# mayursharma/PageRank-using-Apache-Spark

Measured on AMD Instinct MI355X. Metric: PageRank GTEPS/iter + % HBM roofline, R-MAT scale-26 at 1/2/4/8 MI355X, higher is better.
Workload: dtype f64

## Files before the change

include/pagerank_hip.h:

```cpp
#ifndef PAGERANK_HIP_H
#define PAGERANK_HIP_H

#include <stdint.h>

#ifdef __cplusplus
extern "C" {
#endif

#define PR_ABI_VERSION 2

#define PR_OK 0
#define PR_ERR_INVALID (-1)
#define PR_ERR_HIP (-2)
#define PR_ERR_OOM (-3)
#define PR_ERR_COMM (-4)
#define PR_ERR_STATE (-5)
#define PR_ERR_NODEVICE (-6)

#define PR_DANGLING_LOCAL 0u
#define PR_DANGLING_NONE 1u
#define PR_INPUT_DEVICE 2u
#define PR_NO_CANONICAL 4u
#define PR_LAYOUT_FUSED 8u
#define PR_LAYOUT_SPLIT 16u

#define PR_VF_KEY 1u
#define PR_VF_SINK 2u
#define PR_VF_NOLINK 4u
#define PR_VF_INDEG0 8u

#define PR_INFO_N_VERTICES 0
#define PR_INFO_N_EDGES 1
#define PR_INFO_N_SINK 2
#define PR_INFO_N_NOLINK 3
#define PR_INFO_N_INDEG0 4
#define PR_INFO_MAX_INDEG 5
#define PR_INFO_LOCAL_ROWS 6
#define PR_INFO_LOCAL_EDGES 7
#define PR_INFO_PART 8
#define PR_INFO_N_PARTS 9
#define PR_INFO_N_UNITS 10
#define PR_INFO_N_LONG_ROWS 11
#define PR_INFO_DEVICE_BYTES 12
#define PR_INFO_CLASSES 13
#define PR_INFO_XCHG_SEND 14
#define PR_INFO_XCHG_RECV 15
#define PR_INFO_PARTIAL_SLOTS 16
#define PR_INFO_HOT_SLOTS 17
#define PR_INFO_EPILOGUE 18
#define PR_INFO_GATHER_EST 19
#define PR_INFO_WALK_GROUPS 20
#define PR_INFO_LAYOUT 21
#define PR_INFO_HOT_COVER 22
#define PR_INFO_CODE_BITS 23
#define PR_INFO_HOT_GATHER 24
#define PR_INFO_COUNT 25

#define PR_STAT_ITERS 0
#define PR_STAT_LAST_DC 1
#define PR_STAT_LAST_L1 2
#define PR_STAT_SPMV_MS_MEAN 3
#define PR_STAT_SPMV_LAUNCHES 4
#define PR_STAT_ITER_MS_MEAN 5
#define PR_STAT_BUILD_MS 6
#define PR_STAT_EXCHANGE_MS_MEAN 7
#define PR_STAT_COUNT 8

typedef struct pr_graph pr_graph;

typedef void (*pr_iter_cb)(int32_t iter, const double *ranks_or_null, double dangling_sum,
                           double l1_delta, double ms, void *user);
#define PR_CB_RANKS 1u

int pr_abi_version(void);
const char *pr_last_error(void);
int pr_device_count(int32_t *out);

int pr_graph_create(int32_t device, int32_t n_vertices, int64_t n_edges, const int32_t *src,
                    const int32_t *dst, uint32_t flags, pr_graph **out);

int pr_graph_create_part(int32_t device, int32_t part, int32_t n_parts, int32_t n_vertices,
                         int64_t n_edges, const int32_t *src, const int32_t *dst, uint32_t flags,
                         pr_graph **out);

#define PR_BOPT_CLASSES 1
#define PR_BOPT_HOT_SLOTS 2
#define PR_BOPT_EXCHANGE 3
#define PR_BOPT_XCHG_CHUNKS 4
#define PR_BOPT_HOT_RESERVE 5
#define PR_BOPT_EPI_WALK 6
#define PR_BOPT_EPI_NARROW 7
#define PR_BOPT_CODES 8
#define PR_BOPT_PACK_FUSED 9
#define PR_BOPT_XCHG_SDMA 10
#define PR_BOPT_EPI_ORDER 11
int pr_graph_create_ex(int32_t device, int32_t part, int32_t n_parts, int32_t n_vertices, int64_t n_edges,
                       const int32_t *src, const int32_t *dst, uint32_t flags, const int64_t *options,
                       int32_t n_options, pr_graph **out);

int pr_graph_info(const pr_graph *g, int64_t *info, int32_t n_info);

int pr_graph_export_csr(const pr_graph *g, int64_t *row_ptr, int32_t *col_idx, int32_t *out_deg,
                        uint8_t *vflags);

int pr_run(pr_graph *g, int32_t iterations, double teleport, double damping,
           const double *init_ranks, double *ranks_out, pr_iter_cb cb, uint32_t cb_flags,
           void *user);

int pr_reset(pr_graph *g, double teleport, double damping, const double *init_ranks);
int pr_step(pr_graph *g, int32_t iterations);
int pr_sync(pr_graph *g);
int pr_get_ranks(pr_graph *g, double *ranks_out);

int pr_set_teleport(pr_graph *g, const double *teleport);
int pr_set_teleport_sparse(pr_graph *g, int32_t n, const int32_t *ids, const double *values, double rest);

int pr_get_topk(pr_graph *g, int32_t k, int32_t *ids_out, double *ranks_out, int32_t *n_out);
int pr_topk_merge(int32_t n_lists, const int32_t *const *ids, const double *const *ranks,
                  const int32_t *counts, int32_t k, int32_t *ids_out, double *ranks_out, int32_t *n_out);
int pr_set_timing(pr_graph *g, int32_t enable);
int pr_get_stats(pr_graph *g, double *stats, int32_t n_stats);

#define PR_OPT_XCHG_CHUNKS 1
#define PR_OPT_HOT_RESERVE 2
#define PR_OPT_XCHG_IPC 3
#define PR_OPT_XCHG_IPC_BLIT 4
#define PR_OPT_HOT_GATHER 5
int pr_set_option(pr_graph *g, int32_t option, int64_t value);

#define PR_COMM_ID_BYTES 128
int pr_comm_unique_id(uint8_t *id_out);
int pr_graph_attach_comm(pr_graph *g, int32_t rank, int32_t n_ranks, const uint8_t *id);

int pr_group_reset(pr_graph *const *parts, int32_t n_parts, double teleport, double damping,
                   const double *init_ranks);
int pr_group_step(pr_graph *const *parts, int32_t n_parts, int32_t iterations);
int pr_group_sync(pr_graph *const *parts, int32_t n_parts);
int pr_group_topk(pr_graph *const *parts, int32_t n_parts, int32_t k, int32_t *ids_out,
                  double *ranks_out, int32_t *n_out);

void pr_graph_destroy(pr_graph *g);

typedef struct pr_batch pr_batch;
int pr_batch_create(pr_graph *g, int32_t width, pr_batch **out);
int pr_batch_set_teleport(pr_batch *b, int32_t column, const double *teleport);
int pr_batch_set_teleport_sparse(pr_batch *b, int32_t column, int32_t n, const int32_t *ids,
                                 const double *values, double rest);
int pr_batch_reset(pr_batch *b, double teleport, double damping, const double *init_ranks);
int pr_batch_step(pr_batch *b, int32_t iterations);
int pr_batch_step_until(pr_batch *b, int32_t max_iterations, double tol, int32_t *iters_out);
int pr_batch_reset_column(pr_batch *b, int32_t column, const double *init_ranks);
int pr_batch_step_until_any(pr_batch *b, uint32_t active, int32_t max_iterations, double tol,
                            int32_t *executed_out, uint32_t *converged_out);
typedef struct pr_batch_query {
  int32_t n_seeds;
  const int32_t *ids;
  const double *values;
  double rest;
  int32_t n_exclude;
  const int32_t *exclude;
} pr_batch_query;
typedef void (*pr_batch_done_cb)(int32_t query, int32_t column, int32_t iterations, int32_t converged,
                                 double l1, void *user);
int pr_batch_run_queue(pr_batch *b, int32_t n_queries, const pr_batch_query *queries,
                       int32_t max_iterations, double tol, const double *init_ranks,
                       pr_batch_done_cb done, void *user);
#define PR_BATCH_DANGLING_UNIFORM 0
#define PR_BATCH_DANGLING_TELEPORT 1
int pr_batch_set_dangling(pr_batch *b, int32_t mode);
int pr_batch_get_dangling(const pr_batch *b, int32_t *mode_out);
int pr_batch_get_teleport_sums(pr_batch *b, double *sums_out);
int pr_batch_sync(pr_batch *b);
int pr_batch_get_ranks(pr_batch *b, int32_t column, double *ranks_out);
int pr_batch_get_norms(pr_batch *b, double *dc_out, double *l_out);
int pr_batch_get_topk(pr_batch *b, int32_t column, int32_t k, int32_t *ids_out, double *ranks_out,
                      int32_t *n_out);
int pr_batch_set_exclude(pr_batch *b, int32_t column, int32_t n, const int32_t *ids);
int pr_batch_get_topk_all(pr_batch *b, int32_t k, int32_t *ids_out, double *ranks_out, int32_t *n_out);
int pr_batch_info(const pr_batch *b, int64_t *info, int32_t n_info);
void pr_batch_destroy(pr_batch *b);

int pr_gen_rmat(int32_t device, int32_t scale, int64_t n_edges, double a, double b, double c,
                uint64_t seed, int32_t *d_src, int32_t *d_dst);
int pr_gen_er(int32_t device, int32_t scale, int64_t n_edges, uint64_t seed, int32_t *d_src,
              int32_t *d_dst);
int pr_gen_chunglu(int32_t device, int32_t n_labels, int64_t n_edges, double gamma_out, double v0_out,
                   double gamma_in, double v0_in, double src_frac, int64_t n_nolink, uint64_t seed,
                   int32_t *d_src, int32_t *d_dst);
int pr_intern_device(int32_t device, int64_t n_edges, int32_t label_bound, int32_t *d_src,
                     int32_t *d_dst, int32_t *n_vertices_out);

#ifdef __cplusplus
}
#endif

#endif
```

java/src/sparky/hip/PageRankHip.java:

```java
package sparky.hip;

import static java.lang.foreign.ValueLayout.ADDRESS;
import static java.lang.foreign.ValueLayout.JAVA_DOUBLE;
import static java.lang.foreign.ValueLayout.JAVA_INT;
import static java.lang.foreign.ValueLayout.JAVA_LONG;

import java.lang.foreign.Arena;
import java.lang.foreign.FunctionDescriptor;
import java.lang.foreign.Linker;
import java.lang.foreign.MemorySegment;
import java.lang.foreign.SymbolLookup;
import java.lang.invoke.MethodHandle;
import java.lang.invoke.MethodHandles;
import java.lang.invoke.MethodType;

public final class PageRankHip implements AutoCloseable {
    public static final int PR_DANGLING_LOCAL = 0, PR_DANGLING_NONE = 1, PR_NO_CANONICAL = 4;
    static final int PR_CB_RANKS = 1;
    static final int PR_INFO_COUNT = 25;
    public static final int ABI_VERSION = 2;

    private static final Linker LINKER = Linker.nativeLinker();
    private static final SymbolLookup LIB = SymbolLookup.libraryLookup(
            System.getProperty("pagerank.hip.lib", "libpagerank_hip.so"), Arena.global());

    private static MethodHandle h(String name, FunctionDescriptor d) {
        return LINKER.downcallHandle(LIB.find(name).orElseThrow(
                () -> new UnsatisfiedLinkError("libpagerank_hip lacks " + name)), d);
    }

    private static final MethodHandle CREATE = h("pr_graph_create", FunctionDescriptor.of(JAVA_INT,
            JAVA_INT, JAVA_INT, JAVA_LONG, ADDRESS, ADDRESS, JAVA_INT, ADDRESS));
    private static final MethodHandle RUN = h("pr_run", FunctionDescriptor.of(JAVA_INT,
            ADDRESS, JAVA_INT, JAVA_DOUBLE, JAVA_DOUBLE, ADDRESS, ADDRESS, ADDRESS, JAVA_INT, ADDRESS));
    private static final MethodHandle INFO = h("pr_graph_info", FunctionDescriptor.of(JAVA_INT,
            ADDRESS, ADDRESS, JAVA_INT));
    private static final MethodHandle DESTROY = h("pr_graph_destroy", FunctionDescriptor.ofVoid(ADDRESS));
    private static final MethodHandle LAST_ERROR = h("pr_last_error", FunctionDescriptor.of(ADDRESS));
    private static final MethodHandle ABI = h("pr_abi_version", FunctionDescriptor.of(JAVA_INT));

    static {
        try {
            int v = (int) ABI.invokeExact();
            if (v != ABI_VERSION)
                throw new UnsatisfiedLinkError("libpagerank_hip ABI " + v + ", this binding needs " + ABI_VERSION);
        } catch (UnsatisfiedLinkError e) {
            throw e;
        } catch (Throwable t) {
            throw new ExceptionInInitializerError(t);
        }
    }
    private static final FunctionDescriptor CB_DESC = FunctionDescriptor.ofVoid(
            JAVA_INT, ADDRESS, JAVA_DOUBLE, JAVA_DOUBLE, JAVA_DOUBLE, ADDRESS);

    private final Arena arena = Arena.ofConfined();
    private final MemorySegment graph;
    private final int nVertices;
    private IterationListener listener;
    private Throwable listenerError;

    public PageRankHip(int device, int nVertices, int[] src, int[] dst, int flags) throws Throwable {
        if (src.length != dst.length) throw new IllegalArgumentException("src and dst lengths differ");
        this.nVertices = nVertices;
        try (Arena call = Arena.ofConfined()) {
            MemorySegment s = call.allocateFrom(JAVA_INT, src);
            MemorySegment d = call.allocateFrom(JAVA_INT, dst);
            MemorySegment out = call.allocate(ADDRESS);
            check((int) CREATE.invokeExact(device, nVertices, (long) src.length, s, d, flags | PR_NO_CANONICAL, out));
            graph = out.get(ADDRESS, 0);
        }
    }

    public long[] info() throws Throwable {
        try (Arena call = Arena.ofConfined()) {
            MemorySegment a = call.allocate(JAVA_LONG, PR_INFO_COUNT);
            check((int) INFO.invokeExact(graph, a, PR_INFO_COUNT));
            return a.toArray(JAVA_LONG);
        }
    }

    public double[] run(int iterations, double[] initRanks, IterationListener l, boolean ranksInCallback)
            throws Throwable {
        if (initRanks != null && initRanks.length != nVertices)
            throw new IllegalArgumentException("initRanks must hold " + nVertices + " ranks");
        listener = l;
        listenerError = null;
        try (Arena call = Arena.ofConfined()) {
            MemorySegment init = initRanks == null ? MemorySegment.NULL : call.allocateFrom(JAVA_DOUBLE, initRanks);
            MemorySegment out = call.allocate(JAVA_DOUBLE, Math.max(nVertices, 1));
            MemorySegment cb = MemorySegment.NULL;
            if (l != null) {
                MethodHandle target = MethodHandles.lookup().findVirtual(PageRankHip.class, "upcall",
                        MethodType.methodType(void.class, int.class, MemorySegment.class, double.class,
                                double.class, double.class, MemorySegment.class)).bindTo(this);
                cb = LINKER.upcallStub(target, CB_DESC, call);
            }
            int rc = (int) RUN.invokeExact(graph, iterations, 0.15, 0.85, init, out, cb,
                    ranksInCallback ? PR_CB_RANKS : 0, MemorySegment.NULL);
            if (listenerError != null) throw listenerError;
            check(rc);
            return out.asSlice(0, 8L * nVertices).toArray(JAVA_DOUBLE);
        } finally {
            listener = null;
        }
    }

    private void upcall(int iter, MemorySegment ranks, double dc, double l1, double ms, MemorySegment user) {
        if (listenerError != null) return;
        try {
            double[] r = ranks.equals(MemorySegment.NULL) ? null
                    : ranks.reinterpret(8L * nVertices).toArray(JAVA_DOUBLE);
            listener.onIteration(iter, r, dc, l1, ms);
        } catch (Throwable t) {
            listenerError = t;
        }
    }

    private static void check(int rc) throws Throwable {
        if (rc != 0) {
            MemorySegment msg = (MemorySegment) LAST_ERROR.invokeExact();
            throw new RuntimeException("libpagerank_hip error " + rc + ": " + msg.reinterpret(4096).getString(0));
        }
    }

    @Override
    public void close() throws Throwable {
        DESTROY.invokeExact(graph);
        arena.close();
    }
}
```

pagerank-using-apache-spark_amd/csrc/pr_api.hip:

```cpp
#include <rccl/rccl.h>

#include <algorithm>
#include <chrono>
#include <cmath>
#include <cstring>
#include <new>
#include <string>
#include <vector>

#include "pr_graph.h"
#include "pr_topk.h"
#include "pr_xcheck.h"

namespace pr {

static thread_local std::string g_last_error;

void set_error(const std::string &msg) { g_last_error = msg; }
int fail(int code, const std::string &msg) {
  g_last_error = msg;
  return code;
}

int DevBuf::alloc(size_t n) {
  reset();
  if (n == 0) n = 1;
  hipError_t e = hipMalloc(&p, n);
  if (e != hipSuccess) {
    p = nullptr;
    (void)hipGetLastError();
    return fail(PR_ERR_OOM, "hipMalloc(" + std::to_string(n) + " bytes) failed: " + hipGetErrorString(e));
  }
  bytes = n;
  return PR_OK;
}

void DevBuf::reset() {
  if (p) (void)hipFree(p);
  p = nullptr;
  bytes = 0;
}

}

size_t pr_graph::device_bytes() const {
  size_t b = canon_rowptr.bytes + canon_col.bytes + canon_deg.bytes + canon_vflags.bytes;
  b += rowptr.bytes + col.bytes + colp.bytes + rowinfo.bytes + colh.bytes + hunits.bytes + partial.bytes + poff.bytes + rmask.bytes + cbase.bytes + seg_slot.bytes + seg_p0.bytes + r.bytes + cbuf[0].bytes + cbuf[1].bytes + eoff.bytes + epos.bytes;
  b += units.bytes + unit_part.bytes + lr_row.bytes + lr_p0.bytes + piece_part.bytes;
  b += fin_part.bytes + fin_counter.bytes + reset_part.bytes + x_send.bytes + x_sbuf.bytes + hpos.bytes + cside.bytes;
  b += pr::topk_bytes(this);
  b += tele.bytes;
  return b;
}

using pr::fail;

namespace {

struct DeviceGuard {
  int prev = -1;
  explicit DeviceGuard(int dev) {
    if (hipGetDevice(&prev) != hipSuccess) prev = -1;
    (void)hipSetDevice(dev);
  }
  ~DeviceGuard() {
    if (prev >= 0) (void)hipSetDevice(prev);
  }
};

int check_device(int32_t device) {
  int n = 0;
  hipError_t e = hipGetDeviceCount(&n);
  if (e != hipSuccess || n <= 0) {
    (void)hipGetLastError();
    return fail(PR_ERR_NODEVICE, "no HIP device available");
  }
  if (device < 0 || device >= n) return fail(PR_ERR_INVALID, "device index out of range");
  return PR_OK;
}

int parse_options(const int64_t *options, int32_t n, pr_build_opts *o) {
  if (n < 0 || (n > 0 && !options)) return fail(PR_ERR_INVALID, "options is NULL");
  for (int32_t i = 0; i < n; ++i) {
    const int64_t k = options[2 * i], v = options[2 * i + 1];
    switch (k) {
      case PR_BOPT_CLASSES:
        if (v != 0 && v != 8 && v != 16 && v != 32 && v != 64 && v != 128)
          return fail(PR_ERR_INVALID, "PR_BOPT_CLASSES: 0 (policy), 8, 16, 32, 64 or 128");
        o->classes = (int)v;
        break;
      case PR_BOPT_HOT_SLOTS:
        if (v < -1 || v > pr::kHotSlotsMax) return fail(PR_ERR_INVALID, "PR_BOPT_HOT_SLOTS: -1 (default) or 0..18429");
        o->hot_slots = (int)v;
        break;
      case PR_BOPT_EXCHANGE:
        if (v != 0 && v != 1) return fail(PR_ERR_INVALID, "PR_BOPT_EXCHANGE: 0 (runs) or 1 (all-gather)");
        o->allgather = v == 1;
        break;
      case PR_BOPT_XCHG_CHUNKS:
        if (v != 0 && v != 1) return fail(PR_ERR_INVALID, "PR_BOPT_XCHG_CHUNKS: 0 (whole runs) or 1 (overlapped)");
        o->xchg_chunks = v == 1;
        break;
      case PR_BOPT_HOT_RESERVE:
        if (v < 0 || v > 3) return fail(PR_ERR_INVALID, "PR_BOPT_HOT_RESERVE: 0..3 CUs per XCD");
        o->hot_reserve = (int)v;
        break;
      case PR_BOPT_EPI_WALK:
        if (v != 0 && v != 1) return fail(PR_ERR_INVALID, "PR_BOPT_EPI_WALK: 0 (class loop) or 1 (per-row walk)");
        o->epi_walk = v == 1;
        break;
      case PR_BOPT_EPI_NARROW:
        if (v < -1 || v > 1) return fail(PR_ERR_INVALID, "PR_BOPT_EPI_NARROW: -1 (auto), 0 or 1");
        o->epi_narrow = (int)v;
        break;
      case PR_BOPT_CODES:
        if (v != -1 && v != 0) return fail(PR_ERR_INVALID, "PR_BOPT_CODES: -1 (compact where they fit) or 0 (32-bit)");
        o->codes = (int)v;
        break;
      case PR_BOPT_PACK_FUSED:
        if (v != 0 && v != 1) return fail(PR_ERR_INVALID, "PR_BOPT_PACK_FUSED: 0 (pack kernel) or 1 (in the epilogue)");
        o->pack_fused = v == 1;
        break;
      case PR_BOPT_XCHG_SDMA:
        if (v != 0 && v != 1) return fail(PR_ERR_INVALID, "PR_BOPT_XCHG_SDMA: 0 (device copies) or 1 (copy engines)");
        o->xchg_sdma = v == 1;
        break;
      case PR_BOPT_EPI_ORDER:
        if (v < -1 || v > 2)
          return fail(PR_ERR_INVALID, "PR_BOPT_EPI_ORDER: -1 (auto), 0 (row order), 1 (runs of 8 groups heaviest first), "
                                      "2 (groups heaviest first)");
        o->epi_order = (int)v;
        break;
      default:
        return fail(PR_ERR_INVALID, "unknown build option " + std::to_string(k));
    }
  }
  return PR_OK;
}

int create_common(int32_t device, int32_t part, int32_t n_parts, int32_t n_vertices, int64_t n_edges,
                  const int32_t *src, const int32_t *dst, uint32_t flags, const int64_t *options,
                  int32_t n_options, pr_graph **out) {
  if (!out) return fail(PR_ERR_INVALID, "out is NULL");
  *out = nullptr;
  if (n_parts < 1 || part < 0 || part >= n_parts) return fail(PR_ERR_INVALID, "bad part / n_parts");
  if (n_parts > pr::kMaxParts) return fail(PR_ERR_INVALID, "n_parts above 64 is not supported");
  if (n_vertices < 0 || n_edges < 0) return fail(PR_ERR_INVALID, "negative size");
  if (n_edges > 0 && (!src || !dst)) return fail(PR_ERR_INVALID, "src/dst is NULL");
  if (flags & ~(PR_DANGLING_NONE | PR_INPUT_DEVICE | PR_NO_CANONICAL | PR_LAYOUT_FUSED | PR_LAYOUT_SPLIT))
    return fail(PR_ERR_INVALID, "unknown flag bits");
  if ((flags & PR_LAYOUT_FUSED) && (flags & PR_LAYOUT_SPLIT)) return fail(PR_ERR_INVALID, "PR_LAYOUT_FUSED and PR_LAYOUT_SPLIT are exclusive");
  pr_build_opts opts;
  PR_TRY(parse_options(options, n_options, &opts));
  PR_TRY(check_device(device));
  DeviceGuard dg(device);
  pr_graph *g = new (std::nothrow) pr_graph();
  if (!g) return fail(PR_ERR_OOM, "host allocation failed");
  g->opts = opts;
  g->device = device;
  g->flags = flags;
  g->V = n_vertices;
  g->part = part;
  g->nparts = n_parts;
  if (hipStreamCreateWithFlags(&g->stream, hipStreamNonBlocking) != hipSuccess) {
    delete g;
    return fail(PR_ERR_HIP, "hipStreamCreate failed");
  }
  int rc = pr::build_graph(g, n_edges, src, dst);
  if (rc != PR_OK) {
    std::string msg = pr_last_error();
    pr_graph_destroy(g);
    pr::set_error(msg);
    return rc;
  }
  *out = g;
  return PR_OK;
}

}

extern "C" {

int pr_abi_version(void) { return PR_ABI_VERSION; }

const char *pr_last_error(void) { return pr::g_last_error.c_str(); }

int pr_device_count(int32_t *out) {
  if (!out) return fail(PR_ERR_INVALID, "out is NULL");
  int n = 0;
  hipError_t e = hipGetDeviceCount(&n);
  if (e != hipSuccess) {
    (void)hipGetLastError();
    n = 0;
  }
  *out = n;
  return PR_OK;
}

int pr_graph_create(int32_t device, int32_t n_vertices, int64_t n_edges, const int32_t *src,
                    const int32_t *dst, uint32_t flags, pr_graph **out) {
  return create_common(device, 0, 1, n_vertices, n_edges, src, dst, flags, nullptr, 0, out);
}

int pr_graph_create_part(int32_t device, int32_t part, int32_t n_parts, int32_t n_vertices,
                         int64_t n_edges, const int32_t *src, const int32_t *dst, uint32_t flags,
                         pr_graph **out) {
  return create_common(device, part, n_parts, n_vertices, n_edges, src, dst, flags, nullptr, 0, out);
}

int pr_graph_create_ex(int32_t device, int32_t part, int32_t n_parts, int32_t n_vertices, int64_t n_edges,
                       const int32_t *src, const int32_t *dst, uint32_t flags, const int64_t *options,
                       int32_t n_options, pr_graph **out) {
  return create_common(device, part, n_parts, n_vertices, n_edges, src, dst, flags, options, n_options, out);
}

static int64_t xchg_volume(const pr_graph *g, bool send) {
  if (g->nparts <= 1) return 0;
  if (g->x_allgather) return (send ? 1 : g->nparts - 1) * g->S_pad;
  const std::vector<int64_t> &o = send ? g->x_soff : g->x_roff;
  return o.empty() ? 0 : o.back();
}

int pr_graph_info(const pr_graph *g, int64_t *info, int32_t n_info) {
  if (!g || !info) return fail(PR_ERR_INVALID, "NULL argument");
  const int64_t v[PR_INFO_COUNT] = {g->V,        g->E_dedup,  g->n_sink,    g->n_nolink, g->n_indeg0,
                                    g->max_indeg, g->n_local,  g->local_nnz, g->part,     g->nparts,
                                    g->n_units + g->n_hunits, g->n_long + g->n_segs,
                                    (int64_t)g->device_bytes(), g->C,
                                    xchg_volume(g, true), xchg_volume(g, false), g->n_slots,
                                    g->C > 1 ? (int64_t)g->hot.P * g->hot.Kp : 0,
                                    g->C == 1 ? 0 : 3, g->gather_est, g->n_walk_groups, g->layout,
                                    g->hot_cover_ppm, g->C > 1 ? (g->code == pr::kCodeC20 || g->code == pr::kCodeC20P ? 20 : g->code == pr::kCodeC24 || g->code == pr::kCodeC24P ? 24 : 32) : 0,
                                    pr::hot_gather_dense(g) ? 1 : 0};
  for (int32_t i = 0; i < n_info && i < PR_INFO_COUNT; ++i) info[i] = v[i];
  return PR_OK;
}

int pr_graph_export_csr(const pr_graph *g, int64_t *row_ptr, int32_t *col_idx, int32_t *out_deg,
                        uint8_t *vflags) {
  if (!g) return fail(PR_ERR_INVALID, "NULL graph");
  if (!g->has_canonical) return fail(PR_ERR_STATE, "canonical CSR was dropped (PR_NO_CANONICAL)");
  DeviceGuard dg(g->device);
  hipStream_t s = g->stream;
  if (row_ptr)
    PR_HIP(hipMemcpyAsync(row_ptr, g->canon_rowptr.p, sizeof(int64_t) * ((size_t)g->V + 1), hipMemcpyDeviceToHost, s));
  if (col_idx && g->E_dedup > 0)
    PR_HIP(hipMemcpyAsync(col_idx, g->canon_col.p, sizeof(int32_t) * g->E_dedup, hipMemcpyDeviceToHost, s));
  if (out_deg && g->V > 0)
    PR_HIP(hipMemcpyAsync(out_deg, g->canon_deg.p, sizeof(int32_t) * g->V, hipMemcpyDeviceToHost, s));
  if (vflags && g->V > 0)
    PR_HIP(hipMemcpyAsync(vflags, g->canon_vflags.p, (size_t)g->V, hipMemcpyDeviceToHost, s));
  PR_HIP(hipStreamSynchronize(s));
  return PR_OK;
}

int pr_reset(pr_graph *g, double teleport, double damping, const double *init_ranks) {
  if (!g) return fail(PR_ERR_INVALID, "NULL graph");
  DeviceGuard dg(g->device);
  g->teleport = teleport;
  g->damping = damping;
  return pr::iter_reset(g, init_ranks);
}

int pr_set_teleport(pr_graph *g, const double *teleport) {
  if (!g) return fail(PR_ERR_INVALID, "NULL graph");
  if (teleport)
    for (int32_t v = 0; v < g->V; ++v)
      if (!std::isfinite(teleport[v])) return fail(PR_ERR_INVALID, "teleport[" + std::to_string(v) + "] is not finite");
  DeviceGuard dg(g->device);
  return teleport ? pr::set_teleport_dense(g, teleport) : pr::clear_teleport(g);
}

int pr_set_teleport_sparse(pr_graph *g, int32_t n, const int32_t *ids, const double *values, double rest) {
  if (!g) return fail(PR_ERR_INVALID, "NULL graph");
  if (n < 0) return fail(PR_ERR_INVALID, "n < 0");
  if (n > 0 && (!ids || !values)) return fail(PR_ERR_INVALID, "NULL argument");
  if (!std::isfinite(rest)) return fail(PR_ERR_INVALID, "rest is not finite");
  for (int32_t i = 0; i < n; ++i) {
    if (ids[i] < 0 || ids[i] >= g->V)
      return fail(PR_ERR_INVALID, "ids[" + std::to_string(i) + "] = " + std::to_string(ids[i]) + " is outside [0, V)");
    if (!std::isfinite(values[i])) return fail(PR_ERR_INVALID, "values[" + std::to_string(i) + "] is not finite");
  }
  if (n > 1) {
    std::vector<int32_t> sorted(ids, ids + n);
    std::sort(sorted.begin(), sorted.end());
    const auto dup = std::adjacent_find(sorted.begin(), sorted.end());
    if (dup != sorted.end()) return fail(PR_ERR_INVALID, "vertex " + std::to_string(*dup) + " is listed twice in ids");
  }
  DeviceGuard dg(g->device);
  return pr::set_teleport_sparse(g, n, ids, values, rest);
}

int pr_step(pr_graph *g, int32_t iterations) {
  if (!g || iterations < 0) return fail(PR_ERR_INVALID, "bad argument");
  DeviceGuard dg(g->device);
  return pr::iter_step(g, iterations);
}

int pr_sync(pr_graph *g) {
  if (!g) return fail(PR_ERR_INVALID, "NULL graph");
  DeviceGuard dg(g->device);
  PR_TRY(pr::join_exchange(g));
  PR_HIP(hipStreamSynchronize(g->stream));
  return PR_OK;
}

int pr_get_ranks(pr_graph *g, double *ranks_out) {
  if (!g || !ranks_out) return fail(PR_ERR_INVALID, "NULL argument");
  if (!g->ready) return fail(PR_ERR_STATE, "pr_get_ranks before pr_reset");
  DeviceGuard dg(g->device);
  std::vector<double> loc((size_t)g->n_rows);
  if (g->n_rows > 0)
    PR_HIP(hipMemcpyAsync(loc.data(), g->r.p, sizeof(double) * g->n_rows, hipMemcpyDeviceToHost, g->stream));
  PR_HIP(hipStreamSynchronize(g->stream));
  for (int64_t L = 0; L < g->n_rows; ++L)
    if (g->orig_of_local[L] >= 0) ranks_out[g->orig_of_local[L]] = loc[L];
  return PR_OK;
}

int pr_set_timing(pr_graph *g, int32_t enable) {
  if (!g) return fail(PR_ERR_INVALID, "NULL graph");
  g->timing = enable != 0;
  return PR_OK;
}

int pr_set_option(pr_graph *g, int32_t option, int64_t value) {
  if (!g) return fail(PR_ERR_INVALID, "NULL graph");
  DeviceGuard dg(g->device);
  if (option == PR_OPT_HOT_RESERVE) {
    if (value < 0 || value > 3) return fail(PR_ERR_INVALID, "PR_OPT_HOT_RESERVE: 0..3 CUs per XCD");
    if (g->C > 1) PR_TRY(pr::set_hot_reserve(g, (int)value));
    return PR_OK;
  }
  if (option == PR_OPT_HOT_GATHER) {
    if (value < -1 || value > 1) return fail(PR_ERR_INVALID, "PR_OPT_HOT_GATHER: -1 (auto), 0 (per position) or 1 (dense)");
    if (g->C > 1) g->hot_gather = (int)value;
    return PR_OK;
  }
  if (option == PR_OPT_XCHG_IPC_BLIT) {
    if (value != 0 && value != 1) return fail(PR_ERR_INVALID, "PR_OPT_XCHG_IPC_BLIT: 0 (copy engines) or 1 (blit kernel)");
    PR_TRY(pr::join_exchange(g));
    g->x_ipc_blit = value == 1;
    return PR_OK;
  }
  if (option == PR_OPT_XCHG_IPC) {
    if (value < 0 || value > 2)
      return fail(PR_ERR_INVALID, "PR_OPT_XCHG_IPC: 0 (RCCL), 1 (IPC copy engines) or 2 (IPC, per-chunk publication)");
    return pr::set_exchange_ipc(g, (int)value);
  }
  if (option != PR_OPT_XCHG_CHUNKS) return fail(PR_ERR_INVALID, "unknown option");
  PR_TRY(pr::join_exchange(g));
  g->x_chunked = value != 0 && g->n_xc > 1;
  if (g->comm && g->comm_size > 1) PR_TRY(pr::verify_exchange(g));
  return PR_OK;
}

int pr_get_stats(pr_graph *g, double *stats, int32_t n_stats) {
  if (!g || !stats) return fail(PR_ERR_INVALID, "NULL argument");
  DeviceGuard dg(g->device);
  PR_TRY(pr::join_exchange(g));
  PR_HIP(hipStreamSynchronize(g->stream));
  auto mean_ms = [&](const std::vector<std::pair<int, int>> &ev, double *out) -> int {
    double acc = 0.0;
    for (auto &pr_ : ev) {
      float ms = 0.f;
      PR_HIP(hipEventElapsedTime(&ms, g->ev_pool[pr_.first], g->ev_pool[pr_.second]));
      acc += ms;
    }
    *out = ev.empty() ? 0.0 : acc / (double)ev.size();
    return PR_OK;
  };
  double v[PR_STAT_COUNT] = {0};
  v[PR_STAT_ITERS] = (double)g->iters_done;
  if (g->ready) {
    PR_TRY(pr::read_slots(g, g->cur, &v[PR_STAT_LAST_DC], &v[PR_STAT_LAST_L1]));
    if (g->iters_done > 0) {
      double dc_prev = 0, l1_prev = 0;
      PR_TRY(pr::read_slots(g, g->cur ^ 1, &dc_prev, &l1_prev));
      v[PR_STAT_LAST_DC] = dc_prev;
    } else {
      v[PR_STAT_LAST_L1] = 0.0;
    }
  }
  PR_TRY(mean_ms(g->spmv_ev, &v[PR_STAT_SPMV_MS_MEAN]));
  if (g->spmv_passes > 0) v[PR_STAT_SPMV_MS_MEAN] *= (double)g->spmv_ev.size() / (double)g->spmv_passes;
  v[PR_STAT_SPMV_LAUNCHES] = (double)g->spmv_passes;
  if (g->xchg_ev.size() == g->iter_ev.size() && !g->xchg_ev.empty()) {
    double acc = 0.0;
    for (size_t i = 0; i < g->iter_ev.size(); ++i) {
      float a = 0.f, b = 0.f;
      PR_HIP(hipEventElapsedTime(&a, g->ev_pool[g->iter_ev[i].first], g->ev_pool[g->iter_ev[i].second]));
      PR_HIP(hipEventElapsedTime(&b, g->ev_pool[g->iter_ev[i].first], g->ev_pool[g->xchg_ev[i].second]));
      acc += a > b ? a : b;
    }
    v[PR_STAT_ITER_MS_MEAN] = acc / (double)g->iter_ev.size();
  } else {
    PR_TRY(mean_ms(g->iter_ev, &v[PR_STAT_ITER_MS_MEAN]));
    if (g->iter_timed > 0) v[PR_STAT_ITER_MS_MEAN] *= (double)g->iter_ev.size() / (double)g->iter_timed;
  }
  v[PR_STAT_BUILD_MS] = g->build_ms;
  PR_TRY(mean_ms(g->xchg_ev, &v[PR_STAT_EXCHANGE_MS_MEAN]));
  for (int32_t i = 0; i < n_stats && i < PR_STAT_COUNT; ++i) stats[i] = v[i];
  return PR_OK;
}

int pr_run(pr_graph *g, int32_t iterations, double teleport, double damping,
           const double *init_ranks, double *ranks_out, pr_iter_cb cb, uint32_t cb_flags,
           void *user) {
  if (!g || iterations < 0) return fail(PR_ERR_INVALID, "bad argument");
  DeviceGuard dg(g->device);
  g->teleport = teleport;
  g->damping = damping;
  PR_TRY(pr::iter_reset(g, init_ranks));
  std::vector<double> cb_ranks;
  if (cb && (cb_flags & PR_CB_RANKS)) {
    cb_ranks.assign((size_t)g->V, 0.0);
    if (init_ranks) std::memcpy(cb_ranks.data(), init_ranks, sizeof(double) * g->V);
  }
  for (int32_t it = 0; it < iterations; ++it) {
    if (!cb) {
      PR_TRY(pr::iter_step(g, iterations));
      break;
    }
    auto t0 = std::chrono::steady_clock::now();
    double dc = 0, l1 = 0, dummy = 0;
    PR_TRY(pr::read_slots(g, g->cur, &dc, &dummy));
    PR_TRY(pr::iter_step(g, 1));
    PR_HIP(hipStreamSynchronize(g->stream));
    PR_TRY(pr::read_slots(g, g->cur, &dummy, &l1));
    const double ms = std::chrono::duration<double, std::milli>(std::chrono::steady_clock::now() - t0).count();
    const double *rp = nullptr;
    if (cb_flags & PR_CB_RANKS) {
      PR_TRY(pr_get_ranks(g, cb_ranks.data()));
      rp = cb_ranks.data();
    }
    cb(it, rp, dc, l1, ms, user);
  }
  PR_HIP(hipStreamSynchronize(g->stream));
  if (ranks_out) PR_TRY(pr_get_ranks(g, ranks_out));
  return PR_OK;
}

int pr_comm_unique_id(uint8_t *id_out) {
  if (!id_out) return fail(PR_ERR_INVALID, "NULL argument");
  static_assert(sizeof(ncclUniqueId) == PR_COMM_ID_BYTES, "ncclUniqueId size");
  ncclUniqueId id;
  ncclResult_t rc = ncclGetUniqueId(&id);
  if (rc != ncclSuccess) return fail(PR_ERR_COMM, std::string("ncclGetUniqueId: ") + ncclGetErrorString(rc));
  std::memcpy(id_out, &id, sizeof(id));
  return PR_OK;
}

int pr_graph_attach_comm(pr_graph *g, int32_t rank, int32_t n_ranks, const uint8_t *id) {
  if (!g || !id) return fail(PR_ERR_INVALID, "NULL argument");
  if (n_ranks != g->nparts || rank != g->part)
    return fail(PR_ERR_INVALID, "rank/n_ranks must equal the graph's part/n_parts");
  if (g->comm) return fail(PR_ERR_STATE, "communicator already attached");
  DeviceGuard dg(g->device);
  if (!g->comm_scratch.p) {
    const size_t xrec = sizeof(int64_t) * (size_t)pr::xrec_width(n_ranks) * (size_t)(n_ranks + 1);
    PR_TRY(g->comm_scratch.alloc(std::max(pr::kCommScratchBytes, xrec)));
  }
  ncclUniqueId uid;
  std::memcpy(&uid, id, sizeof(uid));
  ncclResult_t rc = ncclCommInitRank(&g->comm, n_ranks, uid, rank);
  if (rc != ncclSuccess) {
    g->comm = nullptr;
    return fail(PR_ERR_COMM, std::string("ncclCommInitRank: ") + ncclGetErrorString(rc));
  }
  g->comm_rank = rank;
  g->comm_size = n_ranks;
  if (n_ranks > 1) {
    const int rv = pr::verify_exchange(g);
    if (rv != PR_OK) {
      ncclCommDestroy(g->comm);
      g->comm = nullptr;
      return rv;
    }
  }
  return PR_OK;
}

static int check_group(pr_graph *const *parts, int32_t n) {
  if (!parts || n < 1) return fail(PR_ERR_INVALID, "bad group");
  for (int32_t p = 0; p < n; ++p) {
    const pr_graph *g = parts[p];
    if (!g) return fail(PR_ERR_INVALID, "NULL part in group");
    if (g->nparts != n || g->part != p) return fail(PR_ERR_INVALID, "parts[p] must be part p of n_parts");
    if (g->V != parts[0]->V || g->S_pad != parts[0]->S_pad) return fail(PR_ERR_INVALID, "parts of different graphs");
    if (g->comm) return fail(PR_ERR_STATE, "a part with an RCCL communicator cannot join a group");
    if (g->x_allgather != parts[0]->x_allgather) return fail(PR_ERR_INVALID, "parts built with different PR_BOPT_EXCHANGE");
  }
  return PR_OK;
}

int pr_group_reset(pr_graph *const *parts, int32_t n_parts, double teleport, double damping,
                   const double *init_ranks) {
  PR_TRY(check_group(parts, n_parts));
  for (int32_t p = 0; p < n_parts; ++p) {
    pr_graph *g = parts[p];
    PR_HIP(hipSetDevice(g->device));
    if (!g->xev) PR_HIP(hipEventCreateWithFlags(&g->xev, hipEventDisableTiming));
    for (int32_t q = 0; q < n_parts; ++q) {
      if (parts[q]->device == g->device) continue;
      int can = 0;
      if (hipDeviceCanAccessPeer(&can, g->device, parts[q]->device) == hipSuccess && can) {
        hipError_t e = hipDeviceEnablePeerAccess(parts[q]->device, 0);
        if (e != hipSuccess && e != hipErrorPeerAccessAlreadyEnabled) PR_HIP(e);
        (void)hipGetLastError();
      }
    }
    g->grouped = true;
    g->teleport = teleport;
    g->damping = damping;
    PR_TRY(pr::iter_reset(g, init_ranks));
  }
  PR_TRY(pr::group_exchange(parts, n_parts, 0));
  for (int32_t p = 0; p < n_parts; ++p) {
    PR_HIP(hipSetDevice(parts[p]->device));
    PR_TRY(pr::join_exchange(parts[p]));
    PR_HIP(hipStreamSynchronize(parts[p]->stream));
    parts[p]->xchg_ev.clear();
  }
  return PR_OK;
}

int pr_group_step(pr_graph *const *parts, int32_t n_parts, int32_t iterations) {
  PR_TRY(check_group(parts, n_parts));
  if (iterations < 0) return fail(PR_ERR_INVALID, "iterations < 0");
  for (int32_t p = 0; p < n_parts; ++p)
    if (!parts[p]->grouped || !parts[p]->ready) return fail(PR_ERR_STATE, "pr_group_step before pr_group_reset");
  std::vector<int> i0((size_t)n_parts, -1);
  for (int32_t it = 0; it < iterations; ++it) {
    for (int32_t p = 0; p < n_parts; ++p) {
      PR_HIP(hipSetDevice(parts[p]->device));
      if (parts[p]->timing) PR_TRY(pr::time_mark(parts[p], parts[p]->stream, &i0[p]));
      PR_TRY(pr::iter_compute(parts[p]));
    }
    PR_TRY(pr::group_exchange(parts, n_parts, parts[0]->cur));
    for (int32_t p = 0; p < n_parts; ++p) {
      if (!parts[p]->timing) continue;
      PR_HIP(hipSetDevice(parts[p]->device));
      int i1 = -1;
      PR_TRY(pr::time_mark(parts[p], parts[p]->stream, &i1));
      parts[p]->iter_ev.push_back({i0[p], i1});
      ++parts[p]->iter_timed;
    }
  }
  return PR_OK;
}

int pr_group_sync(pr_graph *const *parts, int32_t n_parts) {
  PR_TRY(check_group(parts, n_parts));
  for (int32_t p = 0; p < n_parts; ++p) {
    PR_HIP(hipSetDevice(parts[p]->device));
    PR_TRY(pr::join_exchange(parts[p]));
    PR_HIP(hipStreamSynchronize(parts[p]->stream));
  }
  return PR_OK;
}

static int topk_args(int32_t k, const int32_t *ids_out, const double *ranks_out, const int32_t *n_out) {
  if (k < 0) return fail(PR_ERR_INVALID, "k < 0");
  if (!n_out || (k > 0 && (!ids_out || !ranks_out))) return fail(PR_ERR_INVALID, "NULL argument");
  return PR_OK;
}

int pr_get_topk(pr_graph *g, int32_t k, int32_t *ids_out, double *ranks_out, int32_t *n_out) {
  if (!g) return fail(PR_ERR_INVALID, "NULL graph");
  PR_TRY(topk_args(k, ids_out, ranks_out, n_out));
  if (!g->ready) return fail(PR_ERR_STATE, "pr_get_topk before pr_reset");
  DeviceGuard dg(g->device);
  return pr::topk_part(g, k, pr::kTopkNarrowDiv, ids_out, ranks_out, n_out, nullptr);
}

int pr_topk_select_ex(pr_graph *g, int32_t k, int64_t narrow_div, int32_t *ids_out, double *ranks_out,
                      int32_t *n_out, int32_t *info) {
  if (!g) return fail(PR_ERR_INVALID, "NULL graph");
  PR_TRY(topk_args(k, ids_out, ranks_out, n_out));
  if (narrow_div < 0) return fail(PR_ERR_INVALID, "narrow_div < 0");
  if (!g->ready) return fail(PR_ERR_STATE, "pr_get_topk before pr_reset");
  DeviceGuard dg(g->device);
  return pr::topk_part(g, k, narrow_div, ids_out, ranks_out, n_out, info);
}

int pr_topk_merge(int32_t n_lists, const int32_t *const *ids, const double *const *ranks, const int32_t *counts,
                  int32_t k, int32_t *ids_out, double *ranks_out, int32_t *n_out) {
  if (n_lists < 0) return fail(PR_ERR_INVALID, "n_lists < 0");
  PR_TRY(topk_args(k, ids_out, ranks_out, n_out));
  if (n_lists > 0 && (!ids || !ranks || !counts)) return fail(PR_ERR_INVALID, "NULL argument");
  for (int32_t l = 0; l < n_lists; ++l) {
    if (counts[l] < 0) return fail(PR_ERR_INVALID, "negative list length");
    if (counts[l] > 0 && (!ids[l] || !ranks[l])) return fail(PR_ERR_INVALID, "NULL list");
  }
  auto head = [&](int32_t l, int32_t i) {
    uint64_t bits;
    std::memcpy(&bits, &ranks[l][i], sizeof(bits));
    return pr::TopkPair{pr::topk_rank_key(bits), ids[l][i]};
  };
  std::vector<int32_t> at((size_t)n_lists, 0);
  int32_t n = 0;
  for (; n < k; ++n) {
    int32_t best = -1;
    pr::TopkPair bp{0, 0};
    for (int32_t l = 0; l < n_lists; ++l) {
      if (at[l] >= counts[l]) continue;
      const pr::TopkPair h = head(l, at[l]);
      if (best < 0 || pr::topk_before(h, bp)) {
        best = l;
        bp = h;
      }
    }
    if (best < 0) break;
    ids_out[n] = ids[best][at[best]];
    ranks_out[n] = ranks[best][at[best]];
    ++at[best];
  }
  *n_out = n;
  return PR_OK;
}

int pr_group_topk(pr_graph *const *parts, int32_t n_parts, int32_t k, int32_t *ids_out, double *ranks_out,
                  int32_t *n_out) {
  PR_TRY(check_group(parts, n_parts));
  PR_TRY(topk_args(k, ids_out, ranks_out, n_out));
  for (int32_t p = 0; p < n_parts; ++p)
    if (!parts[p]->ready) return fail(PR_ERR_STATE, "pr_group_topk before pr_group_reset");
  std::vector<std::vector<int32_t>> lid((size_t)n_parts);
  std::vector<std::vector<double>> lrk((size_t)n_parts);
  std::vector<const int32_t *> pid((size_t)n_parts);
  std::vector<const double *> prk((size_t)n_parts);
  std::vector<int32_t> cnt((size_t)n_parts, 0);
  for (int32_t p = 0; p < n_parts; ++p) {
    pr_graph *g = parts[p];
    const size_t m = (size_t)std::min<int64_t>(k, g->n_local);
    lid[p].resize(m + 1);
    lrk[p].resize(m + 1);
    DeviceGuard dg(g->device);
    PR_TRY(pr::topk_part(g, k, pr::kTopkNarrowDiv, lid[p].data(), lrk[p].data(), &cnt[p], nullptr));
    pid[p] = lid[p].data();
    prk[p] = lrk[p].data();
  }
  return pr_topk_merge(n_parts, pid.data(), prk.data(), cnt.data(), k, ids_out, ranks_out, n_out);
}

void pr_graph_destroy(pr_graph *g) {
  if (!g) return;
  DeviceGuard dg(g->device);
  if (g->ipc) {
    const bool idle = pr::stream_idle_within(g->stream, 30.0) && pr::stream_idle_within(g->xstream, 30.0);
    if (!idle) {
      pr::set_error("pr_graph_destroy: a stream did not drain within 30 s (a peer of the IPC exchange died?); "
                    "the handle is leaked");
      return;
    }
  }
  if (g->stream) (void)hipStreamSynchronize(g->stream);
  if (g->xstream) (void)hipStreamSynchronize(g->xstream);
  pr::ipc_destroy(g);
  pr::topk_destroy(g);
  if (g->comm) (void)ncclCommDestroy(g->comm);
  for (hipEvent_t e : g->ev_pool) (void)hipEventDestroy(e);
  if (g->xev) (void)hipEventDestroy(g->xev);
  for (hipEvent_t e : g->x_ev) (void)hipEventDestroy(e);
  if (g->x_pack_ev) (void)hipEventDestroy(g->x_pack_ev);
  if (g->x_free_ev) (void)hipEventDestroy(g->x_free_ev);
  if (g->xstream) (void)hipStreamDestroy(g->xstream);
  g->ev_pool.clear();
  hipStream_t s = g->stream;
  g->stream = nullptr;
  delete g;
  if (s) (void)hipStreamDestroy(s);
}

}
```

pagerank-using-apache-spark_amd/csrc/pr_build.hip:

```cpp
#include <algorithm>
#include <cstdlib>
#include <chrono>
#include <vector>

#include "pr_compact.h"
#include "pr_device.h"
#include "pr_graph.h"
#include "pr_plan.h"

namespace pr {
namespace {

constexpr uint64_t kSentinel = ~0ull;

__global__ void k_pack_edges(int64_t E, int32_t V, int b, const int32_t *__restrict__ src,
                             const int32_t *__restrict__ dst, uint64_t *__restrict__ keys,
                             uint8_t *__restrict__ appear, uint8_t *__restrict__ is_key,
                             unsigned *__restrict__ err) {
  for (int64_t i = blockIdx.x * (int64_t)blockDim.x + threadIdx.x; i < E;
       i += (int64_t)gridDim.x * blockDim.x) {
    const int32_t s = src[i], d = dst[i];
    if (s < 0 || s >= V || d < -1 || d >= V) {
      atomicOr(err, 1u);
      keys[i] = kSentinel;
// ... 544 lines not shown
  g->n_nolink = (int64_t)hc[1];
  g->n_indeg0 = (int64_t)hc[2];
  g->max_indeg = (int64_t)hc[3];
  const uint64_t max_outdeg = hc[4];

  g->n_local_max = (V + P - 1) / P;
  g->n_local = V > part ? (V - part + P - 1) / P : 0;
  if (max_outdeg > kRowDegMask) return fail(PR_ERR_INVALID, "out-degree above 2^28-1 is not supported");
  int64_t gather_est = g->n_local_max * 8;
  if (P > 1 && V > 0) {
    PR_HIP(hipMemsetAsync(cnt.p, 0, sizeof(unsigned long long), s));
    hipLaunchKernelGGL(k_reader_est, dim3(grid_for(V, T, 1024)), dim3(T), 0, s, V, P, c_deg.as<int32_t>(),
                       cnt.as<unsigned long long>());
    PR_HIP(hipGetLastError());
    unsigned long long est = 0;
    PR_HIP(hipMemcpyAsync(&est, cnt.p, sizeof(est), hipMemcpyDeviceToHost, s));
    PR_HIP(hipStreamSynchronize(s));
    gather_est += (int64_t)((double)est / 1048576.0 * (double)(P - 1) / (double)P) * 8;
  }
  g->gather_est = gather_est;
  const int bd = bits_for(max_outdeg);
  const uint64_t maxd = (uint64_t(1) << bd) - 1;
  DevBuf vk, vtmp, rank_of, gpos;
  PR_TRY(vk.alloc(sizeof(uint64_t) * ((size_t)V + 1)));
  PR_TRY(vtmp.alloc(sizeof(uint64_t) * ((size_t)V + 1)));
  PR_TRY(rank_of.alloc(sizeof(int32_t) * ((size_t)V + 1)));
  PR_TRY(gpos.alloc(sizeof(int32_t) * ((size_t)V + 1)));
  if (V > 0) {
    hipLaunchKernelGGL(k_order_keys, dim3(grid_for(V, T, 4096)), dim3(T), 0, s, V, b, maxd, c_deg.as<int32_t>(),
                       vk.as<uint64_t>());
    PR_TRY(radix_sort_u64(vk.as<uint64_t>(), vtmp.as<uint64_t>(), V, 0, b + bd, s));
  }
  vtmp.reset();
  const int c_split = class_setting(g->opts, gather_est);
  const bool big = (int64_t)P * g->n_local_max * 8 > kSplitMinSliceBytes;
  int layout = big ? kLayoutSplit : kLayoutFused;
  if (g->flags & PR_LAYOUT_FUSED) layout = kLayoutFused;
  if (g->flags & PR_LAYOUT_SPLIT) layout = kLayoutSplit;
  if ((int64_t)P * (g->n_local_max + 64 + kMaxClasses) * 8 >= (1ll << 31) - (1ll << 20)) layout = kLayoutFused;
  int C = layout == kLayoutSplit ? c_split : 1;
  g->layout = layout;
  g->C = C;
  g->Q_pad = (g->n_local_max + C - 1) / C;
  g->Q_pad = (g->Q_pad + 63) / 64 * 64;
  g->n_rows = (int64_t)C * g->Q_pad;
  g->S_pad = ((g->n_rows + 2 + 63) / 64) * 64;
  if ((int64_t)P * g->S_pad >= (int64_t(1) << 31)) return fail(PR_ERR_INVALID, "gather space exceeds 2^31 entries");
  if (V > 0) {
    hipLaunchKernelGGL(k_rank_gpos, dim3(grid_for(V, T, 65536)), dim3(T), 0, s, V, maskb, P, C,
                       g->Q_pad, g->S_pad, vk.as<uint64_t>(), rank_of.as<int32_t>(), gpos.as<int32_t>());
    PR_HIP(hipGetLastError());
  }
  ClassGeom geo{};
  geo.C = C;
  geo.Q_pad = g->Q_pad;
  geo.S_pad = g->S_pad;
  g->geo = geo;

  DevBuf cmap;
  PR_TRY(build_exchange(g, ukeys, m, b, maskb, rank_of.as<int32_t>(), gpos.as<int32_t>(), &cmap));

  const int64_t R = g->n_rows;
  const int bg = bits_for((uint64_t)P * g->S_pad);
  const int brow = bits_for((uint64_t)R);
  const int bseg = bits_for((uint64_t)C);
  const uint64_t maskg = (uint64_t(1) << bg) - 1;
  int64_t lm = 0;
  PR_TRY(compact_index(m, PartPred{ukeys, rank_of.as<int32_t>(), b, P, part},
                       PartXform{ukeys, gpos.as<int32_t>(), b, bg, brow, maskb, geo},
                       keys.as<uint64_t>(), &lm, s));
  g->local_nnz = lm;
  PR_TRY(radix_sort_u64(keys.as<uint64_t>(), tmp.as<uint64_t>(), lm, 0, bg + brow + bseg, s));
  PR_TRY(g->col.alloc(sizeof(int32_t) * (lm > 0 ? lm : 1)));
  if (lm > 0)
    hipLaunchKernelGGL(k_local_col, dim3(grid_for(lm, T, 65536)), dim3(T), 0, s,
                       keys.as<uint64_t>(), lm, maskg, g->col.as<int32_t>());
  if (cmap.p && lm > 0) {
    DevBuf bad;
    PR_TRY(bad.alloc(sizeof(unsigned long long)));
    PR_HIP(hipMemsetAsync(bad.p, 0, sizeof(unsigned long long), s));
    hipLaunchKernelGGL(k_map_cols, dim3(grid_for(lm, T, 65536)), dim3(T), 0, s, lm, cmap.as<int32_t>(),
                       g->col.as<int32_t>(), bad.as<unsigned long long>());
    unsigned long long hb = 0;
    PR_HIP(hipMemcpyAsync(&hb, bad.p, sizeof(hb), hipMemcpyDeviceToHost, s));
    PR_HIP(hipStreamSynchronize(s));
    if (hb) return fail(PR_ERR_STATE, "exchange lists miss a source of this part's in-links");
  }
  PR_TRY(g->rowinfo.alloc(sizeof(uint32_t) * ((size_t)R + 1)));
  DevBuf orig;
  PR_TRY(orig.alloc(sizeof(int32_t) * ((size_t)R + 1)));
  hipLaunchKernelGGL(k_local_rows, dim3(grid_for(R, T, 65536)), dim3(T), 0, s, R, g->n_local, P, part,
                     geo, maskb, (g->flags & PR_DANGLING_NONE) != 0, vk.as<uint64_t>(),
                     c_deg.as<int32_t>(), c_vflags.as<uint8_t>(), g->rowinfo.as<uint32_t>(),
                     orig.as<int32_t>());
  PR_HIP(hipGetLastError());
  vk.reset();
  rank_of.reset();
  gpos.reset();

  const uint64_t rmask = (uint64_t(1) << brow) - 1;
  std::vector<int64_t> rp;
  std::vector<int32_t> seg_p0;
  std::vector<int32_t> lr_row, lr_p0;
  std::vector<Unit> light_units;
  int64_t pieces = 0;
  g->nblk = (R + 63) / 64;
  std::vector<int64_t> poff(kMaxClasses + 1, 0);
  if (C == 1) {
    DevBuf rp_dev;
    PR_TRY(rp_dev.alloc(sizeof(int64_t) * ((size_t)R + 1)));
    hipLaunchKernelGGL(k_row_ptr_seg, dim3(grid_for(lm + 1, T, 65536)), dim3(T), 0, s, keys.as<uint64_t>(),
                       (int64_t)0, lm, bg, rmask, R, rp_dev.as<int64_t>());
    PR_HIP(hipGetLastError());
    rp.assign((size_t)R + 1, 0);
    PR_HIP(hipMemcpyAsync(rp.data(), rp_dev.p, sizeof(int64_t) * rp.size(), hipMemcpyDeviceToHost, s));
    PR_HIP(hipStreamSynchronize(s));
    keys.reset();
    tmp.reset();
    UnitPlan px;
    plan_units(rp, kUnitNnz, kUnitRows, &px);
    g->rowptr = std::move(rp_dev);
    lr_row = px.lr_row;
    lr_p0 = px.lr_p0;
    light_units = px.units;
    pieces = px.n_pieces;
    if (px.padded_len / 8 >= (int64_t(1) << 32)) return fail(PR_ERR_INVALID, "graph part too large for 32-bit unit offsets");
    PR_TRY(g->colp.alloc(sizeof(int32_t) * (px.padded_len > 0 ? px.padded_len : 8)));
    PR_TRY(build_padded_cols(px, g->col.as<int32_t>(), g->colp.as<int32_t>(), s));
    seg_p0.push_back(0);
  } else {
    SplitPlanner sp;
    PR_TRY(sp.segments(keys.as<uint64_t>(), lm, bg, brow, C, R, g->col.as<int32_t>(), s));
    keys.reset();
    tmp.reset();
    for (int x = 0; x <= C; ++x) poff[x] = sp.cseg[x];
    for (int x = C; x < kMaxClasses; ++x) poff[x + 1] = poff[x];
    for (int x = 0; x < C; ++x)
      if (poff[x + 1] - poff[x] >= (int64_t(1) << 29)) return fail(PR_ERR_INVALID, "a column class exceeds 2^29 segments");
    if (poff[C] >= (int64_t(1) << 31) - 4) return fail(PR_ERR_INVALID, "more than 2^31 - 4 partial slots");
    PR_TRY(sp.block_bases(true, s));
    PR_TRY(sp.units_plan(s));
    g->rmask = std::move(sp.rmask);
    g->cbase = std::move(sp.cbase);
    PR_TRY(plan_epi_walk(g));
    pieces = sp.n_pieces;
    if (sp.entries / 8 >= (int64_t(1) << 32)) return fail(PR_ERR_INVALID, "graph part too large for 32-bit unit offsets");
    int slots = hot_slots_setting(g->opts);
    const bool compact = g->opts.codes != 0 && P == 1 && g->gsize == g->S_pad;
    g->code = compact && g->Q_pad < (int64_t(1) << kC20IdxBits)   ? kCodeC20
              : compact && g->Q_pad < (int64_t(1) << kC24IdxBits) ? kCodeC24
                                                                   : kCodeU32;
    PiecePlan pplan;
    if (g->opts.codes != 0 && P > 1 && P <= kMaxPackParts) {
      PR_TRY(plan_pieces(g, cmap.p ? cmap.as<int32_t>() : nullptr, C, P, &pplan, s));
      HotGeom t{};
      t.P = P;
      t.tbl = 1;
      int ps = slots;
      for (;; --ps) {
        t.Kp = ps / P;
        if (t.lds_bytes() <= (size_t)kHotLdsBytes) break;
      }
      const int64_t top = (int64_t)P * (ps / P) + pplan.vmax;
      g->code = top < (int64_t(1) << kC20IdxBits)   ? kCodeC20P
                : top < (int64_t(1) << kC24IdxBits) ? kCodeC24P
                                                     : kCodeU32;
      if (code_is_piece(g->code)) slots = ps;
    }
    HotGeom hg{};
    hg.C = C;
    hg.P = P;
    hg.Kp = slots / P;
    hg.q_load = (int)std::min<int64_t>(hg.Kp, g->Q_pad);
    hg.S_pad = g->S_pad;
    hg.Q_pad = g->Q_pad;
    hg.tbl = code_is_piece(g->code) ? 1 : 0;
    g->hot = hg;
    DevBuf hotidx;
    const int64_t nh = (int64_t)P * hg.Kp;
    PR_TRY(g->hpos.alloc(sizeof(int32_t) * (size_t)(C * nh > 0 ? C * nh : 1)));
    PR_TRY(hotidx.alloc(sizeof(int32_t) * (size_t)g->gsize));
    PR_HIP(hipMemsetAsync(hotidx.p, 0, sizeof(int32_t) * (size_t)g->gsize, s));
    if (C * nh > 0)
      hipLaunchKernelGGL(k_hot_tables, dim3(grid_for(C * nh, T, 65536)), dim3(T), 0, s, hg,
                         cmap.p ? cmap.as<int32_t>() : nullptr, g->hpos.as<int32_t>(), hotidx.as<int32_t>());
    PR_HIP(hipGetLastError());
    int n_cu = 0;
    PR_HIP(hipDeviceGetAttribute(&n_cu, hipDeviceAttributeMultiprocessorCount, g->device));
    g->hot_grid = std::max(C, n_cu / C * C);
    g->hot_grid_full = g->hot_grid;
    PR_TRY(set_hot_reserve(g, g->opts.hot_reserve));

    PR_TRY(prepare_hot_kernel());
    const int64_t nu = sp.n_units;
    g->n_hunits = nu;
    g->hunits = std::move(sp.units);
    PR_TRY(g->hucum.alloc(sizeof(int64_t) * (kMaxClasses + 1)));
    PR_TRY(g->poff.alloc(sizeof(int64_t) * (kMaxClasses + 1)));
    const bool c20 = g->code == kCodeC20 || g->code == kCodeC20P, c24 = g->code == kCodeC24 || g->code == kCodeC24P;
    const bool piece = code_is_piece(g->code);
    if (piece) {
      PR_TRY(g->ptab.alloc(sizeof(int32_t) * pplan.tbl.size()));
      PR_HIP(hipMemcpyAsync(g->ptab.p, pplan.tbl.data(), sizeof(int32_t) * pplan.tbl.size(), hipMemcpyHostToDevice, s));
    }
    DevBuf pcd;
    if (piece) {
      PR_TRY(pcd.alloc(sizeof(int32_t) * pplan.pc.size()));
      PR_HIP(hipMemcpyAsync(pcd.p, pplan.pc.data(), sizeof(int32_t) * pplan.pc.size(), hipMemcpyHostToDevice, s));
    }
    if (c20 || c24) {
      PR_TRY(g->colh.alloc(sizeof(uint16_t) * (sp.entries > 0 ? sp.entries : 8)));
      PR_TRY(g->cside.alloc((c24 ? sizeof(uint64_t) : sizeof(uint32_t)) * (sp.entries > 0 ? sp.entries / 8 : 1)));
    } else {
      PR_TRY(g->colh.alloc(sizeof(uint32_t) * (sp.entries > 0 ? sp.entries : 8)));
      PR_TRY(g->cside.alloc(sizeof(uint32_t)));
    }
    PR_TRY(g->partial.alloc(sizeof(double) * (size_t)(poff[C] + 2)));
    g->n_slots = poff[C];
    PR_HIP(hipMemcpyAsync(g->hucum.p, sp.ucum.data(), sizeof(int64_t) * (kMaxClasses + 1), hipMemcpyHostToDevice, s));
    PR_HIP(hipMemcpyAsync(g->poff.p, poff.data(), sizeof(int64_t) * (kMaxClasses + 1), hipMemcpyHostToDevice, s));
    if (nu > 0) {
      PR_HIP(hipMemsetAsync(cnt.p, 0, 2 * sizeof(unsigned long long), s));
      const unsigned fgrid = (unsigned)std::min<int64_t>(nu, 65536);
      const int nhs = P * hg.Kp;
      if (piece && c20)
        hipLaunchKernelGGL((k_fill_piece<3, uint32_t>), dim3(fgrid), dim3(64), 0, s, nu, g->hunits.as<Unit>(),
                           sp.src_off.as<int64_t>(), sp.n_real.as<int32_t>(), g->col.as<int32_t>(),
                           g->hucum.as<int64_t>(), C, P, pcd.as<int32_t>(), hotidx.as<int32_t>(), nhs,
                           g->colh.as<uint16_t>(), g->cside.as<uint32_t>(), cnt.as<unsigned long long>(),
                           cnt.as<unsigned long long>() + 1);
      else if (piece)
        hipLaunchKernelGGL((k_fill_piece<4, uint64_t>), dim3(fgrid), dim3(64), 0, s, nu, g->hunits.as<Unit>(),
                           sp.src_off.as<int64_t>(), sp.n_real.as<int32_t>(), g->col.as<int32_t>(),
                           g->hucum.as<int64_t>(), C, P, pcd.as<int32_t>(), hotidx.as<int32_t>(), nhs,
                           g->colh.as<uint16_t>(), g->cside.as<uint64_t>(), cnt.as<unsigned long long>(),
                           cnt.as<unsigned long long>() + 1);
      else if (c20)
        hipLaunchKernelGGL((k_fill_compact<3, uint32_t>), dim3((unsigned)std::min<int64_t>(nu, 65536)), dim3(64), 0, s,
                           nu, g->hunits.as<Unit>(), sp.src_off.as<int64_t>(), sp.n_real.as<int32_t>(),
                           g->col.as<int32_t>(), g->Q_pad, hg.q_load, g->colh.as<uint16_t>(),
                           g->cside.as<uint32_t>(), cnt.as<unsigned long long>(), cnt.as<unsigned long long>() + 1);
      else if (c24)
        hipLaunchKernelGGL((k_fill_compact<4, uint64_t>), dim3((unsigned)std::min<int64_t>(nu, 65536)), dim3(64), 0, s,
                           nu, g->hunits.as<Unit>(), sp.src_off.as<int64_t>(), sp.n_real.as<int32_t>(),
                           g->col.as<int32_t>(), g->Q_pad, hg.q_load, g->colh.as<uint16_t>(),
                           g->cside.as<uint64_t>(), cnt.as<unsigned long long>(), cnt.as<unsigned long long>() + 1);
      else
        hipLaunchKernelGGL(k_fill_hot, dim3((unsigned)std::min<int64_t>(nu, 65536)), dim3(256), 0, s, nu,
                           g->hunits.as<Unit>(), sp.src_off.as<int64_t>(), sp.n_real.as<int32_t>(),
                           g->col.as<int32_t>(), hotidx.as<int32_t>(), g->colh.as<uint32_t>(),
                           cnt.as<unsigned long long>());
      PR_HIP(hipGetLastError());
      unsigned long long n_hot[2] = {0, 0};
      PR_HIP(hipMemcpyAsync(n_hot, cnt.p, sizeof(n_hot), hipMemcpyDeviceToHost, s));
      PR_HIP(hipStreamSynchronize(s));
      if (n_hot[1]) return fail(PR_ERR_STATE, "compact codes: a unit reads outside its class region / pieces");
      g->hot_cover_ppm = lm > 0 ? (int64_t)((double)n_hot[0] * 1e6 / (double)lm) : 0;
    }
    g->n_segs = sp.n_long;
    g->seg_slot = std::move(sp.seg_slot);
    g->seg_p0 = std::move(sp.seg_p0);
  }
  g->col.reset();
  if (lr_p0.empty()) lr_p0.push_back((int32_t)pieces);
  g->n_units = (int64_t)light_units.size();
  g->n_long = (int64_t)lr_row.size();
  g->n_pieces = pieces;
  PR_TRY(g->units.alloc(sizeof(Unit) * (light_units.size() + 1)));
  PR_TRY(g->lr_row.alloc(sizeof(int32_t) * (lr_row.size() + 1)));
  PR_TRY(g->lr_p0.alloc(sizeof(int32_t) * (lr_p0.size() + 1)));
  if (C == 1) {
    g->n_segs = 0;
    PR_TRY(g->seg_slot.alloc(sizeof(int64_t)));
    PR_TRY(g->seg_p0.alloc(sizeof(int32_t) * (seg_p0.size() + 1)));
    PR_HIP(hipMemcpyAsync(g->seg_p0.p, seg_p0.data(), sizeof(int32_t) * seg_p0.size(), hipMemcpyHostToDevice, s));
  }
  PR_TRY(g->piece_part.alloc(sizeof(double) * ((size_t)g->n_pieces + 1)));
  if (!light_units.empty())
    PR_HIP(hipMemcpyAsync(g->units.p, light_units.data(), sizeof(Unit) * light_units.size(), hipMemcpyHostToDevice, s));
  if (!lr_row.empty())
    PR_HIP(hipMemcpyAsync(g->lr_row.p, lr_row.data(), sizeof(int32_t) * lr_row.size(), hipMemcpyHostToDevice, s));
  PR_HIP(hipMemcpyAsync(g->lr_p0.p, lr_p0.data(), sizeof(int32_t) * lr_p0.size(), hipMemcpyHostToDevice, s));
  g->orig_of_local.resize((size_t)R);
  if (R > 0)
    PR_HIP(hipMemcpyAsync(g->orig_of_local.data(), orig.p, sizeof(int32_t) * R, hipMemcpyDeviceToHost, s));
  PR_HIP(hipStreamSynchronize(s));

  PR_TRY(g->r.alloc(sizeof(double) * ((size_t)g->n_rows + 1)));
  for (int k = 0; k < 2; ++k) {
    PR_TRY(g->cbuf[k].alloc(sizeof(double) * (size_t)g->gsize));
    PR_HIP(hipMemsetAsync(g->cbuf[k].p, 0, sizeof(double) * (size_t)g->gsize, s));
  }
  g->fin_blocks = (int)std::min<int64_t>(512, std::max<int64_t>(16, (g->n_long + kThreads / kWave - 1) / (kThreads / kWave)));
  PR_TRY(g->fin_part.alloc(sizeof(double) * 2 * g->fin_blocks));
  PR_TRY(g->fin_counter.alloc(sizeof(unsigned) * 4));
  PR_HIP(hipMemsetAsync(g->fin_counter.p, 0, sizeof(unsigned) * 4, s));
  g->reset_blocks = (int)grid_for(g->n_rows > 0 ? g->n_rows : 1, 256, 2048);
  if (C > 1) {
    const int64_t ngrp = (g->nblk + kEpiGroup - 1) / kEpiGroup;
    const bool auto_narrow = g->n_walk_groups * 10 >= ngrp;
    g->epi_narrow = epi_narrow_ok(C) && (g->opts.epi_narrow < 0 ? auto_narrow : g->opts.epi_narrow != 0);
    g->ep_blocks = (int)grid_for(ngrp, epi_grp_threads(g->epi_narrow) / kWave, 1u << 20);
    PR_TRY(plan_epi_order(g));
  }
  const int64_t ep_parts = C > 1 ? (g->nblk + kEpiGroup - 1) / kEpiGroup : 0;
  PR_TRY(g->unit_part.alloc(sizeof(double) * 2 * ((size_t)g->n_units + ep_parts + 1)));
  PR_TRY(g->reset_part.alloc(sizeof(double) * 2 * g->reset_blocks));

  if (g->flags & PR_NO_CANONICAL) {
    c_rowptr.reset();
    c_col.reset();
    c_deg.reset();
    c_vflags.reset();
    g->has_canonical = false;
  } else {
    g->canon_rowptr = std::move(c_rowptr);
    g->canon_col = std::move(c_col);
    g->canon_deg = std::move(c_deg);
    g->canon_vflags = std::move(c_vflags);
    g->has_canonical = true;
  }
  PR_HIP(hipStreamSynchronize(s));
  g->build_ms = std::chrono::duration<double, std::milli>(std::chrono::steady_clock::now() - t_start).count();
  return PR_OK;
}

}
```

pagerank-using-apache-spark_amd/csrc/pr_graph.h:

```cpp
#pragma once

#include <rccl/rccl.h>

#include <vector>

#include "pr_internal.h"

namespace pr {
struct IpcState;
struct TopkState;
}

struct pr_build_opts {
  int classes = 0;
  int hot_slots = -1;
  bool allgather = false;
  bool xchg_chunks = false;
  int hot_reserve = 0;
  bool epi_walk = true;
  int epi_narrow = -1;
  int codes = -1;
  bool pack_fused = true;
  bool xchg_sdma = false;
  int epi_order = -1;
};

struct pr_graph {
  int device = 0;
  hipStream_t stream = nullptr;
  uint32_t flags = 0;
  pr_build_opts opts;

  int32_t V = 0;
  int64_t E_dedup = 0;
  int part = 0, nparts = 1;
  int64_t n_local = 0;
  int64_t n_rows = 0;
  int layout = 0;
  int C = 1;
  int64_t gather_est = 0;
  int64_t Q_pad = 0;
  int64_t n_local_max = 0;
  int64_t S_pad = 0;
  int64_t local_nnz = 0;

  int64_t n_sink = 0, n_nolink = 0, n_indeg0 = 0, max_indeg = 0;
  int64_t n_units = 0, n_long = 0, n_pieces = 0;
  double build_ms = 0.0;

  pr::DevBuf canon_rowptr, canon_col, canon_deg, canon_vflags;
  bool has_canonical = false;

  pr::DevBuf rowptr, col, colp, rowinfo, r;
  pr::DevBuf colh, hunits, hucum, poff, partial, rmask, cbase, seg_slot, seg_p0, hpos;
  int code = pr::kCodeU32;
  pr::DevBuf cside;
  pr::DevBuf ptab;
  int ep_blocks = 0;
  pr::ClassGeom geo{};
  pr::HotGeom hot{};
  int hot_grid = 0;
  int hot_grid_full = 0;
  int hot_gather = -1;
  bool epi_walk = false;
  bool epi_narrow = false;
  int64_t n_walk_groups = 0;
  pr::DevBuf eoff, epos;
  pr::DevBuf epi_ord;
  int64_t n_hunits = 0, n_segs = 0, nblk = 0, n_slots = 0;
  int64_t hot_cover_ppm = 0;
  pr::DevBuf cbuf[2];
  pr::DevBuf units, unit_part;
  pr::DevBuf lr_row, lr_p0, piece_part;
  pr::DevBuf fin_part, fin_counter;
  pr::DevBuf reset_part;
  int fin_blocks = 0;
  int reset_blocks = 0;
  std::vector<int32_t> orig_of_local;

  double teleport = 0.15, damping = 0.85;
  pr::DevBuf tele;
  bool tele_on = false;
  int cur = 0;
  int64_t iters_done = 0;
  bool ready = false;

  bool timing = false;
  std::vector<hipEvent_t> ev_pool;
  std::vector<std::pair<int, int>> spmv_ev, iter_ev, xchg_ev;
  int64_t spmv_passes = 0, iter_timed = 0;
  size_t ev_next = 0;
  int ev_start_hint = -1;

  int64_t gsize = 0;
  int64_t own_off = 0;
  pr::SlotPos slots{};
  pr::DevBuf x_send, x_sbuf;
  std::vector<int64_t> x_soff, x_roff;
  bool x_allgather = false;
  int n_xc = 1;
  bool x_chunked = false;
  std::vector<int64_t> x_sch, x_rch;
  hipStream_t xstream = nullptr;
  std::vector<hipEvent_t> x_ev;
  hipEvent_t x_pack_ev = nullptr;
  bool x_pending = false;
  bool x_fused = false;
  pr::DevBuf x_pmask, x_sbase;
  int x_packed = -1;

  pr::IpcState *ipc = nullptr;
  bool x_ipc = false;
  bool x_ipc_early = false;
  bool x_ipc_blit = false;
  hipEvent_t x_free_ev = nullptr;

  ncclComm_t comm = nullptr;
  int comm_rank = 0, comm_size = 1;
  pr::DevBuf comm_scratch;
  bool grouped = false;
  hipEvent_t xev = nullptr;

  pr::TopkState *topk = nullptr;

  size_t device_bytes() const;
};

namespace pr {
constexpr size_t kCommScratchBytes = 256 << 10;
int build_graph(pr_graph *g, int64_t n_edges, const int32_t *src, const int32_t *dst);
int iter_reset(pr_graph *g, const double *init_ranks_host);
int plan_epi_walk(pr_graph *g);
int plan_epi_order(pr_graph *g);
int prepare_hot_kernel();
int prepare_tele_kernels(const pr_graph *g);
int set_teleport_dense(pr_graph *g, const double *teleport);
int set_teleport_sparse(pr_graph *g, int32_t n, const int32_t *ids, const double *values, double rest);
int clear_teleport(pr_graph *g);
int launch_hot(pr_graph *g, int in_buf, int ph0 = 0, int ph1 = -1);
int join_exchange(pr_graph *g);
void set_exchange_chunking(pr_graph *g);
int n_hot_phases(const pr_graph *g);
int set_hot_reserve(pr_graph *g, int per_xcd);
bool hot_gather_dense(const pr_graph *g);
int iter_step(pr_graph *g, int32_t iterations);
int iter_compute(pr_graph *g);
int group_exchange(pr_graph *const *parts, int n, int buf);
int build_exchange(pr_graph *g, const uint64_t *ukeys, int64_t m, int b, uint64_t mask, const int32_t *rank_of,
                   const int32_t *gpos, DevBuf *cmap);
int exchange(pr_graph *g, int buf, hipEvent_t ev_a = nullptr, hipEvent_t ev_b = nullptr);
double *send_runs(const pr_graph *g, int buf);
int verify_exchange(pr_graph *g);
int read_slots(pr_graph *g, int buf, double *dc, double *l1);
int set_exchange_ipc(pr_graph *g, int mode);
int ipc_send_runs_free(pr_graph *g, int buf);
bool ipc_early(const pr_graph *g);
int ipc_chunk_sent(pr_graph *g, int buf, int c);
int exchange_ipc(pr_graph *g, int buf, hipEvent_t ev_a, hipEvent_t ev_b);
void ipc_destroy(pr_graph *g);
bool stream_idle_within(hipStream_t s, double seconds);
hipEvent_t next_event(pr_graph *g);
int time_mark(pr_graph *g, hipStream_t s, int *index);
constexpr int64_t kTopkNarrowDiv = 8;
int topk_part(pr_graph *g, int64_t k, int64_t narrow_div, int32_t *ids_out, double *ranks_out, int32_t *n_out,
              int32_t *info);
size_t topk_bytes(const pr_graph *g);
void topk_destroy(pr_graph *g);
int topk_select(TopkState **state, int device, hipStream_t s, const double *r, const int32_t *oid, int64_t n_rows,
                int64_t n_owned, int64_t k, int64_t narrow_div, int32_t *ids_out, double *ranks_out, int32_t *n_out,
                int32_t *info);
size_t topk_state_bytes(const TopkState *t);
void topk_state_free(TopkState *t);
struct BTopkState;
int btopk_select(BTopkState **state, int device, hipStream_t s, const double *R, int64_t V, int width, int stride,
                 const uint16_t *mask, const int64_t *n_excl, int64_t k, int64_t narrow_div, int32_t *ids_out,
                 double *ranks_out, int32_t *n_out, int32_t *info);
int64_t btopk_kernel_ns(const BTopkState *t);
size_t btopk_state_bytes(const BTopkState *t);
void btopk_state_free(BTopkState *t);
}
```

pagerank-using-apache-spark_amd/csrc/pr_iter.hip:

```cpp
#include <algorithm>
#include <climits>
#include <vector>

#include "pr_device.h"
#include "pr_graph.h"
#include "pr_ipc_protocol.h"
#include "pr_spmv.h"

namespace pr {
namespace {

__device__ __forceinline__ void store_sc1(double *p, double x) {
  __hip_atomic_store(reinterpret_cast<unsigned long long *>(p), (unsigned long long)__double_as_longlong(x),
                     __ATOMIC_RELAXED, __HIP_MEMORY_SCOPE_AGENT);
}
__device__ __forceinline__ double load_sc1(const double *p) {
  return __longlong_as_double((long long)__hip_atomic_load(
      reinterpret_cast<const unsigned long long *>(p), __ATOMIC_RELAXED, __HIP_MEMORY_SCOPE_AGENT));
}

template <bool TELE>
__global__ __launch_bounds__(kThreads) void k_finalize(
    int64_t n_long, const int32_t *__restrict__ lr_row, const int32_t *__restrict__ lr_p0,
    const double *__restrict__ piece_part, const double2 *__restrict__ parts, int64_t n_parts,
    double *__restrict__ r, const uint32_t *__restrict__ rowinfo, const double *__restrict__ cin,
    double *__restrict__ cout, SlotPos sp, double n_vertices, double teleport,
    double damping, double *__restrict__ fin_part, unsigned *__restrict__ counter,
    double *__restrict__ slot_out, PackSlots ps, const double *__restrict__ tele) {
  __shared__ double red[kThreads / kWave];
  __shared__ int is_last;
  const int t = threadIdx.x, lane = lane_id();
  double dcp = 0.0, l1p = 0.0;
  if (n_long > 0) {
    const double tdc = dc_from_slots(cin, sp) / n_vertices;
    const int64_t nw = (int64_t)gridDim.x * (kThreads / kWave);
    for (int64_t q = (int64_t)blockIdx.x * (kThreads / kWave) + wave_id(); q < n_long; q += nw) {
      const int32_t p0 = lr_p0[q], np = lr_p0[q + 1] - p0;
      double acc = 0.0;
      for (int k = lane; k < np; k += kWave) acc = __dadd_rn(acc, piece_part[p0 + k]);
      acc = wave_sum(acc);
      if (lane == 0) {
        const int32_t v = lr_row[q];
        const double rold = r[v];
        double tv = teleport;
        if constexpr (TELE) tv = tele[v];
        const double rn = affine(acc, tdc, tv, damping);
        r[v] = rn;
        const uint32_t info = rowinfo[v];
        const uint32_t d = info & kRowDegMask;
        if (d > 0) cout[v] = __ddiv_rn(rn, (double)d);
        else if (info & kRowSink) dcp = __dadd_rn(dcp, rn);
        l1p = __dadd_rn(l1p, fabs(rn - rold));
      }
    }
  }
  for (int64_t i = (int64_t)blockIdx.x * kThreads + t; i < n_parts; i += (int64_t)gridDim.x * kThreads) {
    const double2 pv = parts[i];
    dcp = __dadd_rn(dcp, pv.x);
    l1p = __dadd_rn(l1p, pv.y);
  }
  dcp = block_sum<kThreads>(dcp, red);
  l1p = block_sum<kThreads>(l1p, red);
  if (t == 0) {
    store_sc1(&fin_part[2 * blockIdx.x], dcp);
    store_sc1(&fin_part[2 * blockIdx.x + 1], l1p);
    asm volatile("s_waitcnt vmcnt(0)" ::: "memory");
    const unsigned prev = __hip_atomic_fetch_add(counter, 1u, __ATOMIC_RELAXED, __HIP_MEMORY_SCOPE_AGENT);
    is_last = (prev == gridDim.x - 1) ? 1 : 0;
  }
  __syncthreads();
  if (!is_last) return;
  double a = 0.0, b = 0.0;
  for (int i = t; i < (int)gridDim.x; i += kThreads) {
    a = __dadd_rn(a, load_sc1(&fin_part[2 * i]));
    b = __dadd_rn(b, load_sc1(&fin_part[2 * i + 1]));
  }
  a = block_sum<kThreads>(a, red);
  b = block_sum<kThreads>(b, red);
  if (t == 0) {
    slot_out[0] = a;
    slot_out[1] = b;
    __hip_atomic_store(counter, 0u, __ATOMIC_RELAXED, __HIP_MEMORY_SCOPE_AGENT);
  }
  if (t < ps.n) {
    ps.sbuf[ps.off[t]] = a;
    ps.sbuf[ps.off[t] + 1] = b;
  }
}

__global__ __launch_bounds__(kThreads) void k_reset(int64_t n_rows, const double *__restrict__ init,
                                                    double *__restrict__ r,
                                                    const uint32_t *__restrict__ rowinfo,
                                                    double *__restrict__ cout,
                                                    double2 *__restrict__ parts) {
  __shared__ double red[kThreads / kWave];
  double dcp = 0.0;
  for (int64_t j = (int64_t)blockIdx.x * kThreads + threadIdx.x; j < n_rows;
       j += (int64_t)gridDim.x * kThreads) {
    const uint32_t info = rowinfo[j];
    if (info & kRowHole) {
      r[j] = 0.0;
      continue;
    }
    const double x = init ? init[j] : 1.0;
    r[j] = x;
    const uint32_t d = info & kRowDegMask;
    if (d > 0) cout[j] = __ddiv_rn(x, (double)d);
    else if (info & kRowSink) dcp = __dadd_rn(dcp, x);
  }
  dcp = block_sum<kThreads>(dcp, red);
  if (threadIdx.x == 0) parts[blockIdx.x] = make_double2(dcp, 0.0);
}

int launch_finalize(pr_graph *g, int64_t n_long, const double2 *parts, int64_t n_parts, int in_buf,
                    int out_buf, hipStream_t stream) {
  double *cout = g->cbuf[out_buf].as<double>() + g->own_off;
  PackSlots ps{};
  if (g->x_fused) {
    ps.sbuf = send_runs(g, out_buf);
    for (int q = 0; q < g->nparts; ++q)
      if (q != g->part) ps.off[ps.n++] = g->x_soff[q + 1] - 2;
  }
  const bool tele = g->tele_on && n_long > 0;
  hipLaunchKernelGGL((tele ? k_finalize<true> : k_finalize<false>), dim3(g->fin_blocks), dim3(kThreads), 0, stream,
                     n_long, g->lr_row.as<int32_t>(), g->lr_p0.as<int32_t>(), g->piece_part.as<double>(),
                     parts, n_parts, g->r.as<double>(), g->rowinfo.as<uint32_t>(),
                     g->cbuf[in_buf].as<double>(), cout, g->slots, (double)g->V,
                     g->teleport, g->damping, g->fin_part.as<double>(), g->fin_counter.as<unsigned>(),
                     cout + g->S_pad - 2, ps, tele ? g->tele.as<double>() : nullptr);
  PR_HIP(hipGetLastError());
  return PR_OK;
}

}

hipEvent_t next_event(pr_graph *g) {
  if (g->ev_next >= g->ev_pool.size()) {
    hipEvent_t e;
    if (hipEventCreate(&e) != hipSuccess) return nullptr;
    g->ev_pool.push_back(e);
  }
  return g->ev_pool[g->ev_next++];
}

int time_mark(pr_graph *g, hipStream_t s, int *index) {
  hipEvent_t e = next_event(g);
  if (!e) return fail(PR_ERR_HIP, "hipEventCreate failed");
  PR_HIP(hipEventRecord(e, s));
  *index = (int)g->ev_next - 1;
  return PR_OK;
}

int prepare_hot_kernel() {
  for (int c : {8, 16, 32, 64, 128})
    for (bool walk : {false, true})
      for (bool narrow : {false, true}) {
        if ((walk || narrow) && c > kWave) continue;
        PR_HIP(hipFuncSetAttribute(reinterpret_cast<const void *>(epi_grp_kernel(c, walk, narrow)),
                                   hipFuncAttributeMaxDynamicSharedMemorySize, (int)epi_grp_lds(narrow)));
      }
  return PR_OK;
}

int prepare_tele_kernels(const pr_graph *g) {
  if (g->C <= 1) return PR_OK;
  PR_HIP(hipFuncSetAttribute(reinterpret_cast<const void *>(epi_grp_kernel(g->C, g->epi_walk, g->epi_narrow, true)),
                             hipFuncAttributeMaxDynamicSharedMemorySize, (int)epi_grp_lds(g->epi_narrow)));
  return PR_OK;
}

int plan_epi_walk(pr_graph *g) {
  g->epi_walk = false;
  g->n_walk_groups = 0;
  if (!g->opts.epi_walk || g->C > kWave || g->nblk <= 0) return PR_OK;
  const int64_t ngrp = (g->nblk + kEpiGroup - 1) / kEpiGroup;
  using PlanFn = void (*)(int64_t, const void *, const int32_t *, int64_t *, uint16_t *);
  PlanFn count = nullptr, write = nullptr;
  switch (g->C) {
    case 8: count = k_epi_walk_plan<8, true>, write = k_epi_walk_plan<8, false>; break;
    case 16: count = k_epi_walk_plan<16, true>, write = k_epi_walk_plan<16, false>; break;
    case 32: count = k_epi_walk_plan<32, true>, write = k_epi_walk_plan<32, false>; break;
    case 64: count = k_epi_walk_plan<64, true>, write = k_epi_walk_plan<64, false>; break;
    default: return PR_OK;
  }
  PR_TRY(g->eoff.alloc(sizeof(int64_t) * (size_t)ngrp));
  const unsigned blocks = grid_for(ngrp, kEpiThreads / kWave, 8192);
  hipLaunchKernelGGL(count, dim3(blocks), dim3(kEpiThreads), 0, g->stream, g->nblk, g->rmask.p, g->cbase.as<int32_t>(),
                     g->eoff.as<int64_t>(), nullptr);
  PR_HIP(hipGetLastError());
  std::vector<int64_t> off((size_t)ngrp);
  PR_HIP(hipMemcpyAsync(off.data(), g->eoff.p, sizeof(int64_t) * (size_t)ngrp, hipMemcpyDeviceToHost, g->stream));
  PR_HIP(hipStreamSynchronize(g->stream));
  int64_t total = 0;
  for (auto &o : off) {
    if (o < 0) continue;
    const int64_t n = o;
    o = total;
    total += n;
    ++g->n_walk_groups;
  }
  PR_TRY(g->epos.alloc(sizeof(uint16_t) * (size_t)(total > 0 ? total : 8)));
  PR_HIP(hipMemcpyAsync(g->eoff.p, off.data(), sizeof(int64_t) * (size_t)ngrp, hipMemcpyHostToDevice, g->stream));
  if (total > 0)
    hipLaunchKernelGGL(write, dim3(blocks), dim3(kEpiThreads), 0, g->stream, g->nblk, g->rmask.p,
                       g->cbase.as<int32_t>(), g->eoff.as<int64_t>(), g->epos.as<uint16_t>());
  PR_HIP(hipGetLastError());
  PR_HIP(hipStreamSynchronize(g->stream));
  g->epi_walk = true;
  return PR_OK;
}

namespace {
__global__ __launch_bounds__(kThreads) void k_epi_cost(int64_t nblk, int C, const int32_t *__restrict__ cbase,
                                                       int32_t *__restrict__ cost) {
  const int64_t ngrp = (nblk + kEpiGroup - 1) / kEpiGroup;
  const int64_t gi = (int64_t)blockIdx.x * kThreads + threadIdx.x;
  if (gi >= ngrp) return;
  const int64_t b0 = gi * kEpiGroup, b1 = min(nblk, b0 + kEpiGroup);
  int64_t n = 0;
  for (int x = 0; x < C; ++x) n += (int64_t)cbase[b1 * C + x] - cbase[b0 * C + x];
  cost[gi] = (int32_t)min(n, (int64_t)INT32_MAX);
}
}

constexpr int64_t kEpiOrderRun = 8;
int plan_epi_order(pr_graph *g) {
  g->epi_ord.reset();
  const int order = g->opts.epi_order >= 0 ? g->opts.epi_order : (g->nparts > 1 ? 2 : 0);
  if (order == 0 || g->C <= 1 || g->nblk <= 0) return PR_OK;
  const int64_t ngrp = (g->nblk + kEpiGroup - 1) / kEpiGroup;
  DevBuf dcost;
  PR_TRY(dcost.alloc(sizeof(int32_t) * (size_t)ngrp));
  hipLaunchKernelGGL(k_epi_cost, dim3((unsigned)((ngrp + kThreads - 1) / kThreads)), dim3(kThreads), 0, g->stream,
                     g->nblk, g->C, g->cbase.as<int32_t>(), dcost.as<int32_t>());
  PR_HIP(hipGetLastError());
  std::vector<int32_t> cost((size_t)ngrp), ord(2 * (size_t)ngrp);
  PR_HIP(hipMemcpyAsync(cost.data(), dcost.p, sizeof(int32_t) * (size_t)ngrp, hipMemcpyDeviceToHost, g->stream));
  PR_HIP(hipStreamSynchronize(g->stream));
  const int64_t run = order == 1 ? kEpiOrderRun : 1;
  auto sort_range = [&](int32_t *o, int64_t lo, int64_t hi) {
    std::vector<std::pair<int64_t, int64_t>> runs;
    for (int64_t a = lo; a < hi; a += run) {
      int64_t n = 0;
      for (int64_t k = a; k < std::min(hi, a + run); ++k) n += cost[k];
      runs.emplace_back(-n, a);
    }
    std::sort(runs.begin(), runs.end());
    int64_t w = lo;
    for (const auto &r : runs)
      for (int64_t k = r.second; k < std::min(hi, r.second + run); ++k) o[w++] = (int32_t)k;
  };
  sort_range(ord.data(), 0, ngrp);
  const int nxc = std::max(1, g->C / kXcds);
  const int64_t rows_per_grp = (int64_t)kEpiGroup * kWave, chunk_rows = (int64_t)kXcds * g->Q_pad;
  int64_t lo = 0;
  for (int c = 0; c < nxc; ++c) {
    const int64_t hi = std::max(lo, ipc_epi_chunk_end(ngrp, c, nxc, chunk_rows, rows_per_grp));
    sort_range(ord.data() + ngrp, lo, hi);
    lo = hi;
  }
  if (lo < ngrp) sort_range(ord.data() + ngrp, lo, ngrp);
  PR_TRY(g->epi_ord.alloc(sizeof(int32_t) * ord.size()));
  PR_HIP(hipMemcpyAsync(g->epi_ord.p, ord.data(), sizeof(int32_t) * ord.size(), hipMemcpyHostToDevice, g->stream));
  PR_HIP(hipStreamSynchronize(g->stream));
  return PR_OK;
}

int n_hot_phases(const pr_graph *g) { return g->C > 1 ? std::max(1, g->C / kXcds) : 1; }

int set_hot_reserve(pr_graph *g, int per_xcd) {
  if (per_xcd == 0 || g->C <= 1) {
    g->hot_grid = g->hot_grid_full;
    return PR_OK;
  }
  const int grid = g->hot_grid_full - kXcds * per_xcd;
  if (per_xcd < 0 || grid < kXcds) return fail(PR_ERR_INVALID, "bad CU reserve");
  g->hot_grid = grid;
  return PR_OK;
}

constexpr int64_t kDenseUnitsPerCU = 1024;
bool hot_gather_dense(const pr_graph *g) {
  if (g->C <= 1) return false;
  if (g->hot_gather >= 0) return g->hot_gather == 1;
  return g->n_hunits >= kDenseUnitsPerCU * (int64_t)g->hot_grid_full;
}
template <bool DENSE>
void *hot_kernel(int code) {
  return code == kCodeC20    ? reinterpret_cast<void *>(k_spmv_hot<kCodeC20, DENSE>)
         : code == kCodeC24  ? reinterpret_cast<void *>(k_spmv_hot<kCodeC24, DENSE>)
         : code == kCodeC20P ? reinterpret_cast<void *>(k_spmv_hot<kCodeC20P, DENSE>)
         : code == kCodeC24P ? reinterpret_cast<void *>(k_spmv_hot<kCodeC24P, DENSE>)
                             : reinterpret_cast<void *>(k_spmv_hot<kCodeU32, DENSE>);
}

int launch_hot(pr_graph *g, int in, int ph0, int ph1) {
  if (ph1 < 0) ph1 = n_hot_phases(g);
  const CodeSrc cd{g->colh.p, g->cside.as<uint32_t>()};
  const bool dense = hot_gather_dense(g);
  auto kern = reinterpret_cast<decltype(&k_spmv_hot<kCodeU32, false>)>(dense ? hot_kernel<true>(g->code)
                                                                              : hot_kernel<false>(g->code));
  if (g->hot.lds_bytes() > (size_t)kHotLdsBytes) return fail(PR_ERR_STATE, "hot set exceeds the LDS");
  hipLaunchKernelGGL(kern, dim3((unsigned)g->hot_grid), dim3(kHotThreads), 0, g->stream,
                     g->hunits.as<Unit>(), g->hucum.as<int64_t>(), g->hot, cd, g->cbuf[in].as<double>(),
                     (uint32_t)(sizeof(double) * g->gsize), g->partial.as<double>(), g->poff.as<int64_t>(),
                     g->piece_part.as<double>(), g->hpos.as<int32_t>(), g->ptab.as<int32_t>(), ph0, ph1);
  PR_HIP(hipGetLastError());
  return PR_OK;
}

void set_exchange_chunking(pr_graph *g) { g->x_chunked = g->opts.xchg_chunks && g->n_xc > 1; }

int join_exchange(pr_graph *g) {
  if (!g->x_pending) return PR_OK;
  PR_HIP(hipStreamWaitEvent(g->stream, g->x_ev.back(), 0));
  g->x_pending = false;
  return PR_OK;
}

int iter_reset(pr_graph *g, const double *init_host) {
  hipStream_t s = g->stream;
  PR_TRY(join_exchange(g));
  DevBuf dinit;
  if (init_host && g->n_rows > 0) {
    std::vector<double> loc((size_t)g->n_rows, 0.0);
    for (int64_t L = 0; L < g->n_rows; ++L)
      if (g->orig_of_local[L] >= 0) loc[L] = init_host[g->orig_of_local[L]];
    PR_TRY(dinit.alloc(sizeof(double) * g->n_rows));
    PR_HIP(hipMemcpyAsync(dinit.p, loc.data(), sizeof(double) * g->n_rows, hipMemcpyHostToDevice, s));
    PR_HIP(hipStreamSynchronize(s));
  }
  g->cur = 0;
  g->x_packed = -1;
  if (g->x_free_ev) PR_HIP(hipEventRecord(g->x_free_ev, s));
  PR_TRY(ipc_send_runs_free(g, 0));
  const int64_t own = g->own_off;
  hipLaunchKernelGGL(k_reset, dim3(g->reset_blocks), dim3(kThreads), 0, s, g->n_rows,
                     dinit.p ? dinit.as<double>() : nullptr, g->r.as<double>(), g->rowinfo.as<uint32_t>(),
                     g->cbuf[0].as<double>() + own, g->reset_part.as<double2>());
  PR_HIP(hipGetLastError());
  PR_TRY(launch_finalize(g, 0, g->reset_part.as<double2>(), g->reset_blocks, 0, 0, s));
  if (!g->grouped) {
    PR_TRY(exchange(g, 0));
    PR_TRY(join_exchange(g));
  }
  PR_HIP(hipStreamSynchronize(s));
  g->iters_done = 0;
  g->ready = true;
  g->ev_next = 0;
  g->spmv_ev.clear();
  g->spmv_passes = 0;
  g->iter_timed = 0;
  g->iter_ev.clear();
  g->xchg_ev.clear();
  return PR_OK;
}

namespace {
int64_t epi_groups(const pr_graph *g) { return (g->nblk + kEpiGroup - 1) / kEpiGroup; }
}

int iter_compute(pr_graph *g) {
  hipStream_t s = g->stream;
  const int64_t own = g->own_off;
  const int in = g->cur, out = g->cur ^ 1;
  int open_ev = -1;
  const int hint = g->ev_start_hint;
  g->ev_start_hint = -1;
  bool enqueued = false;
  auto mark_start = [&]() -> int {
    if (!g->timing) return PR_OK;
    if (hint >= 0 && !enqueued) {
      open_ev = hint;
      enqueued = true;
      return PR_OK;
    }
    hipEvent_t e = next_event(g);
    if (!e) return fail(PR_ERR_HIP, "hipEventCreate failed");
    PR_HIP(hipEventRecord(e, s));
    open_ev = (int)g->ev_next - 1;
    return PR_OK;
  };
  auto mark_end = [&]() -> int {
    if (!g->timing) return PR_OK;
    hipEvent_t e = next_event(g);
    if (!e) return fail(PR_ERR_HIP, "hipEventCreate failed");
    PR_HIP(hipEventRecord(e, s));
    g->spmv_ev.push_back({open_ev, (int)g->ev_next - 1});
    open_ev = (int)g->ev_next - 1;
    return PR_OK;
  };
  if (g->x_free_ev) PR_HIP(hipEventRecord(g->x_free_ev, s));
  PR_TRY(ipc_send_runs_free(g, out));
  const int nph = g->C > 1 ? n_hot_phases(g) : 1;
  const bool phased_wait = g->C > 1 && g->n_hunits > 0 && g->x_pending && g->x_chunked && g->n_xc == nph && nph > 1;
  enqueued = g->nparts > 1 || g->x_free_ev != nullptr || g->x_pending;
  if (!phased_wait) PR_TRY(join_exchange(g));
  else PR_HIP(hipStreamWaitEvent(s, g->x_ev[0], 0));
  PR_TRY(mark_start());
  const double *tele = g->tele_on ? g->tele.as<double>() : nullptr;
  if (g->n_units > 0)
    hipLaunchKernelGGL((tele ? k_spmv_units<kPerThread, true, true> : k_spmv_units<kPerThread, true, false>),
                       dim3((unsigned)g->n_units), dim3(kThreads), 0, s,
                       g->units.as<Unit>(), g->rowptr.as<int64_t>(), g->colp.as<int32_t>(),
                       g->cbuf[in].as<double>(), g->cbuf[out].as<double>() + own, g->r.as<double>(),
                       g->rowinfo.as<uint32_t>(), g->piece_part.as<double>(), g->unit_part.as<double2>(),
                       g->slots, g->S_pad, (double)g->V, g->teleport, g->damping, tele);
  int64_t n_parts = g->n_units;
  if (g->C > 1) {
    if (phased_wait) {
      for (int c = 0; c < nph; ++c) {
        if (c > 0) {
          PR_TRY(mark_end());
          PR_HIP(hipStreamWaitEvent(s, g->x_ev[c], 0));
          PR_TRY(mark_start());
        }
        PR_TRY(launch_hot(g, in, c, c + 1));
      }
      g->x_pending = false;
    } else if (g->n_hunits > 0) {
      PR_TRY(launch_hot(g, in));
    }
    if (g->n_segs > 0)
      hipLaunchKernelGGL(k_seg_reduce, dim3(grid_for(g->n_segs, kThreads / kWave, 4096)), dim3(kThreads), 0, s,
                         g->n_segs, g->seg_slot.as<int64_t>(), g->seg_p0.as<int32_t>(), g->piece_part.as<double>(),
                         g->partial.as<double>());
    const EpiGrpFn epi = epi_grp_kernel(g->C, g->epi_walk, g->epi_narrow, tele != nullptr);
    PackDst pd{};
    if (g->x_fused) {
      pd.sbuf = send_runs(g, out);
      pd.P = g->nparts;
      pd.self = g->part;
      for (int q = 0; q < g->nparts; ++q) pd.soff[q] = g->x_soff[q];
    }
    const int64_t ngrp = epi_groups(g);
    const int32_t *ord = g->epi_ord.p ? g->epi_ord.as<int32_t>() + (ipc_early(g) ? ngrp : 0) : nullptr;
    auto epilogue = [&](int64_t g_lo, int64_t g_hi, unsigned grid) -> int {
      hipLaunchKernelGGL(epi, dim3(grid), dim3(epi_grp_threads(g->epi_narrow)), epi_grp_lds(g->epi_narrow), s,
                         g->nblk, g_lo, g_hi, g->partial.as<double>(), g->rmask.p, g->cbase.as<int32_t>(),
                         g->rowinfo.as<uint32_t>(), g->r.as<double>(), g->cbuf[out].as<double>() + own,
                         g->cbuf[in].as<double>(), g->slots, (double)g->V, g->teleport, g->damping,
                         g->unit_part.as<double2>() + g->n_units, g->eoff.as<int64_t>(), g->epos.as<uint16_t>(),
                         g->x_pmask.as<uint8_t>(), g->x_sbase.as<int32_t>(), ord, pd, tele);
      PR_HIP(hipGetLastError());
      return PR_OK;
    };
    if (!ipc_early(g)) {
      PR_TRY(epilogue(0, ngrp, (unsigned)g->ep_blocks));
    } else {
      const int64_t rows_per_grp = (int64_t)kEpiGroup * kWave, chunk_rows = (int64_t)kXcds * g->Q_pad;
      const int wpb = epi_grp_threads(g->epi_narrow) / kWave;
      int64_t g_lo = 0;
      for (int c = 0; c < g->n_xc; ++c) {
        const int64_t g_hi = ipc_epi_chunk_end(ngrp, c, g->n_xc, chunk_rows, rows_per_grp);
        if (g_hi > g_lo) PR_TRY(epilogue(g_lo, g_hi, grid_for(g_hi - g_lo, wpb, 1u << 20)));
        g_lo = std::max(g_lo, g_hi);
        if (c < g->n_xc - 1) PR_TRY(ipc_chunk_sent(g, out, c));
      }
    }
    n_parts += epi_groups(g);
  }
  PR_HIP(hipGetLastError());
  PR_TRY(mark_end());
  if (g->timing) ++g->spmv_passes;
  PR_TRY(launch_finalize(g, g->n_long, g->unit_part.as<double2>(), n_parts, in, out, s));
  g->x_packed = (g->x_fused && g->C > 1) ? out : -1;
  g->cur = out;
  ++g->iters_done;
  return PR_OK;
}

int iter_step(pr_graph *g, int32_t iterations) {
  if (!g->ready) return fail(PR_ERR_STATE, "pr_step before pr_reset");
  if (g->grouped) return fail(PR_ERR_STATE, "graph belongs to a group: use pr_group_step");
  if (g->timing && g->nparts == 1 && iterations > 0) {
    hipEvent_t e0 = next_event(g);
    if (!e0) return fail(PR_ERR_HIP, "hipEventCreate failed");
    PR_HIP(hipEventRecord(e0, g->stream));
    const int i0 = (int)g->ev_next - 1;
    g->timing = false;
    int rc = PR_OK;
    for (int32_t it = 0; it < iterations && rc == PR_OK; ++it) {
      rc = iter_compute(g);
      if (rc == PR_OK) rc = exchange(g, g->cur);
    }
    g->timing = true;
    PR_TRY(rc);
    hipEvent_t e1 = next_event(g);
    if (!e1) return fail(PR_ERR_HIP, "hipEventCreate failed");
    PR_HIP(hipEventRecord(e1, g->stream));
    const int i1 = (int)g->ev_next - 1;
    g->spmv_ev.push_back({i0, i1});
    g->spmv_passes += iterations;
    g->iter_ev.push_back({i0, i1});
    g->iter_timed += iterations;
    return PR_OK;
  }
  int carry = -1;
  for (int32_t it = 0; it < iterations; ++it) {
    hipEvent_t e0 = nullptr, e1 = nullptr;
    int i0 = carry;
    if (g->timing && i0 < 0) {
      e0 = next_event(g);
      if (!e0) return fail(PR_ERR_HIP, "hipEventCreate failed");
      PR_HIP(hipEventRecord(e0, g->stream));
      i0 = (int)g->ev_next - 1;
    }
    g->ev_start_hint = g->timing ? i0 : -1;
    PR_TRY(iter_compute(g));
    hipEvent_t xa = nullptr, xb = nullptr;
    if (g->timing && g->nparts > 1) {
      xa = next_event(g);
      xb = next_event(g);
      if (!xa || !xb) return fail(PR_ERR_HIP, "hipEventCreate failed");
      const int ia = (int)g->ev_next - 2;
      g->xchg_ev.push_back({ia, ia + 1});
    }
    PR_TRY(exchange(g, g->cur, xa, xb));
    if (g->timing) {
      e1 = next_event(g);
      if (!e1) return fail(PR_ERR_HIP, "hipEventCreate failed");
      PR_HIP(hipEventRecord(e1, g->stream));
      const int i1 = (int)g->ev_next - 1;
      g->iter_ev.push_back({i0, i1});
      ++g->iter_timed;
      carry = i1;
    }
  }
  return PR_OK;
}

int read_slots(pr_graph *g, int buf, double *dc, double *l1) {
  PR_TRY(join_exchange(g));
  std::vector<double> h(2 * (size_t)g->nparts);
  for (int p = 0; p < g->nparts; ++p)
    PR_HIP(hipMemcpyAsync(&h[2 * p], g->cbuf[buf].as<double>() + g->slots.pos[p], 2 * sizeof(double),
                          hipMemcpyDeviceToHost, g->stream));
  PR_HIP(hipStreamSynchronize(g->stream));
  double a = 0.0, b = 0.0;
  for (int p = 0; p < g->nparts; ++p) {
    a += h[2 * p];
    b += h[2 * p + 1];
  }
  *dc = a;
  *l1 = b;
  return PR_OK;
}

namespace {
__global__ __launch_bounds__(kThreads) void k_tele_fill(int64_t rows, double value, double *__restrict__ tele) {
  for (int64_t j = (int64_t)blockIdx.x * kThreads + threadIdx.x; j < rows; j += (int64_t)gridDim.x * kThreads)
    tele[j] = value;
}
__global__ __launch_bounds__(kThreads) void k_tele_scatter(int64_t n, const int64_t *__restrict__ rows,
                                                           const double *__restrict__ values,
                                                           double *__restrict__ tele) {
  for (int64_t i = (int64_t)blockIdx.x * kThreads + threadIdx.x; i < n; i += (int64_t)gridDim.x * kThreads)
    tele[rows[i]] = values[i];
}

int tele_quiesce(pr_graph *g) {
  PR_TRY(join_exchange(g));
  PR_HIP(hipStreamSynchronize(g->stream));
  return PR_OK;
}

int tele_ensure(pr_graph *g) {
  if (g->tele.p) return PR_OK;
  DevBuf b;
  PR_TRY(b.alloc(sizeof(double) * ((size_t)g->n_rows + 1)));
  PR_TRY(prepare_tele_kernels(g));
  g->tele = std::move(b);
  return PR_OK;
}
}

int clear_teleport(pr_graph *g) {
  PR_TRY(tele_quiesce(g));
  g->tele_on = false;
  return PR_OK;
}

int set_teleport_dense(pr_graph *g, const double *teleport) {
  PR_TRY(tele_quiesce(g));
  std::vector<double> loc((size_t)g->n_rows, 0.0);
  for (int64_t L = 0; L < g->n_rows; ++L)
    if (g->orig_of_local[L] >= 0) loc[L] = teleport[g->orig_of_local[L]];
  PR_TRY(tele_ensure(g));
  if (g->n_rows > 0) {
    PR_HIP(hipMemcpyAsync(g->tele.p, loc.data(), sizeof(double) * g->n_rows, hipMemcpyHostToDevice, g->stream));
    PR_HIP(hipStreamSynchronize(g->stream));
  }
  g->tele_on = true;
  return PR_OK;
}

int set_teleport_sparse(pr_graph *g, int32_t n, const int32_t *ids, const double *values, double rest) {
  PR_TRY(tele_quiesce(g));
  std::vector<std::pair<int32_t, int32_t>> seeds((size_t)n);
  for (int32_t i = 0; i < n; ++i) seeds[i] = {ids[i], i};
  std::sort(seeds.begin(), seeds.end());
  std::vector<int64_t> rows;
  std::vector<double> vals;
  if (n > 0)
    for (int64_t L = 0; L < g->n_rows; ++L) {
      const int32_t id = g->orig_of_local[L];
      if (id < 0) continue;
      const auto it = std::lower_bound(seeds.begin(), seeds.end(), std::make_pair(id, (int32_t)0));
      if (it == seeds.end() || it->first != id) continue;
      rows.push_back(L);
      vals.push_back(values[it->second]);
    }
  const int64_t m = (int64_t)rows.size();
  DevBuf drows, dvals;
  if (m > 0) {
    PR_TRY(drows.alloc(sizeof(int64_t) * (size_t)m));
    PR_TRY(dvals.alloc(sizeof(double) * (size_t)m));
  }
  PR_TRY(tele_ensure(g));
  hipStream_t s = g->stream;
  if (g->n_rows > 0) {
    hipLaunchKernelGGL(k_tele_fill, dim3(grid_for(g->n_rows, kThreads, 4096)), dim3(kThreads), 0, s, g->n_rows, rest,
                       g->tele.as<double>());
    PR_HIP(hipGetLastError());
  }
  if (m > 0) {
    PR_HIP(hipMemcpyAsync(drows.p, rows.data(), sizeof(int64_t) * (size_t)m, hipMemcpyHostToDevice, s));
    PR_HIP(hipMemcpyAsync(dvals.p, vals.data(), sizeof(double) * (size_t)m, hipMemcpyHostToDevice, s));
    hipLaunchKernelGGL(k_tele_scatter, dim3(grid_for(m, kThreads, 4096)), dim3(kThreads), 0, s, m, drows.as<int64_t>(),
                       dvals.as<double>(), g->tele.as<double>());
    PR_HIP(hipGetLastError());
  }
  PR_HIP(hipStreamSynchronize(s));
  g->tele_on = true;
  return PR_OK;
}

}
```

pagerank-using-apache-spark_amd/csrc/pr_spmv.h:

```cpp
#pragma once

#include <climits>

#include "pr_device.h"
#include "pr_internal.h"

namespace pr {

__device__ __forceinline__ double dc_from_slots(const double *cin, const SlotPos &sp) {
  double dc = 0.0;
  for (int p = 0; p < sp.n; ++p) dc = __dadd_rn(dc, cin[sp.pos[p]]);
  return dc;
}

__device__ __forceinline__ double affine(double S, double tdc, double teleport, double damping) {
  return __dadd_rn(teleport, __dmul_rn(damping, __dadd_rn(S, tdc)));
}

typedef int pr_v4i __attribute__((ext_vector_type(4)));
typedef int pr_v2i __attribute__((ext_vector_type(2)));
typedef pr_v4i pr_v4i_alias __attribute__((may_alias));
typedef uint32_t pr_u32_alias __attribute__((may_alias));
typedef double pr_f64_alias __attribute__((may_alias));

template <int PT, bool NT>
__device__ __forceinline__ void load_cols(const int32_t *__restrict__ p, int32_t (&ci)[PT]) {
  static_assert(PT % 4 == 0, "PT must be a multiple of 4");
  const pr_v4i *q = reinterpret_cast<const pr_v4i *>(p);
#pragma unroll
  for (int k = 0; k < PT / 4; ++k) {
    pr_v4i x;
    if constexpr (NT) x = __builtin_nontemporal_load(q + k);
    else x = q[k];
    ci[4 * k + 0] = x.x;
    ci[4 * k + 1] = x.y;
    ci[4 * k + 2] = x.z;
    ci[4 * k + 3] = x.w;
  }
}

template <int PT, bool NT, bool TELE>
__global__ __launch_bounds__(kThreads) void k_spmv_units(
    const Unit *__restrict__ units, const int64_t *__restrict__ rowptr,
    const int32_t *__restrict__ colp, const double *__restrict__ cin, double *__restrict__ cout,
    double *__restrict__ r, const uint32_t *__restrict__ rowinfo, double *__restrict__ piece_part,
    double2 *__restrict__ unit_part, SlotPos sp, int64_t S_pad, double n_vertices, double teleport,
    double damping, const double *__restrict__ tele) {
  __shared__ double rowsum[kUnitRows];
  __shared__ int32_t lrp[kUnitRows + 1];
  __shared__ double red[kThreads / kWave];
  __shared__ double2 red2[kThreads / kWave];
  __shared__ int32_t wrow_first[kThreads / kWave], wrow_last[kThreads / kWave];
  __shared__ double wval_last[kThreads / kWave];

  const int t = threadIdx.x, lane = lane_id(), w = wave_id();
  const Unit u = units[blockIdx.x];
  const int n = unit_n(u);
  const int i0 = t * PT;
  const bool stream = u.meta >= 0;
  const int nr = stream ? u.meta : 0;
  const int32_t r0 = u.r0;

  int32_t ci[PT];
  if (i0 < n) {
    load_cols<PT, NT>(colp + (int64_t)u.p8 * 8 + i0, ci);
  } else {
#pragma unroll
    for (int j = 0; j < PT; ++j) ci[j] = 0;
  }
  int64_t rp_t = 0;
  double rold0 = 0.0, tele0 = teleport;
  uint32_t info0 = 0;
  if (stream) {
    if (t <= nr) rp_t = rowptr[r0 + t];
    if (t < nr) {
      rold0 = r[(int64_t)r0 + t];
      info0 = rowinfo[(int64_t)r0 + t];
      if constexpr (TELE) tele0 = tele[(int64_t)r0 + t];
    }
  }

  double v[PT];
#pragma unroll
  for (int j = 0; j < PT; ++j) v[j] = (i0 + j < n) ? cin[ci[j]] : 0.0;

  if (!stream) {
    double acc = 0.0;
#pragma unroll
    for (int j = 0; j < PT; ++j) acc = __dadd_rn(acc, v[j]);
    acc = block_sum<kThreads>(acc, red);
    if (t == 0) {
      piece_part[-u.meta - 1] = acc;
      unit_part[blockIdx.x] = make_double2(0.0, 0.0);
    }
    return;
  }

  const int64_t e0 = rowptr[r0];
  if (t <= nr) lrp[t] = (int32_t)(rp_t - e0);
  for (int k = t + kThreads; k <= nr; k += kThreads) lrp[k] = (int32_t)(rowptr[r0 + k] - e0);
  const double tdc = dc_from_slots(cin, sp) / n_vertices;
  __syncthreads();

  int carry_row = -1, first_row = -1;
  double carry_val = 0.0, first_sum = 0.0;
  if (i0 < n) {
    int lo = 0, hi = nr + 1;
    while (lo < hi) {
      const int mid = (lo + hi) >> 1;
      if (lrp[mid] <= i0) lo = mid + 1;
      else hi = mid;
    }
    int cur = lo - 1;
    const int kstart = cur;
    const bool started_before = lrp[cur] < i0;
    int next_end = lrp[cur + 1];
    double acc = 0.0;
    bool open = false;
#pragma unroll
    for (int j = 0; j < PT; ++j) {
      if (i0 + j < n) {
        acc = __dadd_rn(acc, v[j]);
        open = true;
        if (i0 + j + 1 == next_end) {
          if (cur == kstart && started_before) {
            first_row = cur;
            first_sum = acc;
          } else {
            rowsum[cur] = acc;
          }
          acc = 0.0;
          open = false;
          ++cur;
          while (cur < nr && lrp[cur + 1] == lrp[cur]) ++cur;
          next_end = (cur < nr) ? lrp[cur + 1] : INT_MAX;
        }
      }
    }
    if (open) {
      carry_row = cur;
      carry_val = acc;
    }
  }

  int srow = carry_row;
  double sval = carry_val;
#pragma unroll
  for (int off = 1; off < kWave; off <<= 1) {
    const int prow = __shfl_up(srow, off, kWave);
    const double pval = __shfl_up(sval, off, kWave);
    if (lane >= off && srow >= 0 && prow == srow) sval = __dadd_rn(pval, sval);
  }
  const int lane0_row = __shfl(carry_row, 0, kWave);
  if (lane == kWave - 1) {
    wrow_last[w] = srow;
    wval_last[w] = sval;
    wrow_first[w] = lane0_row;
  }
  __syncthreads();
  int prow_in = -1;
  double pval_in = 0.0;
  for (int ww = 0; ww < w; ++ww) {
    const int rl = wrow_last[ww];
    const bool full = (rl >= 0) && (wrow_first[ww] == rl);
    if (full && prow_in == rl) {
      pval_in = __dadd_rn(pval_in, wval_last[ww]);
    } else {
      prow_in = rl;
      pval_in = (rl >= 0) ? wval_last[ww] : 0.0;
    }
  }
  if (srow >= 0 && srow == prow_in && lane0_row == srow) sval = __dadd_rn(pval_in, sval);
  int erow = __shfl_up(srow, 1, kWave);
  double eval = __shfl_up(sval, 1, kWave);
  if (lane == 0) {
    erow = prow_in;
    eval = pval_in;
  }
  if (first_row >= 0) rowsum[first_row] = (erow == first_row) ? __dadd_rn(eval, first_sum) : first_sum;
  __syncthreads();

  double dcp = 0.0, l1p = 0.0;
  for (int k = t; k < nr; k += kThreads) {
    const int64_t vtx = (int64_t)r0 + k;
    const double rold = (k == t) ? rold0 : r[vtx];
    const uint32_t info = (k == t) ? info0 : rowinfo[vtx];
    if (info & kRowHole) continue;
    const double S = (lrp[k + 1] > lrp[k]) ? rowsum[k] : rold;
    double tv = teleport;
    if constexpr (TELE) tv = (k == t) ? tele0 : tele[vtx];
    const double rn = affine(S, tdc, tv, damping);
    r[vtx] = rn;
    const uint32_t d = info & kRowDegMask;
    if (d > 0) cout[vtx] = __ddiv_rn(rn, (double)d);
    else if (info & kRowSink) dcp = __dadd_rn(dcp, rn);
    l1p = __dadd_rn(l1p, fabs(rn - rold));
  }
  const double2 part = block_sum2<kThreads>(make_double2(dcp, l1p), red2);
  if (t == 0) unit_part[blockIdx.x] = part;
}


template <int CTRL>
__device__ __forceinline__ double dpp_f64(double x) {
  const pr_v2i v = __builtin_bit_cast(pr_v2i, x);
  pr_v2i r;
  r.x = __builtin_amdgcn_update_dpp(0, v.x, CTRL, 0xF, 0xF, true);
  r.y = __builtin_amdgcn_update_dpp(0, v.y, CTRL, 0xF, 0xF, true);
  return __builtin_bit_cast(double, r);
}

template <int CTRL>
__device__ __forceinline__ int dpp_i32(int x) {
  return __builtin_amdgcn_update_dpp(0, x, CTRL, 0xF, 0xF, true);
}

__device__ __forceinline__ int wave_incl_scan_i32(int x) {
  const int row = lane_id() >> 4;
  x += dpp_i32<0x111>(x);
  x += dpp_i32<0x112>(x);
  x += dpp_i32<0x114>(x);
  x += dpp_i32<0x118>(x);
  int p = dpp_i32<0x142>(x);
  if (row == 1 || row == 3) x += p;
  p = dpp_i32<0x143>(x);
  if (row >= 2) x += p;
  return x;
}

__device__ __forceinline__ int wave_incl_max_i32(int x) {
  const int row = lane_id() >> 4;
  x = max(x, dpp_i32<0x111>(x));
  x = max(x, dpp_i32<0x112>(x));
  x = max(x, dpp_i32<0x114>(x));
  x = max(x, dpp_i32<0x118>(x));
  int p = dpp_i32<0x142>(x);
  if (row == 1 || row == 3) x = max(x, p);
  p = dpp_i32<0x143>(x);
  if (row >= 2) x = max(x, p);
  return x;
}

struct WaveCodes {
  uint32_t c[kWavePT];
};

__device__ __forceinline__ void wave_unit_codes(const Unit &u, const uint32_t *__restrict__ colh, WaveCodes &w) {
  const __amdgpu_buffer_rsrc_t rs =
      __builtin_amdgcn_make_buffer_rsrc((void *)(colh + (int64_t)u.p8 * 8), 0, u.n * 4, 0x00020000);
  const int base = lane_id() * kWavePT * 4;
#pragma unroll
  for (int q = 0; q < kWavePT / 4; ++q) {
    const pr_v4i x = __builtin_bit_cast(pr_v4i, __builtin_amdgcn_raw_buffer_load_b128(rs, base + 16 * q, 0, 2));
    w.c[4 * q + 0] = (uint32_t)x.x;
    w.c[4 * q + 1] = (uint32_t)x.y;
    w.c[4 * q + 2] = (uint32_t)x.z;
    w.c[4 * q + 3] = (uint32_t)x.w;
  }
}

struct WaveCodesC20 {
  uint32_t w[kWavePT / 2];
  uint32_t s;
};
__device__ __forceinline__ void wave_unit_codes(const Unit &u, const uint16_t *__restrict__ code16,
                                                const uint32_t *__restrict__ cside, WaveCodesC20 &w) {
  const __amdgpu_buffer_rsrc_t rm =
      __builtin_amdgcn_make_buffer_rsrc((void *)(code16 + (int64_t)u.p8 * 8), 0, u.n * 2, 0x00020000);
  const __amdgpu_buffer_rsrc_t rsd =
      __builtin_amdgcn_make_buffer_rsrc((void *)(cside + (int64_t)u.p8), 0, u.n / 2, 0x00020000);
  const pr_v4i x = __builtin_bit_cast(pr_v4i, __builtin_amdgcn_raw_buffer_load_b128(rm, lane_id() * 16, 0, 2));
  w.w[0] = (uint32_t)x.x;
  w.w[1] = (uint32_t)x.y;
  w.w[2] = (uint32_t)x.z;
  w.w[3] = (uint32_t)x.w;
  w.s = __builtin_amdgcn_raw_buffer_load_b32(rsd, lane_id() * 4, 0, 2);
}

struct WaveCodesC24 {
  uint32_t w[kWavePT / 2];
  uint64_t s;
};
__device__ __forceinline__ void wave_unit_codes(const Unit &u, const uint16_t *__restrict__ code16,
                                                const uint64_t *__restrict__ cside, WaveCodesC24 &w) {
  const __amdgpu_buffer_rsrc_t rm =
      __builtin_amdgcn_make_buffer_rsrc((void *)(code16 + (int64_t)u.p8 * 8), 0, u.n * 2, 0x00020000);
  const __amdgpu_buffer_rsrc_t rsd =
      __builtin_amdgcn_make_buffer_rsrc((void *)(cside + (int64_t)u.p8), 0, u.n, 0x00020000);
  const pr_v4i x = __builtin_bit_cast(pr_v4i, __builtin_amdgcn_raw_buffer_load_b128(rm, lane_id() * 16, 0, 2));
  w.w[0] = (uint32_t)x.x;
  w.w[1] = (uint32_t)x.y;
  w.w[2] = (uint32_t)x.z;
  w.w[3] = (uint32_t)x.w;
  w.s = __builtin_bit_cast(uint64_t, __builtin_amdgcn_raw_buffer_load_b64(rsd, lane_id() * 8, 0, 2));
}

__device__ __forceinline__ uint32_t end_marks(const WaveCodes &w) {
  uint32_t endm = 0;
#pragma unroll
  for (int j = 0; j < kWavePT; ++j) endm |= (w.c[j] & 1u) << j;
  return endm;
}
__device__ __forceinline__ uint32_t end_marks(const WaveCodesC20 &w) { return w.s & 0xFFu; }
__device__ __forceinline__ uint32_t end_marks(const WaveCodesC24 &w) { return (uint32_t)w.s & 0xFFu; }

struct LaneMeta {
  uint32_t endm;
// ... 196 lines not shown

__device__ __forceinline__ void stage_segment_sums(const LaneMeta &m, const double (&sv)[kWavePT], double carry,
                                                   int base, double *stage) {
  int e = m.excl - base;
#pragma unroll
  for (int j = 0; j < kWavePT; ++j) {
    const bool end = (m.endm >> j) & 1u;
    if (end && e >= 0 && e < kStageSlots) stage[e] = sv[j];
    e += end ? 1 : 0;
  }
  const int e0 = m.excl - base;
  if (m.endm != 0u && e0 >= 0 && e0 < kStageSlots) stage[e0] = __dadd_rn(carry, stage[e0]);
}


struct UnitSums {
  LaneMeta m;
  double sv[kWavePT];
  double carry;
};

template <class WC>
__device__ __forceinline__ bool wave_unit_sums(const Unit &u, const WC &w, const double (&v)[kWavePT],
                                               double *__restrict__ piece_part, UnitSums &r) {
  if (u.meta < 0) {
    double acc = 0.0;
#pragma unroll
    for (int j = 0; j < kWavePT; ++j) acc = __dadd_rn(acc, v[j]);
    acc = wave_sum(acc);
    if (lane_id() == 0) piece_part[-u.meta - 1] = acc;
    return false;
  }
  r.m = derive_meta(end_marks(w));
  wave_segmented_sums(r.m, v, r.sv, &r.carry);
  return true;
}

__device__ __forceinline__ void wave_unit_store(const Unit &u, const UnitSums &r, double *pcls, double *stage) {
  const int nseg = u.meta;
  static_assert(kStageSlots <= 2 * kWave, "one b128 pass");
  const __amdgpu_buffer_rsrc_t urs =
      __builtin_amdgcn_make_buffer_rsrc((void *)(pcls + u.r0), 0, (uint32_t)nseg * 8u, 0x00020000);
  for (int base = 0; base < nseg; base += kStageSlots) {
    stage_segment_sums(r.m, r.sv, r.carry, base, stage);
    const int n = min(kStageSlots, nseg - base);
    const int i2 = 2 * lane_id();
#if PR_HOT_DIAG == 4 || PR_HOT_DIAG == 6
    if (u.r0 != 0x7FFFFFFF) continue;
#endif
    if (i2 < n)
      __builtin_amdgcn_raw_buffer_store_b128(*reinterpret_cast<const pr_v4i_alias *>(stage + i2), urs,
                                             (uint32_t)(base + i2) * 8u, 0, 2);
  }
}

struct CodeSrc {
  const void *codes;
  const uint32_t *side;
};
template <int CODE>
struct CodeOf {
  using T = WaveCodes;
};
template <>
struct CodeOf<kCodeC20> {
  using T = WaveCodesC20;
};
template <>
struct CodeOf<kCodeC24> {
  using T = WaveCodesC24;
};
template <>
struct CodeOf<kCodeC20P> {
  using T = WaveCodesC20;
};
template <>
struct CodeOf<kCodeC24P> {
  using T = WaveCodesC24;
};
template <int CODE>
__device__ __forceinline__ void unit_codes(const Unit &u, const CodeSrc &cd, typename CodeOf<CODE>::T &w) {
  if constexpr (CODE == kCodeC20 || CODE == kCodeC20P)
    wave_unit_codes(u, static_cast<const uint16_t *>(cd.codes), cd.side, w);
  else if constexpr (CODE == kCodeC24 || CODE == kCodeC24P)
    wave_unit_codes(u, static_cast<const uint16_t *>(cd.codes), reinterpret_cast<const uint64_t *>(cd.side), w);
  else wave_unit_codes(u, static_cast<const uint32_t *>(cd.codes), w);
}

template <int CODE, bool DENSE>
__device__ __forceinline__ void unit_gather(const typename CodeOf<CODE>::T &w, const double *hot, const ClassSrc &cs,
                                            double (&v)[kWavePT], double *win) {
  if constexpr (DENSE && (!PR_HOT_DIAG || PR_HOT_DIAG == 7)) {
    wave_unit_gather_compact<code_is_piece(CODE)>(w, hot, cs, v, win);
  } else {
    (void)win;
    wave_unit_gather<code_is_piece(CODE)>(w, hot, cs, v);
  }
}

template <int CODE, bool DENSE>
__device__ __forceinline__ void hot_class_units(int x, int team, int nteams, const Unit *__restrict__ units,
                                                const int64_t *__restrict__ ucum, const HotGeom &hg,
                                                const CodeSrc &cd, const double *hot, const ClassSrc &cs,
                                                double *__restrict__ partial, const int64_t *__restrict__ poff,
                                                double *__restrict__ piece_part, double *stage) {
  const int64_t p0 = poff[x];
  const int64_t beg = ucum[x], end = ucum[x + 1];
  constexpr int kWaves = kHotThreads / kWave;
  team = (team + 5 * (x / kXcds)) % nteams;
  const int64_t stride = (int64_t)nteams * kWaves;
  uint32_t *ctr = reinterpret_cast<uint32_t *>(const_cast<double *>(hot) + hg.ctr_slot());
  const int lane = lane_id();
  auto counter = [&]() -> uint32_t {
    uint32_t t = 0;
    if (lane == 0) t = atomicAdd(ctr, 1u);
    return (uint32_t)__builtin_amdgcn_readlane((int)t, 0);
  };
  auto take = [&]() -> int64_t {
    const uint32_t t = counter();
    return beg + (int64_t)team * kWaves + (int64_t)(t % kWaves) + (int64_t)(t / kWaves) * stride;
  };
  int64_t k = take();
  if (k >= end) return;
  const __attribute__((address_space(4))) pr_v4i *cu = (const __attribute__((address_space(4))) pr_v4i *)units;
  auto unit_at = [&](int64_t i) -> Unit {
    const pr_v4i q = cu[i];
    return Unit{(uint32_t)q.x, q.y, q.z, q.w};
  };
  const int64_t none_k = ucum[kMaxClasses];
  Unit u[3];
  typename CodeOf<CODE>::T wc[3];
  double v[3][kWavePT];
  int64_t k1 = take();
  u[0] = unit_at(k);
  unit_codes<CODE>(u[0], cd, wc[0]);
  u[1] = unit_at(k1 < end ? k1 : none_k);
  unit_codes<CODE>(u[1], cd, wc[1]);
  unit_gather<CODE, DENSE>(wc[0], hot, cs, v[0], stage);
  while (true) {
#pragma unroll
    for (int sl = 0; sl < 3; ++sl) {
      const int s1 = (sl + 1) % 3, s2 = (sl + 2) % 3;
      const int64_t k2 = take();
      u[s2] = unit_at(k2 < end ? k2 : none_k);
      unit_codes<CODE>(u[s2], cd, wc[s2]);
#if PR_HOT_DIAG == 7
      {
        uint32_t d = (uint32_t)lane;
#pragma unroll
        for (int q = 0; q < 64; ++q) asm volatile("v_add_u32 %0, %0, %1" : "+v"(d) : "v"((uint32_t)q));
        if (d == 0xFFFFFFFFu) piece_part[0] = 0.0;
      }
#endif
      UnitSums us;
      const bool stream = wave_unit_sums(u[sl], wc[sl], v[sl], piece_part, us);
      if (stream) wave_unit_store(u[sl], us, partial + p0, stage);
      unit_gather<CODE, DENSE>(wc[s1], hot, cs, v[s1], stage);
      k = k1;
      k1 = k2;
      if (k >= end) return;
    }
  }
}

template <bool PIECE, bool CONTIG = false>
__device__ __forceinline__ void stage_hot_set(const HotGeom &hg, int x, const int32_t *__restrict__ hpos,
                                              const int32_t *__restrict__ ptab, const double *__restrict__ cin,
                                              double *hot, uint32_t *tblw) {
  const int nh = hg.P * hg.Kp;
  const int32_t *hp = hpos + (int64_t)x * nh;
  const double *reg = cin + (int64_t)x * hg.Q_pad;
  const bool load = PR_HOT_DIAG != 5 || x < kXcds;
  constexpr int kSB = 6;
  for (int b0 = 0; load && b0 < nh; b0 += kSB * kHotThreads) {
    int32_t pos[kSB];
    double val[kSB];
    if constexpr (CONTIG) {
#pragma unroll
      for (int j = 0; j < kSB; ++j) {
        const int i = b0 + (int)threadIdx.x + j * kHotThreads;
        val[j] = i < hg.q_load ? reg[i] : 0.0;
      }
    } else {
#pragma unroll
      for (int j = 0; j < kSB; ++j) {
        const int i = b0 + (int)threadIdx.x + j * kHotThreads;
        pos[j] = i < nh ? hp[i] : -1;
      }
#pragma unroll
      for (int j = 0; j < kSB; ++j) val[j] = pos[j] >= 0 ? cin[pos[j]] : 0.0;
    }
#pragma unroll
    for (int j = 0; j < kSB; ++j) {
      const int i = b0 + (int)threadIdx.x + j * kHotThreads;
      if (i < nh) hot[1 + i] = val[j];
    }
  }
  if constexpr (PIECE)
    for (int i = (int)threadIdx.x; i < kPieceTblWords; i += kHotThreads)
      tblw[i] = (uint32_t)ptab[(int64_t)x * kPieceTblWords + i];
  if (threadIdx.x == 0) {
    hot[0] = 0.0;
    hot[hg.slots()] = 0.0;
    *reinterpret_cast<uint32_t *>(hot + hg.ctr_slot()) = 0u;
  }
}

template <int CODE, bool DENSE>
__global__ __launch_bounds__(kHotThreads) void k_spmv_hot(const Unit *__restrict__ units,
                                                          const int64_t *__restrict__ ucum, HotGeom hg,
                                                          CodeSrc cd, const double *__restrict__ cin,
                                                          uint32_t cin_bytes, double *__restrict__ partial,
                                                          const int64_t *__restrict__ poff,
                                                          double *__restrict__ piece_part,
                                                          const int32_t *__restrict__ hpos,
                                                          const int32_t *__restrict__ ptab, int ph0, int ph1) {
  __shared__ double hot[kHotLdsBytes / sizeof(double)];
  constexpr bool kPiece = code_is_piece(CODE);
  ClassSrc cs;
  cs.zb = (uint32_t)hg.slots() * 8u;
  cs.hb = kPiece ? cs.zb : (uint32_t)(hg.q_load + 1) * 8u;
  uint32_t *tblw = reinterpret_cast<uint32_t *>(hot + hg.tbl_off());
  cs.tbl = tblw;
  if constexpr (CODE == kCodeU32 || kPiece)
    cs.crs = __builtin_amdgcn_make_buffer_rsrc((void *)cin, 0, cin_bytes, 0x00020000);
  const int wv = __builtin_amdgcn_readfirstlane(wave_id());
  double *stage = hot + hg.stage_off() + wv * kStageSlots;
  const int team = (int)(blockIdx.x / kXcds), nteams = (int)(gridDim.x / kXcds);
  for (int ph = ph0; ph < ph1; ++ph) {
    const int x = (int)(blockIdx.x % kXcds) + kXcds * ph;
    if constexpr (CODE == kCodeC20 || CODE == kCodeC24) {
      const int64_t first = (int64_t)x * hg.Q_pad + hg.q_load;
      cs.crs = __builtin_amdgcn_make_buffer_rsrc((void *)(cin + first), 0,
                                                 (uint32_t)((hg.Q_pad - hg.q_load) * 8), 0x00020000);
    }
    if (ph > ph0) __syncthreads();
    stage_hot_set<kPiece, CODE == kCodeC20 || CODE == kCodeC24>(hg, x, hpos, ptab, cin, hot, tblw);
    __syncthreads();
    hot_class_units<CODE, DENSE>(x, team, nteams, units, ucum, hg, cd, hot, cs, partial, poff, piece_part, stage);
  }
}

__global__ __launch_bounds__(kThreads) void k_seg_reduce(int64_t n_seg, const int64_t *__restrict__ seg_slot,
                                                         const int32_t *__restrict__ seg_p0,
                                                         const double *__restrict__ piece_part,
                                                         double *__restrict__ partial) {
  const int lane = lane_id();
  const int64_t nw = (int64_t)gridDim.x * (kThreads / kWave);
  for (int64_t q = (int64_t)blockIdx.x * (kThreads / kWave) + wave_id(); q < n_seg; q += nw) {
    const int32_t p0 = seg_p0[q], np = seg_p0[q + 1] - p0;
    double acc = 0.0;
    for (int k = lane; k < np; k += kWave) acc = __dadd_rn(acc, piece_part[p0 + k]);
    acc = wave_sum(acc);
    if (lane == 0) partial[seg_slot[q]] = acc;
  }
}

template <int G>
__device__ __forceinline__ int epi_class_add(const uint32_t (&mw)[G], uint32_t bit, int run, const double *win,
                                             int zslot, double (&S)[G]) {
  double v[G];
#pragma unroll
  for (int g = 0; g < G; ++g) {
    const bool has = (mw[g] & bit) != 0u;
    const unsigned long long bal = __ballot(has);
    const int idx = (int)__builtin_amdgcn_mbcnt_hi((uint32_t)(bal >> 32),
                                                   __builtin_amdgcn_mbcnt_lo((uint32_t)bal, (uint32_t)run));
    v[g] = win[has ? idx : zslot];
    run += __popcll(bal);
  }
#pragma unroll
  for (int g = 0; g < G; ++g) S[g] = __dadd_rn(S[g], v[g]);
  return run;
}

template <int C, int W>
__device__ __forceinline__ int walk_batch_end(int x0, int incl, int pre, int sincl, int spre) {
  static_assert(W >= 64 * kEpiGroup + 2 + 2 * 8 * kEpiGroup, "one class and its positions fit the window");
  const int lane = lane_id();
  const int base = __builtin_amdgcn_readlane(pre, x0), sbase = __builtin_amdgcn_readlane(spre, x0);
  const int need = (incl - base) + 2 * ((sincl - sbase + 7) >> 3);
  const unsigned long long over = __ballot(lane >= x0 && lane < C && need > W);
  return over ? (int)__builtin_ctzll(over) : C;
}
__device__ __forceinline__ uint64_t class_range_mask(int x0, int x1) {
  const uint64_t hi = x1 >= 64 ? ~0ull : ((1ull << x1) - 1ull);
  return hi & ~((1ull << x0) - 1ull);
}


struct EpiArgs {
  int64_t nblk;
  const double *partial;
  const void *rmask;
  const int32_t *cbase;
  const uint32_t *rowinfo;
  double *r, *cout;
  double teleport, damping;
  const int64_t *eoff;
  const uint16_t *epos;
  const uint8_t *pmask;
  const int32_t *sbase;
  const double *tele;
};

#ifndef PR_EPI_DMA_AUX
#define PR_EPI_DMA_AUX 0
#endif
#ifndef PR_EPI_LATE_ROW
#define PR_EPI_LATE_ROW 0
#endif
#ifndef PR_EPI_TELE_EARLY
#define PR_EPI_TELE_EARLY 0
#endif

template <int C, bool WALK, bool TELE>
__device__ __forceinline__ void epi_group(const EpiArgs &a, const PackDst &pd, int64_t gi, double tdc, double *win,
                                          double2 *__restrict__ ep_part) {
  double dcp = 0.0, l1p = 0.0;
  constexpr int G = kEpiGroup, W = kEpiWin;
  constexpr int MW = mask_words<C>();
  static_assert(MW == 1 || MW == 2 || MW == 4, "mask words");
  static_assert(W >= 64 * G + 2, "one class run of a group must fit the window");
  static_assert(!WALK || C <= kWave, "the per-row walk needs at most 64 classes");
  const int lane = lane_id();
  const int64_t b0 = gi * G;
  const int nb = (int)min((int64_t)G, a.nblk - b0);
  uint32_t mw[MW][G], info[G];
  double rold[G], S[G];
  double tv[G];
  double cnv[G];
  uint32_t pmv[G];
#pragma unroll
  for (int g = 0; g < G; ++g) pmv[g] = (pd.P > 1 && g < nb) ? a.pmask[(b0 + g) * kWave + lane] : 0u;
#pragma unroll
  for (int g = 0; g < G; ++g) {
    const int64_t L = (b0 + g) * kWave + lane;
    const bool ok = g < nb;
    if constexpr (MW == 4) {
      const uint4 q = ok ? static_cast<const uint4 *>(a.rmask)[L] : make_uint4(0u, 0u, 0u, 0u);
      mw[0][g] = q.x, mw[1][g] = q.y, mw[2][g] = q.z, mw[3][g] = q.w;
    } else if constexpr (MW == 2) {
      const uint2 q = ok ? static_cast<const uint2 *>(a.rmask)[L] : make_uint2(0u, 0u);
      mw[0][g] = q.x, mw[1][g] = q.y;
    } else {
      mw[0][g] = ok ? static_cast<const uint32_t *>(a.rmask)[L] : 0u;
    }
#if !PR_EPI_LATE_ROW
    info[g] = ok ? a.rowinfo[L] : kRowHole;
    rold[g] = ok ? a.r[L] : 0.0;
#endif
#if PR_EPI_TELE_EARLY
    if constexpr (TELE) tv[g] = ok ? a.tele[L] : 0.0;
#endif
    S[g] = 0.0;
  }
  const int cs = lane < C ? a.cbase[b0 * C + lane] : 0;
  const int ce = lane < C ? a.cbase[(b0 + nb) * C + lane] : 0;
  if constexpr (C <= kWave) {
    const int sa = cs & ~1;
    const int n2 = (lane < C && ce > cs) ? (((ce + 1) & ~1) - sa) : 0;
    const int incl = wave_incl_scan_i32(n2);
    const int pre = incl - n2;
    const int roff = incl - n2 + (cs - sa);
    bool walked = false;
    if constexpr (WALK) {
      const int64_t eo = a.eoff[gi];
      if (eo >= 0) {
        const int nsl = lane < C ? ce - cs : 0;
        const int sincl = wave_incl_scan_i32(nsl);
        for (int y = 0; y < C; ++y) {
          const int n = __builtin_amdgcn_readlane(n2, y);
          if (n == 0) continue;
          const double *src = a.partial + __builtin_amdgcn_readlane(sa, y);
          double *dst = win + __builtin_amdgcn_readlane(pre, y);
          for (int o = 0; o < n; o += 2 * kWave)
            if (o + 2 * lane < n) __builtin_amdgcn_global_load_lds(src + o + 2 * lane, dst + o, 16, 0, PR_EPI_DMA_AUX);
        }
        const int Tb = __builtin_amdgcn_readlane(incl, C - 1);
        const int nl = (__builtin_amdgcn_readlane(sincl, C - 1) + 7) >> 3;
        const double *esrc = reinterpret_cast<const double *>(a.epos + eo);
        for (int o = 0; o < nl; o += kWave)
          if (o + lane < nl) __builtin_amdgcn_global_load_lds(esrc + 2 * (o + lane), win + Tb + 2 * o, 16, 0, PR_EPI_DMA_AUX);
        __builtin_amdgcn_s_waitcnt(0);
        const uint16_t *ep = reinterpret_cast<const uint16_t *>(win + Tb);
        int acc = 0;
#pragma unroll
        for (int g = 0; g < G; ++g) {
          const uint64_t m = (uint64_t)(MW > 1 ? mw[MW > 1 ? 1 : 0][g] : 0u) << 32 | mw[0][g];
          const int cnt = __popcll(m);
          const int inc = wave_incl_scan_i32(cnt);
          const uint16_t *e = ep + acc + inc - cnt;
          acc += __builtin_amdgcn_readlane(inc, kWave - 1);
          for (int k = 0; __ballot(k < cnt) != 0ull; ++k)
            if (k < cnt) S[g] = __dadd_rn(S[g], win[e[k]]);
        }
        __builtin_amdgcn_s_waitcnt(0);
        walked = true;
      }
    }
    for (int x0 = 0; x0 < C && !walked;) {
      const int base = __builtin_amdgcn_readlane(pre, x0);
      const unsigned long long over = __ballot(lane >= x0 && lane < C && incl - base > W);
      const int x1 = over ? (int)__builtin_ctzll(over) : C;
      for (int y = x0; y < x1; ++y) {
        const int n = __builtin_amdgcn_readlane(n2, y);
        if (n == 0) continue;
        const double *src = a.partial + __builtin_amdgcn_readlane(sa, y);
        double *dst = win + (__builtin_amdgcn_readlane(pre, y) - base);
        for (int o = 0; o < n; o += 2 * kWave)
          if (o + 2 * lane < n) __builtin_amdgcn_global_load_lds(src + o + 2 * lane, dst + o, 16, 0, PR_EPI_DMA_AUX);
      }
      __builtin_amdgcn_s_waitcnt(0);
      for (int y = x0; y < x1; ++y) {
        if (__builtin_amdgcn_readlane(n2, y) == 0) continue;
        const uint32_t bit = 1u << (y & 31);
        const int run = __builtin_amdgcn_readlane(roff, y) - base;
        if (MW == 1 || y < 32) epi_class_add<G>(mw[0], bit, run, win, W, S);
        else epi_class_add<G>(mw[MW > 1 ? 1 : 0], bit, run, win, W, S);
      }
      __builtin_amdgcn_s_waitcnt(0);
      x0 = x1;
    }
  } else {
    const int cs1 = lane + kWave < C ? a.cbase[b0 * C + kWave + lane] : 0;
    const int ce1 = lane + kWave < C ? a.cbase[(b0 + nb) * C + kWave + lane] : 0;
    auto run_start = [&](int y) {
      return y < kWave ? __builtin_amdgcn_readlane(cs, y) : __builtin_amdgcn_readlane(cs1, y - kWave);
    };
    auto run_end = [&](int y) {
      return y < kWave ? __builtin_amdgcn_readlane(ce, y) : __builtin_amdgcn_readlane(ce1, y - kWave);
    };
    for (int x = 0; x < C;) {
      int fill = 0, xe = x;
      for (; xe < C; ++xe) {
        const int s = run_start(xe), e = run_end(xe);
        if (e == s) continue;
        const int sa = s & ~1, n2 = ((e + 1) & ~1) - sa;
        if (xe > x && fill + n2 > W) break;
        const double *src = a.partial + sa;
        for (int o = 0; o < n2; o += 2 * kWave)
          if (o + 2 * lane < n2) __builtin_amdgcn_global_load_lds(src + o + 2 * lane, win + fill + o, 16, 0, PR_EPI_DMA_AUX);
        fill += n2;
      }
      __builtin_amdgcn_s_waitcnt(0);
      fill = 0;
      for (int y = x; y < xe; ++y) {
        const int s = run_start(y), e = run_end(y);
        if (e == s) continue;
        const int sa = s & ~1;
        const uint32_t bit = 1u << (y & 31);
        const int run = fill + (s - sa);
        if (y < 32) epi_class_add<G>(mw[0], bit, run, win, W, S);
        else if (y < 64) epi_class_add<G>(mw[MW > 1 ? 1 : 0], bit, run, win, W, S);
        else if (y < 96) epi_class_add<G>(mw[MW > 2 ? 2 : 0], bit, run, win, W, S);
        else epi_class_add<G>(mw[MW > 3 ? 3 : 0], bit, run, win, W, S);
        fill += ((e + 1) & ~1) - sa;
      }
      __builtin_amdgcn_s_waitcnt(0);
      x = xe;
    }
  }
#if PR_EPI_LATE_ROW
#pragma unroll
  for (int g = 0; g < G; ++g) {
    const int64_t L = (b0 + g) * kWave + lane;
    const bool ok = g < nb;
    info[g] = ok ? a.rowinfo[L] : kRowHole;
    rold[g] = ok ? a.r[L] : 0.0;
  }
#endif
#pragma unroll
  for (int g = 0; g < G; ++g) {
    const int64_t L = (b0 + g) * kWave + lane;
    if constexpr (!TELE) tv[g] = a.teleport;
#if !PR_EPI_TELE_EARLY
    else tv[g] = g < nb ? a.tele[L] : 0.0;
#endif
    double Sv = S[g];
    uint32_t any = 0u;
#pragma unroll
    for (int w = 0; w < MW; ++w) any |= mw[w][g];
    if (any == 0u) Sv = rold[g];
    const double rn = affine(Sv, tdc, tv[g], a.damping);
    double cn = 0.0;
    if (!(info[g] & kRowHole)) {
      a.r[L] = rn;
      const uint32_t d = info[g] & kRowDegMask;
      if (d > 0) {
        cn = __ddiv_rn(rn, (double)d);
        a.cout[L] = cn;
      } else if (info[g] & kRowSink) {
        dcp = __dadd_rn(dcp, rn);
      }
      l1p = __dadd_rn(l1p, fabs(rn - rold[g]));
    }
    cnv[g] = cn;
  }
  static_assert(G * kWave <= W, "a group's run for one peer fits the window");
  if (pd.P > 1) {
    const int64_t sb0 = b0 * pd.P;
    for (int q = 0; q < pd.P; ++q) {
      int run = 0;
#pragma unroll
      for (int g = 0; g < G; ++g) {
        const bool has = (pmv[g] >> q) & 1u;
        const unsigned long long bal = __ballot(has);
        const int k = (int)__builtin_amdgcn_mbcnt_hi((uint32_t)(bal >> 32), __builtin_amdgcn_mbcnt_lo((uint32_t)bal, (uint32_t)run));
        if (has) win[k] = cnv[g];
        run += __popcll(bal);
      }
      if (run == 0) continue;
      const __amdgpu_buffer_rsrc_t rs = __builtin_amdgcn_make_buffer_rsrc(
          (void *)(pd.sbuf + pd.soff[q] + a.sbase[sb0 + q]), 0, (uint32_t)run * 8u, 0x00020000);
      for (int o = 0; o < run; o += 2 * kWave) {
        const int i = o + 2 * lane;
        if (i < run)
          __builtin_amdgcn_raw_buffer_store_b128(*reinterpret_cast<const pr_v4i_alias *>(win + i), rs, (uint32_t)i * 8u, 0, 0);
      }
    }
  }
  dcp = wave_sum(dcp);
  l1p = wave_sum(l1p);
  if (lane == 0) ep_part[gi] = make_double2(dcp, l1p);
}

#ifndef PR_EPI_WAVES
#define PR_EPI_WAVES 0
#endif
#if PR_EPI_WAVES > 0
#define PR_EPI_BOUNDS(NT) __attribute__((amdgpu_flat_work_group_size(NT, NT), amdgpu_waves_per_eu(PR_EPI_WAVES)))
#else
#define PR_EPI_BOUNDS(NT) __launch_bounds__(NT, 4)
#endif
template <int C, bool WALK, int NT, bool TELE>
__global__ PR_EPI_BOUNDS(NT) void k_epilogue_grp(
    int64_t nblk, int64_t g_lo, int64_t g_hi, const double *__restrict__ partial, const void *__restrict__ rmask_v,
    const int32_t *__restrict__ cbase, const uint32_t *__restrict__ rowinfo, double *__restrict__ r,
    double *__restrict__ cout, const double *__restrict__ cin, SlotPos sp, double n_vertices, double teleport,
    double damping, double2 *__restrict__ ep_part , const int64_t *__restrict__ eoff,
    const uint16_t *__restrict__ epos, const uint8_t *__restrict__ pmask, const int32_t *__restrict__ sbase,
    const int32_t *__restrict__ order, PackDst pd, const double *__restrict__ tele) {
  constexpr int W = kEpiWin;
  constexpr int NW = NT / kWave;
  extern __shared__ double epi_lds[];
  const EpiArgs a{nblk, partial, rmask_v, cbase, rowinfo, r, cout, teleport, damping, eoff, epos, pmask, sbase, tele};
  const int lane = lane_id();
  const int wv = __builtin_amdgcn_readfirstlane(wave_id());
  double *win = epi_lds + wv * (W + 2);
  if (lane == 0) win[W] = 0.0;
  const double tdc = dc_from_slots(cin, sp) / n_vertices;
  const int64_t nw = (int64_t)gridDim.x * NW;
  for (int64_t k = g_lo + (int64_t)blockIdx.x * NW + wv; k < g_hi; k += nw)
    epi_group<C, WALK, TELE>(a, pd, order ? (int64_t)order[k] : k, tdc, win, ep_part);
}

template <int C, bool COUNT>
__global__ __launch_bounds__(kEpiThreads) void k_epi_walk_plan(int64_t nblk, const void *__restrict__ rmask_v,
                                                               const int32_t *__restrict__ cbase,
                                                               int64_t *__restrict__ eoff,
                                                               uint16_t *__restrict__ epos) {
  static_assert(C <= kWave, "per-row walk: at most 64 classes");
  constexpr int G = kEpiGroup, W = kEpiWin;
  constexpr int MW = mask_words<C>();
  const int lane = lane_id();
  const int64_t ngrp = (nblk + G - 1) / G;
  const int64_t nw = (int64_t)gridDim.x * (kEpiThreads / kWave);
  for (int64_t gi = (int64_t)blockIdx.x * (kEpiThreads / kWave) + wave_id(); gi < ngrp; gi += nw) {
    int64_t ebase = 0;
    if constexpr (!COUNT) {
      ebase = eoff[gi];
      if (ebase < 0) continue;
    }
    const int64_t b0 = gi * G;
    const int nb = (int)min((int64_t)G, nblk - b0);
    uint64_t m[G];
#pragma unroll
    for (int g = 0; g < G; ++g) {
      const int64_t L = (b0 + g) * kWave + lane;
      if (g >= nb) m[g] = 0;
      else if constexpr (MW == 2) m[g] = static_cast<const uint64_t *>(rmask_v)[L];
      else m[g] = static_cast<const uint32_t *>(rmask_v)[L];
    }
    const int cs = lane < C ? cbase[b0 * C + lane] : 0;
    const int ce = lane < C ? cbase[(b0 + nb) * C + lane] : 0;
    const int sa = cs & ~1;
    const int n2 = (lane < C && ce > cs) ? (((ce + 1) & ~1) - sa) : 0;
    const int incl = wave_incl_scan_i32(n2);
    const int pre = incl - n2;
    const int roff = pre + (cs - sa);
    const int nsl = lane < C ? ce - cs : 0;
    const int sincl = wave_incl_scan_i32(nsl);
    const int spre = sincl - nsl;
    const int x1 = walk_batch_end<C, W>(0, incl, pre, sincl, spre);
    const int nl = (__builtin_amdgcn_readlane(sincl, x1 - 1) + 7) >> 3;
    if constexpr (COUNT) {
      if (lane == 0) eoff[gi] = x1 == C ? 8 * (int64_t)nl : -1;
    } else {
      int pref[G], acc = 0;
#pragma unroll
      for (int g = 0; g < G; ++g) {
        const int cnt = __popcll(m[g]);
        const int inc = wave_incl_scan_i32(cnt);
        pref[g] = acc + inc - cnt;
        acc += __builtin_amdgcn_readlane(inc, kWave - 1);
      }
      for (int x = 0; x < C; ++x) {
        int run = __builtin_amdgcn_readlane(roff, x);
#pragma unroll
        for (int g = 0; g < G; ++g) {
          const bool has = (m[g] >> x) & 1ull;
          const unsigned long long bal = __ballot(has);
          if (has) {
            const int k = __popcll(m[g] & ((1ull << x) - 1ull));
            epos[ebase + pref[g] + k] = (uint16_t)__builtin_amdgcn_mbcnt_hi(
                (uint32_t)(bal >> 32), __builtin_amdgcn_mbcnt_lo((uint32_t)bal, (uint32_t)run));
          }
          run += __popcll(bal);
        }
      }
    }
  }
}

using EpiGrpFn = void (*)(int64_t, int64_t, int64_t, const double *, const void *, const int32_t *, const uint32_t *, double *,
                          double *, const double *, SlotPos, double, double, double, double2 *, const int64_t *,
                          const uint16_t *, const uint8_t *, const int32_t *, const int32_t *, PackDst, const double *);
template <int C, bool TELE>
inline EpiGrpFn epi_grp_kernel_c(bool walk, bool narrow) {
  if constexpr (C <= kWave) {
    if (narrow)
      return walk ? k_epilogue_grp<C, true, kEpiThreadsNarrow, TELE> : k_epilogue_grp<C, false, kEpiThreadsNarrow, TELE>;
    if (walk) return k_epilogue_grp<C, true, kEpiThreads, TELE>;
  }
  return k_epilogue_grp<C, false, kEpiThreads, TELE>;
}
template <bool TELE>
inline EpiGrpFn epi_grp_kernel_t(int C, bool walk, bool narrow) {
  switch (C) {
    case 8: return epi_grp_kernel_c<8, TELE>(walk, narrow);
    case 16: return epi_grp_kernel_c<16, TELE>(walk, narrow);
    case 32: return epi_grp_kernel_c<32, TELE>(walk, narrow);
    case 64: return epi_grp_kernel_c<64, TELE>(walk, narrow);
    default: return epi_grp_kernel_c<128, TELE>(false, false);
  }
}
inline EpiGrpFn epi_grp_kernel(int C, bool walk, bool narrow, bool tele = false) {
  return tele ? epi_grp_kernel_t<true>(C, walk, narrow) : epi_grp_kernel_t<false>(C, walk, narrow);
}

}
```

pagerank-using-apache-spark_amd/sparky_hip/_lib.py:

```python
from __future__ import annotations

import ctypes
import os
import sys

_PKG_DIR = os.path.dirname(os.path.abspath(__file__))
BUILD_DIR = os.path.join(os.path.dirname(_PKG_DIR), "build")
LIB_PATH = os.environ.get("PR_LIB_PATH") or os.path.join(BUILD_DIR, "libpagerank_hip.so")

ABI_VERSION = 2

PR_OK = 0
PR_ERR_INVALID = -1
PR_ERR_HIP = -2
PR_ERR_OOM = -3
PR_ERR_COMM = -4
PR_ERR_STATE = -5
PR_ERR_NODEVICE = -6

PR_DANGLING_LOCAL = 0
PR_DANGLING_NONE = 1
PR_INPUT_DEVICE = 2
PR_NO_CANONICAL = 4
PR_LAYOUT_FUSED = 8
PR_LAYOUT_SPLIT = 16

PR_VF_KEY, PR_VF_SINK, PR_VF_NOLINK, PR_VF_INDEG0 = 1, 2, 4, 8

INFO_NAMES = ["n_vertices", "n_edges", "n_sink", "n_nolink", "n_indeg0", "max_indeg", "local_rows",
              "local_edges", "part", "n_parts", "n_units", "n_long_rows", "device_bytes", "classes",
              "xchg_send", "xchg_recv", "partial_slots", "hot_slots", "epilogue", "gather_est",
              "walk_groups", "layout", "hot_cover_ppm", "code_bits", "hot_gather"]
BUILD_OPTIONS = {"classes": 1, "hot_slots": 2, "exchange_allgather": 3, "xchg_chunks": 4, "hot_reserve": 5,
                 "epi_walk": 6, "epi_narrow": 7, "codes": 8, "pack_fused": 9, "xchg_sdma": 10,
                 "epi_order": 11}
STAT_NAMES = ["iters", "last_dc", "last_l1", "spmv_ms_mean", "spmv_launches", "iter_ms_mean",
              "build_ms", "exchange_ms_mean"]
PR_CB_RANKS = 1
PR_OPT_XCHG_CHUNKS = 1
PR_OPT_HOT_RESERVE = 2
PR_OPT_XCHG_IPC = 3
PR_OPT_XCHG_IPC_BLIT = 4
PR_OPT_HOT_GATHER = 5
PR_COMM_ID_BYTES = 128

EXPORTED = [
    "pr_abi_version", "pr_last_error", "pr_device_count", "pr_graph_create", "pr_graph_create_part",
    "pr_graph_create_ex",
    "pr_graph_info", "pr_graph_export_csr", "pr_run", "pr_reset", "pr_step", "pr_sync",
    "pr_get_ranks", "pr_set_timing", "pr_set_option", "pr_get_stats", "pr_comm_unique_id", "pr_graph_attach_comm",
    "pr_graph_destroy", "pr_gen_rmat", "pr_gen_er", "pr_gen_chunglu", "pr_intern_device", "pr_group_reset",
    "pr_group_step", "pr_group_sync", "pr_get_topk", "pr_group_topk", "pr_topk_merge",
    "pr_set_teleport", "pr_set_teleport_sparse",
    "pr_batch_create", "pr_batch_set_teleport", "pr_batch_set_teleport_sparse", "pr_batch_reset", "pr_batch_step",
    "pr_batch_sync", "pr_batch_get_ranks", "pr_batch_get_norms", "pr_batch_get_topk", "pr_batch_info",
    "pr_batch_destroy", "pr_batch_set_exclude", "pr_batch_get_topk_all", "pr_batch_step_until",
    "pr_batch_reset_column", "pr_batch_step_until_any", "pr_batch_run_queue",
    "pr_batch_set_dangling", "pr_batch_get_dangling", "pr_batch_get_teleport_sums",
]
BATCH_INFO_NAMES = ["width", "stride", "n_units", "n_long_rows", "device_bytes", "iters", "last_step_ns"]
BATCH_MAX_WIDTH = 16
PR_BATCH_DANGLING_UNIFORM = 0
PR_BATCH_DANGLING_TELEPORT = 1
BATCH_DANGLING_MODES = {"uniform": PR_BATCH_DANGLING_UNIFORM, "teleport": PR_BATCH_DANGLING_TELEPORT}

ITER_CB = ctypes.CFUNCTYPE(None, ctypes.c_int32, ctypes.POINTER(ctypes.c_double), ctypes.c_double,
                           ctypes.c_double, ctypes.c_double, ctypes.c_void_p)


class BatchQuery(ctypes.Structure):
    _fields_ = [("n_seeds", ctypes.c_int32), ("ids", ctypes.c_void_p), ("values", ctypes.c_void_p),
                ("rest", ctypes.c_double), ("n_exclude", ctypes.c_int32), ("exclude", ctypes.c_void_p)]


BATCH_DONE_CB = ctypes.CFUNCTYPE(None, ctypes.c_int32, ctypes.c_int32, ctypes.c_int32, ctypes.c_int32, ctypes.c_double,
                                 ctypes.c_void_p)


class PageRankError(RuntimeError):

    def __init__(self, code: int, msg: str):
        super().__init__(f"libpagerank_hip error {code}: {msg}")
        self.code = code


_lib = None
OPTIONAL = set()


def load() -> ctypes.CDLL:
    global _lib
    if _lib is not None:
        return _lib
    if "torch" not in sys.modules:
        try:
            import torch
        except ImportError:
            pass
    if not os.path.exists(LIB_PATH):
        raise FileNotFoundError(
            f"{LIB_PATH} is missing: build it with `make -C pagerank-using-apache-spark_amd/csrc` "
            "or `python -c 'import __graft_entry__ as g; g.build()'`")
    L = ctypes.CDLL(LIB_PATH)
    P = ctypes.c_void_p
    i32, i64, u32, u64, dbl = ctypes.c_int32, ctypes.c_int64, ctypes.c_uint32, ctypes.c_uint64, ctypes.c_double
    sig = {
        "pr_abi_version": ([], ctypes.c_int),
        "pr_last_error": ([], ctypes.c_char_p),
        "pr_device_count": ([P], ctypes.c_int),
        "pr_graph_create": ([i32, i32, i64, P, P, u32, P], ctypes.c_int),
        "pr_graph_create_part": ([i32, i32, i32, i32, i64, P, P, u32, P], ctypes.c_int),
        "pr_graph_create_ex": ([i32, i32, i32, i32, i64, P, P, u32, P, i32, P], ctypes.c_int),
        "pr_graph_info": ([P, P, i32], ctypes.c_int),
        "pr_graph_export_csr": ([P, P, P, P, P], ctypes.c_int),
        "pr_run": ([P, i32, dbl, dbl, P, P, ITER_CB, u32, P], ctypes.c_int),
        "pr_reset": ([P, dbl, dbl, P], ctypes.c_int),
        "pr_step": ([P, i32], ctypes.c_int),
        "pr_sync": ([P], ctypes.c_int),
        "pr_get_ranks": ([P, P], ctypes.c_int),
        "pr_set_timing": ([P, i32], ctypes.c_int),
        "pr_set_option": ([P, i32, i64], ctypes.c_int),
        "pr_get_stats": ([P, P, i32], ctypes.c_int),
        "pr_comm_unique_id": ([P], ctypes.c_int),
        "pr_graph_attach_comm": ([P, i32, i32, P], ctypes.c_int),
        "pr_graph_destroy": ([P], None),
        "pr_gen_rmat": ([i32, i32, i64, dbl, dbl, dbl, u64, P, P], ctypes.c_int),
        "pr_gen_er": ([i32, i32, i64, u64, P, P], ctypes.c_int),
        "pr_gen_chunglu": ([i32, i32, i64, dbl, dbl, dbl, dbl, dbl, i64, u64, P, P], ctypes.c_int),
        "pr_intern_device": ([i32, i64, i32, P, P, P], ctypes.c_int),
        "pr_group_reset": ([P, i32, dbl, dbl, P], ctypes.c_int),
        "pr_group_step": ([P, i32, i32], ctypes.c_int),
        "pr_group_sync": ([P, i32], ctypes.c_int),
        "pr_get_topk": ([P, i32, P, P, P], ctypes.c_int),
        "pr_group_topk": ([P, i32, i32, P, P, P], ctypes.c_int),
        "pr_topk_merge": ([i32, P, P, P, i32, P, P, P], ctypes.c_int),
        "pr_set_teleport": ([P, P], ctypes.c_int),
        "pr_set_teleport_sparse": ([P, i32, P, P, dbl], ctypes.c_int),
        "pr_batch_create": ([P, i32, P], ctypes.c_int),
        "pr_batch_set_teleport": ([P, i32, P], ctypes.c_int),
        "pr_batch_set_teleport_sparse": ([P, i32, i32, P, P, dbl], ctypes.c_int),
        "pr_batch_reset": ([P, dbl, dbl, P], ctypes.c_int),
        "pr_batch_step": ([P, i32], ctypes.c_int),
        "pr_batch_sync": ([P], ctypes.c_int),
        "pr_batch_get_ranks": ([P, i32, P], ctypes.c_int),
        "pr_batch_get_norms": ([P, P, P], ctypes.c_int),
        "pr_batch_get_topk": ([P, i32, i32, P, P, P], ctypes.c_int),
        "pr_batch_info": ([P, P, i32], ctypes.c_int),
        "pr_batch_destroy": ([P], None),
        "pr_batch_set_exclude": ([P, i32, i32, P], ctypes.c_int),
        "pr_batch_get_topk_all": ([P, i32, P, P, P], ctypes.c_int),
        "pr_batch_step_until": ([P, i32, dbl, P], ctypes.c_int),
        "pr_topk_select_ex": ([P, i32, i64, P, P, P, P], ctypes.c_int),
        "pr_batch_topk_all_ex": ([P, i32, i64, P, P, P, P], ctypes.c_int),
        "pr_batch_topk_all_kernel_ns": ([P, P], ctypes.c_int),
        "pr_batch_step_until_ex": ([P, i32, dbl, i32, P, P], ctypes.c_int),
        "pr_batch_reset_column": ([P, i32, P], ctypes.c_int),
        "pr_batch_step_until_any": ([P, u32, i32, dbl, P, P], ctypes.c_int),
        "pr_batch_run_queue": ([P, i32, P, i32, dbl, P, P, P], ctypes.c_int),
        "pr_batch_step_until_any_ex": ([P, u32, i32, dbl, i32, P, P, P], ctypes.c_int),
        "pr_batch_set_dangling": ([P, i32], ctypes.c_int),
        "pr_batch_get_dangling": ([P, P], ctypes.c_int),
        "pr_batch_get_teleport_sums": ([P, P], ctypes.c_int),
        "pr_batch_get_ranks_ex": ([P, i32, P], ctypes.c_int),
    }
    for name, (args, res) in sig.items():
        if name in OPTIONAL and not hasattr(L, name):
            continue
        fn = getattr(L, name)
        fn.argtypes = args
        fn.restype = res
    v = L.pr_abi_version()
    if v != ABI_VERSION:
        raise ImportError(f"{LIB_PATH} has ABI version {v}; this binding needs {ABI_VERSION} (rebuild the library)")
    _lib = L
    return L


def check(rc: int) -> None:
    if rc != PR_OK:
        msg = load().pr_last_error()
        raise PageRankError(rc, msg.decode() if msg else "")
```

pagerank-using-apache-spark_amd/sparky_hip/graph.py:

```python
from __future__ import annotations

import ctypes
from dataclasses import dataclass
from typing import Callable, List, Optional

import numpy as np

from . import _lib
from ._lib import check


def _ptr(a: Optional[np.ndarray]):
    return None if a is None else ctypes.c_void_p(a.ctypes.data)


@dataclass
class CanonicalCSR:
    row_ptr: np.ndarray
    col_idx: np.ndarray
    out_deg: np.ndarray
    vflags: np.ndarray


@dataclass
class IterationStats:
    iteration: int
    dangling_sum: float
    l1_delta: float
    ms: float


def _init_array(init_ranks, n_vertices: int):
    if init_ranks is None:
        return None
    init = np.ascontiguousarray(init_ranks, dtype=np.float64)
    if init.shape != (n_vertices,):
        raise ValueError(f"init_ranks must have shape ({n_vertices},), got {init.shape}")
    return init


def _teleport_array(teleport, n_vertices: int):
    if teleport is None:
        return None
    t = np.ascontiguousarray(teleport, dtype=np.float64)
    if t.shape != (n_vertices,):
        raise ValueError(f"teleport must have shape ({n_vertices},), got {t.shape}")
    return t


def _sparse_arrays(ids, values):
    i = np.ascontiguousarray(ids, dtype=np.int32)
    v = np.ascontiguousarray(values, dtype=np.float64)
    if i.ndim != 1 or i.shape != v.shape:
        raise ValueError("ids and values must be 1-D arrays of the same length")
    return i, v


def device_count() -> int:
    n = ctypes.c_int32(0)
    check(_lib.load().pr_device_count(ctypes.byref(n)))
    return n.value


class PageRankGraph:

    def __init__(self, n_vertices: int, src, dst, *, device: int = 0, dangling: str = "local",
                 part: int = 0, n_parts: int = 1, keep_canonical: bool = True,
                 device_input: bool = False, n_edges: Optional[int] = None, layout: str = "auto",
                 options: Optional[dict] = None):
        L = _lib.load()
        flags = 0
        if dangling == "none":
            flags |= _lib.PR_DANGLING_NONE
        elif dangling != "local":
            raise ValueError("dangling must be 'local' or 'none'")
        if not keep_canonical:
            flags |= _lib.PR_NO_CANONICAL
        if layout == "fused":
            flags |= _lib.PR_LAYOUT_FUSED
        elif layout == "split":
            flags |= _lib.PR_LAYOUT_SPLIT
        elif layout != "auto":
            raise ValueError("layout must be 'auto', 'fused' or 'split'")
        if device_input:
            flags |= _lib.PR_INPUT_DEVICE
            if n_edges is None:
                raise ValueError("n_edges is required with device_input=True")
            ps, pd = ctypes.c_void_p(int(src)), ctypes.c_void_p(int(dst))
            ne = int(n_edges)
        else:
            src = np.ascontiguousarray(src, dtype=np.int32)
            dst = np.ascontiguousarray(dst, dtype=np.int32)
            if src.shape != dst.shape:
                raise ValueError("src and dst must have the same length")
            ps, pd = _ptr(src), _ptr(dst)
            ne = int(src.shape[0])
        self._h = ctypes.c_void_p()
        opts = options or {}
        unknown = set(opts) - set(_lib.BUILD_OPTIONS)
        if unknown:
            raise ValueError(f"unknown build options {sorted(unknown)}")
        kv = np.array([x for k, v in opts.items() for x in (_lib.BUILD_OPTIONS[k], int(v))], np.int64)
        if opts:
            rc = L.pr_graph_create_ex(device, part, n_parts, int(n_vertices), ne, ps, pd, flags, _ptr(kv), len(opts),
                                      ctypes.byref(self._h))
        elif n_parts == 1 and part == 0:
            rc = L.pr_graph_create(device, int(n_vertices), ne, ps, pd, flags, ctypes.byref(self._h))
        else:
            rc = L.pr_graph_create_part(device, part, n_parts, int(n_vertices), ne, ps, pd, flags,
                                        ctypes.byref(self._h))
        check(rc)
        self.n_vertices = int(n_vertices)
        self.part, self.n_parts = part, n_parts

    def close(self) -> None:
        if getattr(self, "_h", None) and self._h.value:
            _lib.load().pr_graph_destroy(self._h)
            self._h = ctypes.c_void_p()

    def __del__(self):
        try:
            self.close()
        except Exception:
            pass

    def __enter__(self):
        return self

    def __exit__(self, *exc):
        self.close()

    def info(self) -> dict:
        a = np.zeros(len(_lib.INFO_NAMES), np.int64)
        check(_lib.load().pr_graph_info(self._h, _ptr(a), len(a)))
        return dict(zip(_lib.INFO_NAMES, (int(x) for x in a)))

    def export_csr(self) -> CanonicalCSR:
        inf = self.info()
        V, E = inf["n_vertices"], inf["n_edges"]
        rp = np.zeros(V + 1, np.int64)
        col = np.zeros(max(E, 1), np.int32)
        deg = np.zeros(max(V, 1), np.int32)
        vf = np.zeros(max(V, 1), np.uint8)
        check(_lib.load().pr_graph_export_csr(self._h, _ptr(rp), _ptr(col), _ptr(deg), _ptr(vf)))
        return CanonicalCSR(rp, col[:E], deg[:V], vf[:V])

    def stats(self) -> dict:
        a = np.zeros(len(_lib.STAT_NAMES), np.float64)
        check(_lib.load().pr_get_stats(self._h, _ptr(a), len(a)))
        return dict(zip(_lib.STAT_NAMES, (float(x) for x in a)))

    def run(self, iterations: int = 10, *, teleport: float = 0.15, damping: float = 0.85,
            init_ranks=None, callback: Optional[Callable] = None, want_ranks_in_callback: bool = False):
        V = self.n_vertices
        out = np.zeros(max(V, 1), np.float64)
        init = _init_array(init_ranks, V)
        history: List[IterationStats] = []
        errors: List[BaseException] = []

        def _cb(it, rp, dc, l1, ms, _user):
            st = IterationStats(int(it), float(dc), float(l1), float(ms))
            history.append(st)
            if callback is not None and not errors:
                try:
                    arr = np.ctypeslib.as_array(rp, shape=(V,)).copy() if rp else None
                    callback(int(it), arr, st)
                except BaseException as e:
                    errors.append(e)

        cb = _lib.ITER_CB(_cb)
        flags = _lib.PR_CB_RANKS if want_ranks_in_callback else 0
        check(_lib.load().pr_run(self._h, int(iterations), teleport, damping, _ptr(init), _ptr(out),
                                 cb, flags, None))
        if errors:
            raise errors[0]
        return out[:V], history

    def reset(self, *, teleport: float = 0.15, damping: float = 0.85, init_ranks=None) -> None:
        init = _init_array(init_ranks, self.n_vertices)
        check(_lib.load().pr_reset(self._h, teleport, damping, _ptr(init)))

    def step(self, iterations: int) -> None:
        check(_lib.load().pr_step(self._h, int(iterations)))

    def sync(self) -> None:
        check(_lib.load().pr_sync(self._h))

    def ranks(self, out: Optional[np.ndarray] = None) -> np.ndarray:
        if out is None:
            out = np.zeros(max(self.n_vertices, 1), np.float64)
        check(_lib.load().pr_get_ranks(self._h, _ptr(out)))
        return out[: self.n_vertices]

    def set_teleport(self, teleport) -> None:
        t = _teleport_array(teleport, self.n_vertices)
        check(_lib.load().pr_set_teleport(self._h, _ptr(t)))

    def set_teleport_sparse(self, ids, values, rest: float = 0.0) -> None:
        i, v = _sparse_arrays(ids, values)
        check(_lib.load().pr_set_teleport_sparse(self._h, int(i.shape[0]), _ptr(i), _ptr(v), float(rest)))

    def topk(self, k: int):
        k = int(k)
        ids, rk = np.zeros(max(k, 1), np.int32), np.zeros(max(k, 1), np.float64)
        n = ctypes.c_int32(0)
        check(_lib.load().pr_get_topk(self._h, k, _ptr(ids), _ptr(rk), ctypes.byref(n)))
        return ids[: n.value], rk[: n.value]

    def _topk_ex(self, k: int, narrow_div: int):
        k = int(k)
        ids, rk = np.zeros(max(k, 1), np.int32), np.zeros(max(k, 1), np.float64)
        n = ctypes.c_int32(0)
        info = np.zeros(4, np.int32)
        check(_lib.load().pr_topk_select_ex(self._h, k, int(narrow_div), _ptr(ids), _ptr(rk), ctypes.byref(n),
                                            _ptr(info)))
        return ids[: n.value], rk[: n.value], dict(zip(("passes", "row_passes", "cand_passes", "narrowed_at"),
                                                       (int(x) for x in info)))

    def set_timing(self, enable: bool) -> None:
        check(_lib.load().pr_set_timing(self._h, 1 if enable else 0))

    def set_exchange_chunks(self, on: bool) -> None:
        check(_lib.load().pr_set_option(self._h, _lib.PR_OPT_XCHG_CHUNKS, 1 if on else 0))

    def set_hot_reserve(self, cus_per_xcd: int) -> None:
        check(_lib.load().pr_set_option(self._h, _lib.PR_OPT_HOT_RESERVE, int(cus_per_xcd)))

    def set_hot_gather(self, mode: int) -> None:
        check(_lib.load().pr_set_option(self._h, _lib.PR_OPT_HOT_GATHER, int(mode)))

    def set_exchange_ipc(self, mode) -> None:
        v = int(mode)
        if v not in (0, 1, 2):
            raise ValueError("exchange ipc mode must be 0, 1 or 2")
        check(_lib.load().pr_set_option(self._h, _lib.PR_OPT_XCHG_IPC, v))

    def set_exchange_ipc_blit(self, on: bool) -> None:
        check(_lib.load().pr_set_option(self._h, _lib.PR_OPT_XCHG_IPC_BLIT, 1 if on else 0))

    def attach_comm(self, rank: int, n_ranks: int, uid: bytes) -> None:
        buf = (ctypes.c_uint8 * _lib.PR_COMM_ID_BYTES).from_buffer_copy(uid)
        check(_lib.load().pr_graph_attach_comm(self._h, rank, n_ranks, buf))


def merge_topk(lists, k: int):
    k = int(k)
    lists = [(np.ascontiguousarray(i, dtype=np.int32), np.ascontiguousarray(r, dtype=np.float64)) for i, r in lists]
    for i, r in lists:
        if i.shape != r.shape or i.ndim != 1:
            raise ValueError("every list is a pair of 1-D arrays of the same length")
    n_l = len(lists)
    pid = (ctypes.c_void_p * max(n_l, 1))(*[i.ctypes.data for i, _ in lists])
    prk = (ctypes.c_void_p * max(n_l, 1))(*[r.ctypes.data for _, r in lists])
    cnt = np.array([i.shape[0] for i, _ in lists] or [0], np.int32)
    ids, rk = np.zeros(max(k, 1), np.int32), np.zeros(max(k, 1), np.float64)
    n = ctypes.c_int32(0)
    check(_lib.load().pr_topk_merge(n_l, pid, prk, _ptr(cnt), k, _ptr(ids), _ptr(rk), ctypes.byref(n)))
    return ids[: n.value], rk[: n.value]


def comm_unique_id() -> bytes:
    buf = (ctypes.c_uint8 * _lib.PR_COMM_ID_BYTES)()
    check(_lib.load().pr_comm_unique_id(buf))
    return bytes(buf)


def gen_rmat(device: int, scale: int, n_edges: int, src_ptr: int, dst_ptr: int, *, a=0.57, b=0.19,
             c=0.19, seed: int = 1) -> None:
    check(_lib.load().pr_gen_rmat(device, scale, n_edges, a, b, c, seed, ctypes.c_void_p(src_ptr),
                                  ctypes.c_void_p(dst_ptr)))


CHUNGLU_PRESETS = {
    "lj": dict(n_labels=4_847_571, n_edges=68_993_773, gamma_out=2.3, v0_out=84.0, gamma_in=2.3, v0_in=84.0,
               src_frac=1.0, n_nolink=0, seed=4),
    "twitter": dict(n_labels=41_652_230, n_edges=1_468_365_182, gamma_out=2.2, v0_out=100.0, gamma_in=2.1,
                    v0_in=50.0, src_frac=0.85, n_nolink=2_082_611, seed=5),
}


def gen_chunglu(device: int, n_labels: int, n_edges: int, src_ptr: int, dst_ptr: int, *, gamma_out: float,
                v0_out: float, gamma_in: float, v0_in: float, src_frac: float = 1.0, n_nolink: int = 0,
                seed: int = 4) -> None:
    check(_lib.load().pr_gen_chunglu(device, n_labels, n_edges, gamma_out, v0_out, gamma_in, v0_in, src_frac,
                                     n_nolink, seed, ctypes.c_void_p(src_ptr), ctypes.c_void_p(dst_ptr)))


def gen_er(device: int, scale: int, n_edges: int, src_ptr: int, dst_ptr: int, *, seed: int = 3) -> None:
    check(_lib.load().pr_gen_er(device, scale, n_edges, seed, ctypes.c_void_p(src_ptr),
                                ctypes.c_void_p(dst_ptr)))


def intern_device(device: int, n_edges: int, label_bound: int, src_ptr: int, dst_ptr: int) -> int:
    nv = ctypes.c_int32(0)
    check(_lib.load().pr_intern_device(device, n_edges, label_bound, ctypes.c_void_p(src_ptr),
                                       ctypes.c_void_p(dst_ptr), ctypes.byref(nv)))
    return nv.value


class PartGroup:

    def __init__(self, parts):
        self.parts = list(parts)
        n = len(self.parts)
        self._arr = (ctypes.c_void_p * n)(*[p._h.value for p in self.parts])

    def reset(self, *, teleport=0.15, damping=0.85, init_ranks=None):
        init = _init_array(init_ranks, self.parts[0].n_vertices)
        check(_lib.load().pr_group_reset(self._arr, len(self.parts), teleport, damping, _ptr(init)))

    def step(self, iterations: int):
        check(_lib.load().pr_group_step(self._arr, len(self.parts), int(iterations)))

    def sync(self):
        check(_lib.load().pr_group_sync(self._arr, len(self.parts)))

    def ranks(self) -> np.ndarray:
        V = self.parts[0].n_vertices
        out = np.full(max(V, 1), np.nan)
        for p in self.parts:
            p.ranks(out)
        return out[:V]

    def set_teleport(self, teleport) -> None:
        t = _teleport_array(teleport, self.parts[0].n_vertices)
        for p in self.parts:
            p.set_teleport(t)

    def set_teleport_sparse(self, ids, values, rest: float = 0.0) -> None:
        i, v = _sparse_arrays(ids, values)
        for p in self.parts:
            p.set_teleport_sparse(i, v, rest)

    def topk(self, k: int):
        k = int(k)
        ids, rk = np.zeros(max(k, 1), np.int32), np.zeros(max(k, 1), np.float64)
        n = ctypes.c_int32(0)
        check(_lib.load().pr_group_topk(self._arr, len(self.parts), k, _ptr(ids), _ptr(rk), ctypes.byref(n)))
        return ids[: n.value], rk[: n.value]

    def run(self, iterations: int, **kw) -> np.ndarray:
        self.reset(**kw)
        self.step(iterations)
        self.sync()
        return self.ranks()
```

Measured before the change: 384.9.

## Elide full rank write-back in mid-batch epilogues using packed in-degree-zero ranks

Adds a mid-batch epilogue variant that skips writing the full rank vector on iterations other than the last two of a multi-iteration step. Ranks of rows with no in-links are packed once into a compact r0 array so the epilogue can still recover them, and the rank array is written again on the second-to-last iteration. The aim is to cut HBM write traffic in the epilogue for large graphs (enabled by group-count threshold). In exchange it adds a pack kernel per step, extra build-time planning with a host sync, and more kernel variants.

Result: slower. 376.4 (-2.2%).

```diff
diff --git a/include/pagerank_hip.h b/include/pagerank_hip.h
--- a/include/pagerank_hip.h
+++ b/include/pagerank_hip.h
@@ -54,7 +54,10 @@
 #define PR_INFO_HOT_COVER 22
 #define PR_INFO_CODE_BITS 23
 #define PR_INFO_HOT_GATHER 24
-#define PR_INFO_COUNT 25
+#define PR_INFO_IN0_ROWS 25
+#define PR_INFO_IN0_EMPTY_BLOCKS 26
+#define PR_INFO_IN0_FULL_BLOCKS 27
+#define PR_INFO_COUNT 28
 
 #define PR_STAT_ITERS 0
 #define PR_STAT_LAST_DC 1
@@ -94,6 +97,7 @@
 #define PR_BOPT_PACK_FUSED 9
 #define PR_BOPT_XCHG_SDMA 10
 #define PR_BOPT_EPI_ORDER 11
+#define PR_BOPT_EPI_ELIDE 12
 int pr_graph_create_ex(int32_t device, int32_t part, int32_t n_parts, int32_t n_vertices, int64_t n_edges,
                        const int32_t *src, const int32_t *dst, uint32_t flags, const int64_t *options,
                        int32_t n_options, pr_graph **out);
@@ -126,6 +130,7 @@
 #define PR_OPT_XCHG_IPC 3
 #define PR_OPT_XCHG_IPC_BLIT 4
 #define PR_OPT_HOT_GATHER 5
+#define PR_OPT_EPI_ELIDE 6
 int pr_set_option(pr_graph *g, int32_t option, int64_t value);
 
 #define PR_COMM_ID_BYTES 128
diff --git a/java/src/sparky/hip/PageRankHip.java b/java/src/sparky/hip/PageRankHip.java
--- a/java/src/sparky/hip/PageRankHip.java
+++ b/java/src/sparky/hip/PageRankHip.java
@@ -17,7 +17,7 @@
 public final class PageRankHip implements AutoCloseable {
     public static final int PR_DANGLING_LOCAL = 0, PR_DANGLING_NONE = 1, PR_NO_CANONICAL = 4;
     static final int PR_CB_RANKS = 1;
-    static final int PR_INFO_COUNT = 25;
+    static final int PR_INFO_COUNT = 28;
     public static final int ABI_VERSION = 2;
 
     private static final Linker LINKER = Linker.nativeLinker();
diff --git a/pagerank-using-apache-spark_amd/csrc/pr_api.hip b/pagerank-using-apache-spark_amd/csrc/pr_api.hip
--- a/pagerank-using-apache-spark_amd/csrc/pr_api.hip
+++ b/pagerank-using-apache-spark_amd/csrc/pr_api.hip
@@ -45,7 +45,7 @@
 
 size_t pr_graph::device_bytes() const {
   size_t b = canon_rowptr.bytes + canon_col.bytes + canon_deg.bytes + canon_vflags.bytes;
-  b += rowptr.bytes + col.bytes + colp.bytes + rowinfo.bytes + colh.bytes + hunits.bytes + partial.bytes + poff.bytes + rmask.bytes + cbase.bytes + seg_slot.bytes + seg_p0.bytes + r.bytes + cbuf[0].bytes + cbuf[1].bytes + eoff.bytes + epos.bytes;
+  b += rowptr.bytes + col.bytes + colp.bytes + rowinfo.bytes + colh.bytes + hunits.bytes + partial.bytes + poff.bytes + rmask.bytes + cbase.bytes + seg_slot.bytes + seg_p0.bytes + r.bytes + cbuf[0].bytes + cbuf[1].bytes + eoff.bytes + epos.bytes + in0_base.bytes + r0.bytes;
   b += units.bytes + unit_part.bytes + lr_row.bytes + lr_p0.bytes + piece_part.bytes;
   b += fin_part.bytes + fin_counter.bytes + reset_part.bytes + x_send.bytes + x_sbuf.bytes + hpos.bytes + cside.bytes;
   b += pr::topk_bytes(this);
@@ -130,6 +130,10 @@
           return fail(PR_ERR_INVALID, "PR_BOPT_EPI_ORDER: -1 (auto), 0 (row order), 1 (runs of 8 groups heaviest first), "
                                       "2 (groups heaviest first)");
         o->epi_order = (int)v;
+        break;
+      case PR_BOPT_EPI_ELIDE:
+        if (v < -1 || v > 1) return fail(PR_ERR_INVALID, "PR_BOPT_EPI_ELIDE: -1 (by size), 0 (the full epilogue every iteration) or 1 (elide mid-batch)");
+        o->epi_elide = (int)v;
         break;
       default:
         return fail(PR_ERR_INVALID, "unknown build option " + std::to_string(k));
@@ -231,7 +235,7 @@
                                     g->C > 1 ? (int64_t)g->hot.P * g->hot.Kp : 0,
                                     g->C == 1 ? 0 : 3, g->gather_est, g->n_walk_groups, g->layout,
                                     g->hot_cover_ppm, g->C > 1 ? (g->code == pr::kCodeC20 || g->code == pr::kCodeC20P ? 20 : g->code == pr::kCodeC24 || g->code == pr::kCodeC24P ? 24 : 32) : 0,
-                                    pr::hot_gather_dense(g) ? 1 : 0};
+                                    pr::hot_gather_dense(g) ? 1 : 0, g->n_in0, g->n_in0_empty, g->n_in0_full};
   for (int32_t i = 0; i < n_info && i < PR_INFO_COUNT; ++i) info[i] = v[i];
   return PR_OK;
 }
@@ -335,6 +339,11 @@
   if (option == PR_OPT_HOT_GATHER) {
     if (value < -1 || value > 1) return fail(PR_ERR_INVALID, "PR_OPT_HOT_GATHER: -1 (auto), 0 (per position) or 1 (dense)");
     if (g->C > 1) g->hot_gather = (int)value;
+    return PR_OK;
+  }
+  if (option == PR_OPT_EPI_ELIDE) {
+    if (value < -1 || value > 1) return fail(PR_ERR_INVALID, "PR_OPT_EPI_ELIDE: -1 (by size), 0 (the full epilogue every iteration) or 1 (elide mid-batch)");
+    g->epi_elide = (int)value;
     return PR_OK;
   }
   if (option == PR_OPT_XCHG_IPC_BLIT) {
@@ -533,9 +542,12 @@
   std::vector<int> i0((size_t)n_parts, -1);
   for (int32_t it = 0; it < iterations; ++it) {
     for (int32_t p = 0; p < n_parts; ++p) {
-      PR_HIP(hipSetDevice(parts[p]->device));
-      if (parts[p]->timing) PR_TRY(pr::time_mark(parts[p], parts[p]->stream, &i0[p]));
-      PR_TRY(pr::iter_compute(parts[p]));
+      pr_graph *g = parts[p];
+      PR_HIP(hipSetDevice(g->device));
+      const bool elide = pr::iter_elides(g, iterations);
+      if (it == 0 && elide) PR_TRY(pr::iter_pack_in0(g));
+      if (g->timing) PR_TRY(pr::time_mark(g, g->stream, &i0[p]));
+      PR_TRY(pr::iter_compute(g, pr::epi_mode(it, iterations, elide)));
     }
     PR_TRY(pr::group_exchange(parts, n_parts, parts[0]->cur));
     for (int32_t p = 0; p < n_parts; ++p) {
diff --git a/pagerank-using-apache-spark_amd/csrc/pr_build.hip b/pagerank-using-apache-spark_amd/csrc/pr_build.hip
--- a/pagerank-using-apache-spark_amd/csrc/pr_build.hip
+++ b/pagerank-using-apache-spark_amd/csrc/pr_build.hip
@@ -870,7 +870,9 @@
     g->epi_narrow = epi_narrow_ok(C) && (g->opts.epi_narrow < 0 ? auto_narrow : g->opts.epi_narrow != 0);
     g->ep_blocks = (int)grid_for(ngrp, epi_grp_threads(g->epi_narrow) / kWave, 1u << 20);
     PR_TRY(plan_epi_order(g));
-  }
+    PR_TRY(plan_in0(g));
+  }
+  g->epi_elide = g->opts.epi_elide;
   const int64_t ep_parts = C > 1 ? (g->nblk + kEpiGroup - 1) / kEpiGroup : 0;
   PR_TRY(g->unit_part.alloc(sizeof(double) * 2 * ((size_t)g->n_units + ep_parts + 1)));
   PR_TRY(g->reset_part.alloc(sizeof(double) * 2 * g->reset_blocks));
diff --git a/pagerank-using-apache-spark_amd/csrc/pr_epi_modes.h b/pagerank-using-apache-spark_amd/csrc/pr_epi_modes.h
--- /dev/null
+++ b/pagerank-using-apache-spark_amd/csrc/pr_epi_modes.h
@@ -0,0 +1,50 @@
+#pragma once
+
+#include <stdint.h>
+
+#if defined(__HIPCC__)
+#define PR_HD __host__ __device__
+#else
+#define PR_HD
+#endif
+
+namespace pr {
+
+constexpr int kEpiFull = 0;
+constexpr int kEpiMid = 1;
+constexpr int kEpiMidWriteR = 2;
+
+PR_HD inline int epi_mode(int64_t it, int64_t K, bool elide) {
+  if (!elide || K <= 2 || it >= K - 1) return kEpiFull;
+  return it == K - 2 ? kEpiMidWriteR : kEpiMid;
+}
+PR_HD inline bool epi_elides(int64_t K, bool elide) { return epi_mode(0, K, elide) != kEpiFull; }
+
+constexpr int64_t kEpiElideMinGroups = 256 * 4 * 4;
+PR_HD inline bool epi_elide_on(int setting, int64_t groups) {
+  return setting > 0 || (setting < 0 && groups >= kEpiElideMinGroups);
+}
+
+constexpr uint32_t kIn0FlagIndeg0 = 1u << 29;
+constexpr uint32_t kIn0FlagHole = 1u << 30;
+PR_HD inline bool in0_row(uint32_t rowinfo) { return (rowinfo & (kIn0FlagIndeg0 | kIn0FlagHole)) == kIn0FlagIndeg0; }
+PR_HD inline int64_t in0_pos(int64_t base, uint64_t ballot, int lane) {
+  return base + __builtin_popcountll(ballot & ((uint64_t(1) << lane) - 1));
+}
+
+inline int64_t in0_prefix(const int32_t *cnt, int64_t nblk, int32_t *base, int64_t *n_empty, int64_t *n_full) {
+  int64_t run = 0, e = 0, f = 0;
+  for (int64_t b = 0; b < nblk; ++b) {
+    base[b] = (int32_t)run;
+    run += cnt[b];
+    e += cnt[b] == 0;
+    f += cnt[b] == 64;
+    if (run > INT32_MAX) return -1;
+  }
+  base[nblk] = (int32_t)run;
+  *n_empty = e;
+  *n_full = f;
+  return run;
+}
+
+}
diff --git a/pagerank-using-apache-spark_amd/csrc/pr_graph.h b/pagerank-using-apache-spark_amd/csrc/pr_graph.h
--- a/pagerank-using-apache-spark_amd/csrc/pr_graph.h
+++ b/pagerank-using-apache-spark_amd/csrc/pr_graph.h
@@ -4,6 +4,7 @@
 
 #include <vector>
 
+#include "pr_epi_modes.h"
 #include "pr_internal.h"
 
 namespace pr {
@@ -23,6 +24,7 @@
   bool pack_fused = true;
   bool xchg_sdma = false;
   int epi_order = -1;
+  int epi_elide = -1;
 };
 
 struct pr_graph {
@@ -67,6 +69,9 @@
   int64_t n_walk_groups = 0;
   pr::DevBuf eoff, epos;
   pr::DevBuf epi_ord;
+  int epi_elide = -1;
+  pr::DevBuf in0_base, r0;
+  int64_t n_in0 = 0, n_in0_empty = 0, n_in0_full = 0;
   int64_t n_hunits = 0, n_segs = 0, nblk = 0, n_slots = 0;
   int64_t hot_cover_ppm = 0;
   pr::DevBuf cbuf[2];
@@ -132,6 +137,7 @@
 int iter_reset(pr_graph *g, const double *init_ranks_host);
 int plan_epi_walk(pr_graph *g);
 int plan_epi_order(pr_graph *g);
+int plan_in0(pr_graph *g);
 int prepare_hot_kernel();
 int prepare_tele_kernels(const pr_graph *g);
 int set_teleport_dense(pr_graph *g, const double *teleport);
@@ -144,7 +150,9 @@
 int set_hot_reserve(pr_graph *g, int per_xcd);
 bool hot_gather_dense(const pr_graph *g);
 int iter_step(pr_graph *g, int32_t iterations);
-int iter_compute(pr_graph *g);
+int iter_compute(pr_graph *g, int epi = 0);
+int iter_pack_in0(pr_graph *g);
+bool iter_elides(const pr_graph *g, int64_t iterations);
 int group_exchange(pr_graph *const *parts, int n, int buf);
 int build_exchange(pr_graph *g, const uint64_t *ukeys, int64_t m, int b, uint64_t mask, const int32_t *rank_of,
                    const int32_t *gpos, DevBuf *cmap);
diff --git a/pagerank-using-apache-spark_amd/csrc/pr_iter.hip b/pagerank-using-apache-spark_amd/csrc/pr_iter.hip
--- a/pagerank-using-apache-spark_amd/csrc/pr_iter.hip
+++ b/pagerank-using-apache-spark_amd/csrc/pr_iter.hip
@@ -158,6 +158,8 @@
         if ((walk || narrow) && c > kWave) continue;
         PR_HIP(hipFuncSetAttribute(reinterpret_cast<const void *>(epi_grp_kernel(c, walk, narrow)),
                                    hipFuncAttributeMaxDynamicSharedMemorySize, (int)epi_grp_lds(narrow)));
+        PR_HIP(hipFuncSetAttribute(reinterpret_cast<const void *>(epi_mid_kernel(c, walk, narrow)),
+                                   hipFuncAttributeMaxDynamicSharedMemorySize, (int)epi_grp_lds(narrow)));
       }
   return PR_OK;
 }
@@ -166,6 +168,35 @@
   if (g->C <= 1) return PR_OK;
   PR_HIP(hipFuncSetAttribute(reinterpret_cast<const void *>(epi_grp_kernel(g->C, g->epi_walk, g->epi_narrow, true)),
                              hipFuncAttributeMaxDynamicSharedMemorySize, (int)epi_grp_lds(g->epi_narrow)));
+  PR_HIP(hipFuncSetAttribute(reinterpret_cast<const void *>(epi_mid_kernel(g->C, g->epi_walk, g->epi_narrow, true)),
+                             hipFuncAttributeMaxDynamicSharedMemorySize, (int)epi_grp_lds(g->epi_narrow)));
+  return PR_OK;
+}
+
+int plan_in0(pr_graph *g) {
+  g->n_in0 = g->n_in0_empty = g->n_in0_full = 0;
+  if (g->C <= 1 || g->nblk <= 0) return PR_OK;
+  DevBuf dcnt, dbad;
+  PR_TRY(dcnt.alloc(sizeof(int32_t) * (size_t)g->nblk));
+  PR_TRY(dbad.alloc(sizeof(unsigned)));
+  PR_HIP(hipMemsetAsync(dbad.p, 0, sizeof(unsigned), g->stream));
+  const int mw = (g->C + 31) / 32;
+  hipLaunchKernelGGL(k_in0_count, dim3(grid_for(g->nblk, kThreads / kWave, 8192)), dim3(kThreads), 0, g->stream,
+                     g->nblk, g->rowinfo.as<uint32_t>(), g->rmask.as<uint32_t>(), mw, dcnt.as<int32_t>(),
+                     dbad.as<unsigned>());
+  PR_HIP(hipGetLastError());
+  std::vector<int32_t> cnt((size_t)g->nblk), base((size_t)g->nblk + 1);
+  unsigned bad = 0;
+  PR_HIP(hipMemcpyAsync(cnt.data(), dcnt.p, sizeof(int32_t) * cnt.size(), hipMemcpyDeviceToHost, g->stream));
+  PR_HIP(hipMemcpyAsync(&bad, dbad.p, sizeof(unsigned), hipMemcpyDeviceToHost, g->stream));
+  PR_HIP(hipStreamSynchronize(g->stream));
+  if (bad) return fail(PR_ERR_STATE, "rows whose in-degree-0 flag and class mask disagree");
+  g->n_in0 = in0_prefix(cnt.data(), g->nblk, base.data(), &g->n_in0_empty, &g->n_in0_full);
+  if (g->n_in0 < 0) return fail(PR_ERR_INVALID, "more than 2^31 rows without in-links");
+  PR_TRY(g->in0_base.alloc(sizeof(int32_t) * base.size()));
+  PR_TRY(g->r0.alloc(sizeof(double) * (size_t)(g->n_in0 + 1)));
+  PR_HIP(hipMemcpyAsync(g->in0_base.p, base.data(), sizeof(int32_t) * base.size(), hipMemcpyHostToDevice, g->stream));
+  PR_HIP(hipStreamSynchronize(g->stream));
   return PR_OK;
 }
 
@@ -360,7 +391,18 @@
 int64_t epi_groups(const pr_graph *g) { return (g->nblk + kEpiGroup - 1) / kEpiGroup; }
 }
 
-int iter_compute(pr_graph *g) {
+bool iter_elides(const pr_graph *g, int64_t iterations) {
+  return g->C > 1 && g->nblk > 0 && epi_elides(iterations, epi_elide_on(g->epi_elide, epi_groups(g)));
+}
+
+int iter_pack_in0(pr_graph *g) {
+  hipLaunchKernelGGL(k_in0_pack, dim3(grid_for(g->nblk, kThreads / kWave, 8192)), dim3(kThreads), 0, g->stream, g->nblk,
+                     g->rowinfo.as<uint32_t>(), g->in0_base.as<int32_t>(), g->r.as<double>(), g->r0.as<double>());
+  PR_HIP(hipGetLastError());
+  return PR_OK;
+}
+
+int iter_compute(pr_graph *g, int epi_md) {
   hipStream_t s = g->stream;
   const int64_t own = g->own_off;
   const int in = g->cur, out = g->cur ^ 1;
@@ -435,7 +477,19 @@
     }
     const int64_t ngrp = epi_groups(g);
     const int32_t *ord = g->epi_ord.p ? g->epi_ord.as<int32_t>() + (ipc_early(g) ? ngrp : 0) : nullptr;
+    const EpiMidFn epi_mid = epi_md == kEpiFull ? nullptr : epi_mid_kernel(g->C, g->epi_walk, g->epi_narrow, tele != nullptr);
     auto epilogue = [&](int64_t g_lo, int64_t g_hi, unsigned grid) -> int {
+      if (epi_mid) {
+        hipLaunchKernelGGL(epi_mid, dim3(grid), dim3(epi_grp_threads(g->epi_narrow)), epi_grp_lds(g->epi_narrow), s,
+                           g->nblk, g_lo, g_hi, g->partial.as<double>(), g->rmask.p, g->cbase.as<int32_t>(),
+                           g->rowinfo.as<uint32_t>(), g->r.as<double>(), g->cbuf[out].as<double>() + own,
+                           g->cbuf[in].as<double>(), g->slots, (double)g->V, g->teleport, g->damping,
+                           g->unit_part.as<double2>() + g->n_units, g->eoff.as<int64_t>(), g->epos.as<uint16_t>(),
+                           g->x_pmask.as<uint8_t>(), g->x_sbase.as<int32_t>(), ord, pd, tele, g->r0.as<double>(),
+                           g->in0_base.as<int32_t>(), epi_md == kEpiMidWriteR ? 1 : 0);
+        PR_HIP(hipGetLastError());
+        return PR_OK;
+      }
       hipLaunchKernelGGL(epi, dim3(grid), dim3(epi_grp_threads(g->epi_narrow)), epi_grp_lds(g->epi_narrow), s,
                          g->nblk, g_lo, g_hi, g->partial.as<double>(), g->rmask.p, g->cbase.as<int32_t>(),
                          g->rowinfo.as<uint32_t>(), g->r.as<double>(), g->cbuf[out].as<double>() + own,
@@ -473,15 +527,16 @@
 int iter_step(pr_graph *g, int32_t iterations) {
   if (!g->ready) return fail(PR_ERR_STATE, "pr_step before pr_reset");
   if (g->grouped) return fail(PR_ERR_STATE, "graph belongs to a group: use pr_group_step");
+  const bool elide = iter_elides(g, iterations);
   if (g->timing && g->nparts == 1 && iterations > 0) {
     hipEvent_t e0 = next_event(g);
     if (!e0) return fail(PR_ERR_HIP, "hipEventCreate failed");
     PR_HIP(hipEventRecord(e0, g->stream));
     const int i0 = (int)g->ev_next - 1;
     g->timing = false;
-    int rc = PR_OK;
+    int rc = elide ? iter_pack_in0(g) : PR_OK;
     for (int32_t it = 0; it < iterations && rc == PR_OK; ++it) {
-      rc = iter_compute(g);
+      rc = iter_compute(g, epi_mode(it, iterations, elide));
       if (rc == PR_OK) rc = exchange(g, g->cur);
     }
     g->timing = true;
@@ -496,6 +551,7 @@
     g->iter_timed += iterations;
     return PR_OK;
   }
+  if (elide) PR_TRY(iter_pack_in0(g));
   int carry = -1;
   for (int32_t it = 0; it < iterations; ++it) {
     hipEvent_t e0 = nullptr, e1 = nullptr;
@@ -507,7 +563,7 @@
       i0 = (int)g->ev_next - 1;
     }
     g->ev_start_hint = g->timing ? i0 : -1;
-    PR_TRY(iter_compute(g));
+    PR_TRY(iter_compute(g, epi_mode(it, iterations, elide)));
     hipEvent_t xa = nullptr, xb = nullptr;
     if (g->timing && g->nparts > 1) {
       xa = next_event(g);
diff --git a/pagerank-using-apache-spark_amd/csrc/pr_spmv.h b/pagerank-using-apache-spark_amd/csrc/pr_spmv.h
--- a/pagerank-using-apache-spark_amd/csrc/pr_spmv.h
+++ b/pagerank-using-apache-spark_amd/csrc/pr_spmv.h
@@ -3,6 +3,7 @@
 #include <climits>
 
 #include "pr_device.h"
+#include "pr_epi_modes.h"
 #include "pr_internal.h"
 
 namespace pr {
@@ -805,6 +806,9 @@
   const uint8_t *pmask;
   const int32_t *sbase;
   const double *tele;
+  double *r0 = nullptr;
+  const int32_t *in0_base = nullptr;
+  int write_r = 0;
 };
 
 #ifndef PR_EPI_DMA_AUX
@@ -817,7 +821,7 @@
 #define PR_EPI_TELE_EARLY 0
 #endif
 
-template <int C, bool WALK, bool TELE>
+template <int C, bool WALK, bool TELE, bool MID = false>
 __device__ __forceinline__ void epi_group(const EpiArgs &a, const PackDst &pd, int64_t gi, double tdc, double *win,
                                           double2 *__restrict__ ep_part) {
   double dcp = 0.0, l1p = 0.0;
@@ -826,6 +830,8 @@
   static_assert(MW == 1 || MW == 2 || MW == 4, "mask words");
   static_assert(W >= 64 * G + 2, "one class run of a group must fit the window");
   static_assert(!WALK || C <= kWave, "the per-row walk needs at most 64 classes");
+  static_assert(!(MID && PR_EPI_LATE_ROW), "the mid epilogue takes rowinfo before the class loop");
+  static_assert(kIn0FlagIndeg0 == kRowIndeg0 && kIn0FlagHole == kRowHole, "pr_epi_modes.h rowinfo bits");
   const int lane = lane_id();
   const int64_t b0 = gi * G;
   const int nb = (int)min((int64_t)G, a.nblk - b0);
@@ -851,7 +857,7 @@
     }
 #if !PR_EPI_LATE_ROW
     info[g] = ok ? a.rowinfo[L] : kRowHole;
-    rold[g] = ok ? a.r[L] : 0.0;
+    if constexpr (!MID) rold[g] = ok ? a.r[L] : 0.0;
 #endif
 #if PR_EPI_TELE_EARLY
     if constexpr (TELE) tv[g] = ok ? a.tele[L] : 0.0;
@@ -860,12 +866,25 @@
   }
   const int cs = lane < C ? a.cbase[b0 * C + lane] : 0;
   const int ce = lane < C ? a.cbase[(b0 + nb) * C + lane] : 0;
+  int in0_first = 0;
+  if constexpr (MID) in0_first = a.in0_base[b0];
+  auto load_in0 = [&]() {
+    int base = __builtin_amdgcn_readfirstlane(in0_first);
+#pragma unroll
+    for (int g = 0; g < G; ++g) {
+      const bool z = in0_row(info[g]);
+      const unsigned long long bal = __ballot(z);
+      rold[g] = z ? a.r0[in0_pos(base, bal, lane)] : 0.0;
+      base += __popcll(bal);
+    }
+  };
   if constexpr (C <= kWave) {
     const int sa = cs & ~1;
     const int n2 = (lane < C && ce > cs) ? (((ce + 1) & ~1) - sa) : 0;
     const int incl = wave_incl_scan_i32(n2);
     const int pre = incl - n2;
     const int roff = incl - n2 + (cs - sa);
+    if constexpr (MID) load_in0();
     bool walked = false;
     if constexpr (WALK) {
       const int64_t eo = a.eoff[gi];
@@ -934,6 +953,7 @@
     auto run_end = [&](int y) {
       return y < kWave ? __builtin_amdgcn_readlane(ce, y) : __builtin_amdgcn_readlane(ce1, y - kWave);
     };
+    if constexpr (MID) load_in0();
     for (int x = 0; x < C;) {
       int fill = 0, xe = x;
       for (; xe < C; ++xe) {
@@ -988,7 +1008,8 @@
     const double rn = affine(Sv, tdc, tv[g], a.damping);
     double cn = 0.0;
     if (!(info[g] & kRowHole)) {
-      a.r[L] = rn;
+      if constexpr (!MID) a.r[L] = rn;
+      else if (a.write_r) a.r[L] = rn;
       const uint32_t d = info[g] & kRowDegMask;
       if (d > 0) {
         cn = __ddiv_rn(rn, (double)d);
@@ -996,9 +1017,20 @@
       } else if (info[g] & kRowSink) {
         dcp = __dadd_rn(dcp, rn);
       }
-      l1p = __dadd_rn(l1p, fabs(rn - rold[g]));
+      if constexpr (!MID) l1p = __dadd_rn(l1p, fabs(rn - rold[g]));
     }
     cnv[g] = cn;
+    if constexpr (MID) rold[g] = rn;
+  }
+  if constexpr (MID) {
+    int base = __builtin_amdgcn_readfirstlane(in0_first);
+#pragma unroll
+    for (int g = 0; g < G; ++g) {
+      const bool z = in0_row(info[g]);
+      const unsigned long long bal = __ballot(z);
+      if (z) a.r0[in0_pos(base, bal, lane)] = rold[g];
+      base += __popcll(bal);
+    }
   }
   static_assert(G * kWave <= W, "a group's run for one peer fits the window");
   if (pd.P > 1) {
@@ -1024,7 +1056,7 @@
     }
   }
   dcp = wave_sum(dcp);
-  l1p = wave_sum(l1p);
+  if constexpr (!MID) l1p = wave_sum(l1p);
   if (lane == 0) ep_part[gi] = make_double2(dcp, l1p);
 }
 
@@ -1058,6 +1090,60 @@
     epi_group<C, WALK, TELE>(a, pd, order ? (int64_t)order[k] : k, tdc, win, ep_part);
 }
 
+template <int C, bool WALK, int NT, bool TELE>
+__global__ PR_EPI_BOUNDS(NT) void k_epilogue_grp_mid(
+    int64_t nblk, int64_t g_lo, int64_t g_hi, const double *__restrict__ partial, const void *__restrict__ rmask_v,
+    const int32_t *__restrict__ cbase, const uint32_t *__restrict__ rowinfo, double *__restrict__ r,
+    double *__restrict__ cout, const double *__restrict__ cin, SlotPos sp, double n_vertices, double teleport,
+    double damping, double2 *__restrict__ ep_part , const int64_t *__restrict__ eoff,
+    const uint16_t *__restrict__ epos, const uint8_t *__restrict__ pmask, const int32_t *__restrict__ sbase,
+    const int32_t *__restrict__ order, PackDst pd, const double *__restrict__ tele, double *__restrict__ r0,
+    const int32_t *__restrict__ in0_base, int write_r) {
+  constexpr int W = kEpiWin;
+  constexpr int NW = NT / kWave;
+  extern __shared__ double epi_lds[];
+  const EpiArgs a{nblk, partial, rmask_v, cbase, rowinfo, r,    cout, teleport, damping,
+                  eoff, epos,    pmask,   sbase, tele,    r0,   in0_base, write_r};
+  const int lane = lane_id();
+  const int wv = __builtin_amdgcn_readfirstlane(wave_id());
+  double *win = epi_lds + wv * (W + 2);
+  if (lane == 0) win[W] = 0.0;
+  const double tdc = dc_from_slots(cin, sp) / n_vertices;
+  const int64_t nw = (int64_t)gridDim.x * NW;
+  for (int64_t k = g_lo + (int64_t)blockIdx.x * NW + wv; k < g_hi; k += nw)
+    epi_group<C, WALK, TELE, true>(a, pd, order ? (int64_t)order[k] : k, tdc, win, ep_part);
+}
+
+__global__ __launch_bounds__(kThreads) void k_in0_pack(int64_t nblk, const uint32_t *__restrict__ rowinfo,
+                                                       const int32_t *__restrict__ in0_base,
+                                                       const double *__restrict__ r, double *__restrict__ r0) {
+  const int lane = lane_id();
+  const int64_t nw = (int64_t)gridDim.x * (kThreads / kWave);
+  for (int64_t b = (int64_t)blockIdx.x * (kThreads / kWave) + wave_id(); b < nblk; b += nw) {
+    const int64_t L = b * kWave + lane;
+    const bool z = in0_row(rowinfo[L]);
+    const unsigned long long bal = __ballot(z);
+    if (z) r0[in0_pos(in0_base[b], bal, lane)] = r[L];
+  }
+}
+
+__global__ __launch_bounds__(kThreads) void k_in0_count(int64_t nblk, const uint32_t *__restrict__ rowinfo,
+                                                        const uint32_t *__restrict__ rmask, int mw,
+                                                        int32_t *__restrict__ cnt, unsigned *__restrict__ bad) {
+  const int lane = lane_id();
+  const int64_t nw = (int64_t)gridDim.x * (kThreads / kWave);
+  for (int64_t b = (int64_t)blockIdx.x * (kThreads / kWave) + wave_id(); b < nblk; b += nw) {
+    const int64_t L = b * kWave + lane;
+    const uint32_t info = rowinfo[L];
+    uint32_t any = 0u;
+    for (int w = 0; w < mw; ++w) any |= rmask[L * mw + w];
+    const bool z = in0_row(info);
+    if (!(info & kRowHole) && z != (any == 0u)) atomicAdd(bad, 1u);
+    const unsigned long long bal = __ballot(z);
+    if (lane == 0) cnt[b] = __popcll(bal);
+  }
+}
+
 template <int C, bool COUNT>
 __global__ __launch_bounds__(kEpiThreads) void k_epi_walk_plan(int64_t nblk, const void *__restrict__ rmask_v,
                                                                const int32_t *__restrict__ cbase,
@@ -1152,4 +1238,31 @@
   return tele ? epi_grp_kernel_t<true>(C, walk, narrow) : epi_grp_kernel_t<false>(C, walk, narrow);
 }
 
-}
+using EpiMidFn = void (*)(int64_t, int64_t, int64_t, const double *, const void *, const int32_t *, const uint32_t *, double *,
+                          double *, const double *, SlotPos, double, double, double, double2 *, const int64_t *,
+                          const uint16_t *, const uint8_t *, const int32_t *, const int32_t *, PackDst, const double *,
+                          double *, const int32_t *, int);
+template <int C, bool TELE>
+inline EpiMidFn epi_mid_kernel_c(bool walk, bool narrow) {
+  if constexpr (C <= kWave) {
+    if (narrow)
+      return walk ? k_epilogue_grp_mid<C, true, kEpiThreadsNarrow, TELE> : k_epilogue_grp_mid<C, false, kEpiThreadsNarrow, TELE>;
+    if (walk) return k_epilogue_grp_mid<C, true, kEpiThreads, TELE>;
+  }
+  return k_epilogue_grp_mid<C, false, kEpiThreads, TELE>;
+}
+template <bool TELE>
+inline EpiMidFn epi_mid_kernel_t(int C, bool walk, bool narrow) {
+  switch (C) {
+    case 8: return epi_mid_kernel_c<8, TELE>(walk, narrow);
+    case 16: return epi_mid_kernel_c<16, TELE>(walk, narrow);
+    case 32: return epi_mid_kernel_c<32, TELE>(walk, narrow);
+    case 64: return epi_mid_kernel_c<64, TELE>(walk, narrow);
+    default: return epi_mid_kernel_c<128, TELE>(false, false);
+  }
+}
+inline EpiMidFn epi_mid_kernel(int C, bool walk, bool narrow, bool tele = false) {
+  return tele ? epi_mid_kernel_t<true>(C, walk, narrow) : epi_mid_kernel_t<false>(C, walk, narrow);
+}
+
+}
diff --git a/pagerank-using-apache-spark_amd/host/epi_modes_shim.cpp b/pagerank-using-apache-spark_amd/host/epi_modes_shim.cpp
--- /dev/null
+++ b/pagerank-using-apache-spark_amd/host/epi_modes_shim.cpp
@@ -0,0 +1,28 @@
+#include "pr_epi_modes.h"
+
+#include <cstddef>
+#include <vector>
+
+extern "C" {
+int pre_mode(int64_t it, int64_t K, int elide) { return pr::epi_mode(it, K, elide != 0); }
+int pre_elides(int64_t K, int elide) { return pr::epi_elides(K, elide != 0) ? 1 : 0; }
+int pre_elide_on(int setting, int64_t groups) { return pr::epi_elide_on(setting, groups) ? 1 : 0; }
+int64_t pre_elide_min_groups(void) { return pr::kEpiElideMinGroups; }
+int pre_mode_consts(int *full, int *mid, int *mid_write_r) {
+  *full = pr::kEpiFull, *mid = pr::kEpiMid, *mid_write_r = pr::kEpiMidWriteR;
+  return 3;
+}
+int64_t pre_positions(const uint32_t *rowinfo, int64_t n_rows, int32_t *base, int64_t *pos, int64_t *n_empty,
+                      int64_t *n_full) {
+  const int64_t nblk = (n_rows + 63) / 64;
+  std::vector<uint64_t> bal((size_t)nblk, 0);
+  std::vector<int32_t> cnt((size_t)nblk, 0);
+  for (int64_t L = 0; L < n_rows; ++L)
+    if (pr::in0_row(rowinfo[L])) bal[L / 64] |= uint64_t(1) << (L % 64);
+  for (int64_t b = 0; b < nblk; ++b) cnt[b] = __builtin_popcountll(bal[b]);
+  const int64_t total = pr::in0_prefix(cnt.data(), nblk, base, n_empty, n_full);
+  for (int64_t L = 0; L < n_rows; ++L)
+    pos[L] = pr::in0_row(rowinfo[L]) ? pr::in0_pos(base[L / 64], bal[L / 64], (int)(L % 64)) : -1;
+  return total;
+}
+}
diff --git a/pagerank-using-apache-spark_amd/sparky_hip/_lib.py b/pagerank-using-apache-spark_amd/sparky_hip/_lib.py
--- a/pagerank-using-apache-spark_amd/sparky_hip/_lib.py
+++ b/pagerank-using-apache-spark_amd/sparky_hip/_lib.py
@@ -30,10 +30,11 @@
 INFO_NAMES = ["n_vertices", "n_edges", "n_sink", "n_nolink", "n_indeg0", "max_indeg", "local_rows",
               "local_edges", "part", "n_parts", "n_units", "n_long_rows", "device_bytes", "classes",
               "xchg_send", "xchg_recv", "partial_slots", "hot_slots", "epilogue", "gather_est",
-              "walk_groups", "layout", "hot_cover_ppm", "code_bits", "hot_gather"]
+              "walk_groups", "layout", "hot_cover_ppm", "code_bits", "hot_gather", "in0_rows",
+              "in0_empty_blocks", "in0_full_blocks"]
 BUILD_OPTIONS = {"classes": 1, "hot_slots": 2, "exchange_allgather": 3, "xchg_chunks": 4, "hot_reserve": 5,
                  "epi_walk": 6, "epi_narrow": 7, "codes": 8, "pack_fused": 9, "xchg_sdma": 10,
-                 "epi_order": 11}
+                 "epi_order": 11, "epi_elide": 12}
 STAT_NAMES = ["iters", "last_dc", "last_l1", "spmv_ms_mean", "spmv_launches", "iter_ms_mean",
               "build_ms", "exchange_ms_mean"]
 PR_CB_RANKS = 1
@@ -42,6 +43,7 @@
 PR_OPT_XCHG_IPC = 3
 PR_OPT_XCHG_IPC_BLIT = 4
 PR_OPT_HOT_GATHER = 5
+PR_OPT_EPI_ELIDE = 6
 PR_COMM_ID_BYTES = 128
 
 EXPORTED = [
diff --git a/pagerank-using-apache-spark_amd/sparky_hip/graph.py b/pagerank-using-apache-spark_amd/sparky_hip/graph.py
--- a/pagerank-using-apache-spark_amd/sparky_hip/graph.py
+++ b/pagerank-using-apache-spark_amd/sparky_hip/graph.py
@@ -229,6 +229,9 @@
     def set_hot_gather(self, mode: int) -> None:
         check(_lib.load().pr_set_option(self._h, _lib.PR_OPT_HOT_GATHER, int(mode)))
 
+    def set_epi_elide(self, mode) -> None:
+        check(_lib.load().pr_set_option(self._h, _lib.PR_OPT_EPI_ELIDE, int(mode)))
+
     def set_exchange_ipc(self, mode) -> None:
         v = int(mode)
         if v not in (0, 1, 2):
```
